# ucsdmanorlab/PSSR2

Hardware: AMD Instinct MI355X
Metric: HR tiles/sec (512^2 4xSR) train (higher is better)
Workload: dtype bf16

## Files before the change

### include/pssr_mi355.h

```cpp
#ifndef PSSR_MI355_H
#define PSSR_MI355_H

#include <stdint.h>

#ifdef __cplusplus
extern "C" {
#endif

typedef void* pssr_stream_t;

enum { PSSR_F32 = 0, PSSR_BF16 = 1, PSSR_F16 = 2 };

enum {
    PSSR_OK = 0,
    PSSR_ERR_ARG = -1,
    PSSR_ERR_LAUNCH = -2,
    PSSR_ERR_UNSUPPORTED = -3
};

int pssr_abi_version(void);
const char* pssr_last_error(void);

int pssr_pack_conv_weight(const float* w_oihw, void* packed, int cout, int cin, int ks,
                          int ci_begin, int ci_count, int mode, const int32_t* n_perm,
                          int k_pad, int n_pad, int dtype, pssr_stream_t stream);
typedef struct pssr_pack_item {
    const float* w; void* packed; const int32_t* n_perm;
    int32_t cout, cin, ks, ci_begin, ci_count, mode, k_pad, n_pad, dtype, center;
} pssr_pack_item;
int pssr_pack_conv_weight_batch(const pssr_pack_item* items_dev, int n_items, pssr_stream_t stream);
int64_t pssr_packed_weight_bytes(int taps, int k_pad, int n_pad, int dtype);

int pssr_unpack_conv_wgrad(const float* dw_packed, float* dw_oihw, int cout, int cin, int ks,
                           int ci_begin, int ci_count, int mode, const int32_t* n_perm,
                           int k_pad, int accumulate, pssr_stream_t stream);
int pssr_unpack_conv_wgrad_parts(const float* dw_parts, int parts, int rows, float* dw_oihw, int cout, int cin, int ks,
                                 int ci_begin, int ci_count, int mode, const int32_t* n_perm,
                                 int k_pad, int accumulate, pssr_stream_t stream);

enum { PSSR_PRO_NONE = 0, PSSR_PRO_BN_RELU = 1,
       PSSR_PRO_GELU = 2  };
enum {
    PSSR_EPI_STORE = 0,
    PSSR_EPI_TAIL = 1,
    PSSR_EPI_DGRAD_MASK = 2,
    PSSR_EPI_DGRAD_GELU = 4,
    PSSR_EPI_HEADQ = 5,
    PSSR_EPI_FINAL = 3
};
#define PSSR_STAT_STRIPES 32
#define PSSR_STAT_ROWS (2 * PSSR_STAT_STRIPES)

enum {
    PSSR_FLAG_RELU = 1,
    PSSR_FLAG_STATS = 2,
    PSSR_FLAG_HEADQ = 8,
    PSSR_FLAG_AFFINE = 4,
    PSSR_FLAG_SOLO = 32,
    PSSR_FLAG_SHUF2 = 16
};

typedef struct pssr_conv_desc {
    int32_t dtype;
    int32_t n, h, w;
    const void* in0; int32_t in0_cstride, in0_coff, cin0, taps0;
    const void* w0;
    const void* in1; int32_t in1_cstride, in1_coff, cin1, taps1;
    const void* w1;
    int32_t prologue;
    const float* pro_scale;
    const float* pro_shift;
    void* out; int32_t out_cstride, out_coff, cout, n_pad;
    const float* bias;
    int32_t epilogue, flags;
    const void* aux; int32_t aux_cstride, aux_coff;
    const float* aux_scale; const float* aux_shift;
    const float* aux_mean; const float* aux_invstd;
    double* stats;
    int32_t in0_blk, out_blk, aux_blk;
    float out_scale, out_shift;
    void* workspace; int64_t workspace_bytes;
    const float* head_w; float* head_q;
} pssr_conv_desc;

int pssr_conv2d(const pssr_conv_desc* desc, pssr_stream_t stream);
int64_t pssr_conv2d_workspace_bytes(const pssr_conv_desc* desc);
int pssr_conv2d_pipeline_mode(int mode);

int pssr_set_option(const char* name, int value);
int pssr_get_option(const char* name);

typedef struct pssr_wgrad_desc {
    int32_t dtype;
    int32_t n, h, w;
    const void* dy; int32_t dy_cstride, dy_coff, dy_blk, cout;
    const void* in; int32_t in_cstride, in_coff, in_blk, cin_pad;
    int32_t taps;
    int32_t prologue; const float* pro_scale; const float* pro_shift;
    float* dw;
    int32_t dw_parts;
} pssr_wgrad_desc;

int pssr_conv2d_wgrad(const pssr_wgrad_desc* desc, pssr_stream_t stream);
int pssr_conv2d_wgrad_parts(const pssr_wgrad_desc* desc);



int pssr_channel_stats_nchw(const float* x, int n, int c, int64_t hw, float pre_scale, float pre_shift,
                            double* stats, pssr_stream_t stream);

int pssr_bn_finalize(const double* stats, double count, const float* gamma, const float* beta, float eps,
                     float momentum, float* running_mean, float* running_var, float* scale, float* shift,
                     float* mean, float* invstd, int c, pssr_stream_t stream);
int pssr_bn_eval_affine(const float* gamma, const float* beta, const float* running_mean,
                        const float* running_var, float eps, float* scale, float* shift, int c,
                        pssr_stream_t stream);
int pssr_bn_relu_apply(const void* y, int y_cs, int y_co, const float* scale, const float* shift, void* a, int a_cs,
                       int a_co, int64_t npix, int c, int dtype, pssr_stream_t stream);
int pssr_bn_bwd_coefs(const double* stats, double count, const float* gamma, const float* mean,
                      const float* invstd, float* coef_a, float* coef_b, float* coef_c, float* dgamma,
                      float* dbeta, int c, pssr_stream_t stream);
int pssr_bn_bwd_apply(const void* g, int g_cs, int g_co, const void* y, int y_cs, int y_co,
                      const float* coef_a, const float* coef_b, const float* coef_c,
                      void* dy, int dy_cs, int dy_co, int64_t npix, int c, int dtype, pssr_stream_t stream);

int pssr_input_im2col(const float* x_nchw, void* xcol, int n, int c, int h, int w, int xc,
                      float pre_scale, float pre_shift, const float* scale, const float* shift,
                      int dtype, pssr_stream_t stream);
int pssr_input_norm_bwd(const void* dxcol_a, const void* dxcol_b, int xc, const float* x_nchw,
                        float pre_scale, float pre_shift, const float* mean, const float* invstd,
                        int n, int c, int h, int w, double* stats, int dtype, pssr_stream_t stream);

int pssr_input_norm_bwd2(const void* dxcol_a, const void* dxcol_b, int xc, const void* dpatch, int pc, int patch,
                         const float* x_nchw, float pre_scale, float pre_shift, const float* mean, const float* invstd,
                         int n, int c, int h, int w, double* stats, int dtype, pssr_stream_t stream);

int pssr_maxpool2(const void* in, int in_cs, int in_co, void* out, int out_cs, int out_co,
                  int n, int h, int w, int c, int dtype, pssr_stream_t stream);
int pssr_maxpool2_bwd(const void* act, int act_cs, int act_co, const void* dpool, int dp_cs, int dp_co,
                      const void* dskip, int ds_cs, int ds_co, void* dout, int do_cs, int do_co,
                      int n, int h, int w, int c, int dtype, pssr_stream_t stream);

int pssr_pixel_shuffle(const void* lo, int lo_cs, int lo_co, void* hi, int hi_cs, int hi_co,
                       int n, int h, int w, int c_hi, int r, int inverse, int dtype, pssr_stream_t stream);

int pssr_relu_bwd_stats(const void* dout, int do_cs, int do_co, const void* out, int o_cs, int o_co,
                        const void* y, int y_cs, int y_co, const float* mean, const float* invstd,
                        void* dz, int dz_cs, int dz_co, double* stats, int64_t npix, int c, int dtype,
                        pssr_stream_t stream);

int pssr_relu_bwd_stats_pool(const void* dpool, int dp_cs, int dp_co, const void* dskip, int ds_cs, int ds_co,
                             const void* out, int o_cs, int o_co, const void* y, int y_cs, int y_co,
                             const float* mean, const float* invstd, void* dz, int dz_cs, int dz_co, double* stats,
                             int n, int h, int w, int c, int dtype, pssr_stream_t stream);
int pssr_relu_bwd_stats_unshuffle(const void* dhi, int dh_cs, int dh_co, const void* out, int o_cs, int o_co,
                                  const void* y, int y_cs, int y_co, const float* mean, const float* invstd,
                                  void* dz, int dz_cs, int dz_co, double* stats, int n, int h, int w, int c, int dtype,
                                  pssr_stream_t stream);

int pssr_channel_sum_nhwc(const void* x, int cs, int co, int64_t npix, int c, double* out, int dtype,
                          pssr_stream_t stream);
int pssr_nchw_to_nhwc(const float* in, void* out, int n, int c, int64_t hw, int out_cs, float scale,
                      int dtype, pssr_stream_t stream);
int pssr_clip_u8(const float* in, uint8_t* out, int64_t n, pssr_stream_t stream);
int pssr_f64_to_f32(const double* in, float* out, int n, int accumulate, int stripes, pssr_stream_t stream);

int pssr_ssim_level_fwd(const float* x, const float* y, int planes, int h, int w, const float* win_host,
                        int k, float c1, float c2, double* sums, double* l1_sum, pssr_stream_t stream);
int pssr_avgpool2_planes(const float* in, float* out, int planes, int h, int w, pssr_stream_t stream);
int pssr_msssim_weights(const double* sums, int levels, int planes, const double* nvalid,
                        const float* level_weights, int ms, float mix, const double* l1_sum,
                        double l1_numel, const float* grad_out, float* loss_out, float* wts,
                        float* l1_coef, pssr_stream_t stream);
int pssr_ssim_level_bwd(const float* x, const float* y, int planes, int h, int w, const float* win_host,
                        int k, float c1, float c2, const float* wts, int use_ssim, const float* dcoarse,
                        int hc, int wc, const float* l1_coef, float* dx, pssr_stream_t stream);

int pssr_ssim_level_fwd_adj(const float* x, const float* y, float in_div, int planes, int h, int w, const float* win_host, int k,
                            float c1, float c2, int use_ssim, double* sums, double* l1_sum, int stripes, int64_t stripe_stride,
                            float* adj, pssr_stream_t stream);
int pssr_msssim_weights_striped(const double* sums, int stripes, int64_t stripe_stride, double* folded, int levels, int planes,
                                const double* nvalid, const float* level_weights, int ms, float mix, const double* l1_sum,
                                double l1_numel, const float* grad_out, float* loss_out, float* wts, float* l1_coef,
                                pssr_stream_t stream);
int pssr_ssim_level_bwd_adj(const float* x, const float* y, float in_div, const float* adj, int planes, int h, int w,
                            const float* win_host, int k, const float* wts, const float* dcoarse, int hc, int wc,
                            const float* l1_coef, float* dx, pssr_stream_t stream);
int pssr_avgpool2_planes_div(const float* in, float in_div, float* out, int planes, int h, int w, pssr_stream_t stream);
int pssr_avgpool2_pair_div(const float* x, const float* y, float in_div, float* xo, float* yo, int planes, int h, int w,
                           pssr_stream_t stream);

int pssr_adamw_step(float* p, const float* g, float* m, float* v, int64_t n, float lr, float beta1,
                    float beta2, float eps, float weight_decay, int64_t step, float grad_scale,
                    pssr_stream_t stream);
int pssr_adamw_step_dev(float* p, const float* g, float* m, float* v, int64_t n, int64_t* state,
                        float beta1, float beta2, float eps, float weight_decay, float grad_scale,
                        pssr_stream_t stream);
int pssr_amp_check(const float* g, int64_t n, int32_t* amp, pssr_stream_t stream);
int pssr_adamw_step_amp(float* p, const float* g, float* m, float* v, int64_t n, int64_t* state,
                        float beta1, float beta2, float eps, float weight_decay, float grad_scale,
                        int32_t* amp, float growth, float backoff, int interval, pssr_stream_t stream);

int pssr_bilinear_down_u8(const uint8_t* hr, uint8_t* tmp, uint8_t* lr, int planes, int H, int W,
                          int h, int w, pssr_stream_t stream);
int pssr_u8_to_f32(const uint8_t* in, float* out, int64_t n, pssr_stream_t stream);
int pssr_crappify_gaussian(const float* in, float* out, int tiles, int64_t per_tile, float intensity,
                           float gain, float spread, uint64_t seed, uint64_t tile_offset,
                           const double* noise, int flags, const uint64_t* tile_counter,
                           pssr_stream_t stream);
int pssr_crappify_poisson(const float* in, float* out, int tiles, int64_t per_tile, float intensity,
                          float gain, float spread, uint64_t seed, uint64_t tile_offset, int flags,
                          const uint64_t* tile_counter, pssr_stream_t stream);
int pssr_crappify_poisson_samples(const float* in, const double* samples, float* out, int64_t n, double intensity,
                                  double gain, int flags, pssr_stream_t stream);
int pssr_counter_add(uint64_t* counter, uint64_t inc, pssr_stream_t stream);
int pssr_gaussian_blur(const float* in, float* tmp, float* out, int planes, int h, int w, float sigma,
                       float gain, int flags, pssr_stream_t stream);

int pssr_crappify_saltpepper(const float* in, float* out, int tiles, int64_t per_tile, float amount, float gain, float spread,
                             uint64_t seed, uint64_t tile_offset, int flags, const uint64_t* tile_counter, pssr_stream_t stream);
int pssr_gaussian_blur_tiles(const float* in, float* tmp, float* out, int tiles, int planes_per_tile, int h, int w, float sigma,
                             float spread, float gain, uint64_t seed, uint64_t tile_offset, int flags, const uint64_t* tile_counter,
                             pssr_stream_t stream);
typedef struct pssr_gather_item { const uint8_t* src; int sh, sw, rot, flip_axis; } pssr_gather_item;
int pssr_gen_pair_geometry_u8(const pssr_gather_item* items_dev, int n_items, uint8_t* out, int c, int res, pssr_stream_t stream);
typedef struct pssr_sheet_desc { const uint8_t* base; int frames, h, w, reserved; } pssr_sheet_desc;
typedef struct pssr_window_item { int sheet, frame0, y0, x0, rot, flip_axis; } pssr_window_item;
int pssr_gather_windows_u8(const pssr_sheet_desc* sheets_dev, int n_sheets, const pssr_window_item* items_dev, int n_items,
                           uint8_t* out, int c, int res, pssr_stream_t stream);

typedef struct pssr_collage_panel {
    const void* src; int64_t image_stride; int32_t row_pitch, src_h, src_w, is_f32; const int32_t* yi; const int32_t* xi;
} pssr_collage_panel;
int pssr_collage_rows_u8(const pssr_collage_panel* panels, int n_panels, uint8_t* canvas, int64_t canvas_pitch, int row0, int n_images,
                         int h, int w, pssr_stream_t stream);

int64_t pssr_window_attn_workspace_bytes(int B, int H, int W, int heads, int ws);
int pssr_window_attn_fwd(const void* qkv, const float* bias_table, void* out, float* lse, int B, int H, int W, int C, int heads, int ws,
                         int shift, float scale, int dtype, pssr_stream_t stream);
int pssr_window_attn_bwd(const void* qkv, const float* bias_table, const float* lse, const void* dout, void* dqkv, float* dbias_table,
                         void* workspace, int64_t workspace_bytes, int B, int H, int W, int C, int heads, int ws, int shift, float scale,
                         int dtype, pssr_stream_t stream);


int pssr_input_plain(const float* x_nchw, void* out, int n, int c, int h, int w, int out_cs, float pre_scale, float pre_shift,
                     int dtype, pssr_stream_t stream);
int pssr_im2col_dil(const void* in, int in_cs, int in_co, int c, const float* scale, const float* shift, void* col, int cp,
                    int n, int h, int w, int dil, int dtype, pssr_stream_t stream);
int pssr_col2im_dil(const void* dcol, int cp, void* out, int out_cs, int out_co, int c, int n, int h, int w, int dil,
                    const void* y, int y_cs, int y_co, const float* scale, const float* shift, const float* mean,
                    const float* invstd, double* stats, int dtype, pssr_stream_t stream);
int pssr_channel_stats_nhwc(const void* x, int cs, int co, int c, int64_t npix, double* stats, int dtype, pssr_stream_t stream);
int pssr_sum_relu(const void* const* ins, const int* in_cs, const int* in_co, int n_in, void* out, int out_cs, int out_co,
                  int64_t npix, int c, int relu, int dtype, pssr_stream_t stream);
int pssr_relu_mask(const void* dout, int do_cs, int do_co, const void* out, int o_cs, int o_co, void* dz, int dz_cs, int dz_co,
                   int64_t npix, int c, int dtype, pssr_stream_t stream);
int pssr_affine_relu(const void* x, int cs, int co, const float* scale, const float* shift, void* out, int out_cs, int out_co,
                     int64_t npix, int c, int dtype, pssr_stream_t stream);
int pssr_maxpool_k(const void* in, int in_cs, int in_co, void* out, int out_cs, int out_co, int n, int h, int w, int c, int k,
                   int dtype, pssr_stream_t stream);
int pssr_maxpool_k_bwd(const void* act, int act_cs, int act_co, const void* dpool, int dp_cs, int dp_co, void* dx, int dx_cs,
                       int dx_co, int n, int h, int w, int c, int k, int dtype, pssr_stream_t stream);
int pssr_bilinear_up(const void* in, int in_cs, int in_co, void* out, int out_cs, int out_co, int n, int hs, int ws, int h, int w,
                     int c, int dtype, pssr_stream_t stream);
int pssr_bilinear_up_bwd(const void* dout, int do_cs, int do_co, void* din, int di_cs, int di_co, int n, int hs, int ws, int h,
                         int w, int c, int dtype, pssr_stream_t stream);

int pssr_input_patchify(const float* x_nchw, void* xpatch, int n, int c, int h, int w, int ps, int pc,
                        float pre_scale, float pre_shift, const float* scale, const float* shift, int dtype,
                        pssr_stream_t stream);
int pssr_dwconv7_pack(const float* w, float* packed, int c, int flip, pssr_stream_t stream);
#define PSSR_DWPACK_BATCH_MAX 48
typedef struct pssr_dwpack_batch {
    const float* w[PSSR_DWPACK_BATCH_MAX];
    float* packed[PSSR_DWPACK_BATCH_MAX];
    int32_t c[PSSR_DWPACK_BATCH_MAX];
    int32_t flip[PSSR_DWPACK_BATCH_MAX];
} pssr_dwpack_batch;
int pssr_dwconv7_pack_batch(const pssr_dwpack_batch* items, int n_items, pssr_stream_t stream);
int pssr_dwconv7(const void* in, int in_cs, int in_co, const float* w_packed, const float* bias, void* out, int out_cs,
                 int out_co, int n, int h, int w, int c, int accumulate, int dtype, pssr_stream_t stream);
int pssr_dwconv7_wgrad(const void* dy, int dy_cs, int dy_co, const void* x, int x_cs, int x_co, float* dw, int n, int h,
                       int w, int c, int dtype, pssr_stream_t stream);
int64_t pssr_dwconv7_wgrad_workspace_bytes(int n, int h, int w, int c);
int pssr_dwconv7_wgrad_ws(const void* dy, int dy_cs, int dy_co, const void* x, int x_cs, int x_co, float* dw, int n, int h,
                          int w, int c, int dtype, void* workspace, int64_t workspace_bytes, pssr_stream_t stream);
int pssr_layernorm2d_fwd(const void* in, int in_cs, int in_co, const float* gamma, const float* beta, float eps, void* out,
                         int out_cs, int out_co, int s2d, int c_pad, int n, int h, int w, int c, float* mean, float* rstd,
                         int dtype, pssr_stream_t stream);
int pssr_layernorm2d_bwd(const void* g, int g_cs, int g_co, int s2d, int c_pad, const void* x, int x_cs, int x_co,
                         const float* gamma, const float* mean, const float* rstd, void* dx, int dx_cs, int dx_co,
                         int accumulate, int n, int h, int w, int c, double* stats, int dtype, pssr_stream_t stream);
int pssr_image_channel_dot(const void* a, int a_cs, int a_co, const void* b, int b_cs, int b_co, int n, int hw, int c,
                           float scale, float* out, int dtype, pssr_stream_t stream);
int64_t pssr_image_channel_dot_workspace_bytes(int n, int hw, int c);
int pssr_image_channel_dot_ws(const void* a, int a_cs, int a_co, const void* b, int b_cs, int b_co, int n, int hw, int c,
                              float scale, float* out, int dtype, void* workspace, int64_t workspace_bytes, pssr_stream_t stream);
int pssr_ese_gate(const float* s_mean, const float* w_fc, const float* b_fc, int n, int c, float* u, float* gate,
                  pssr_stream_t stream);
int pssr_scale_nc(const void* t, int t_cs, int t_co, const float* gate, const float* gamma, const float* add, void* out,
                  int out_cs, int out_co, int n, int hw, int c, int dtype, pssr_stream_t stream);
int pssr_ese_bwd(const float* A, const float* gate, const float* u, const float* gamma, const float* s_mean,
                 const float* w_fc, int n, int c, int hw, float* du, float* dgamma, float* db_fc, float* dw_fc, float* add,
                 pssr_stream_t stream);

int pssr_head_q_gather(const float* q, const float* bias, float* out_nchw, int n, int h, int w,
                       float out_scale, float out_shift, pssr_stream_t stream);

int pssr_head_conv_fwd(const void* act, int act_cs, int act_co, int blk, const float* w_oihw, const float* bias,
                       float* out_nchw, int n, int h, int w, int cin, int cout, float out_scale, float out_shift,
                       int dtype, pssr_stream_t stream);
int pssr_head_conv_dgrad(const float* g_nchw, float g_scale, const float* w_oihw, const void* act, int act_cs, int act_co,
                         void* dact, int d_cs, int d_co, int blk, int n, int h, int w, int cin, int cout, int dtype,
                         pssr_stream_t stream);
int pssr_head_conv_wgrad(const float* g_nchw, float g_scale, const void* act, int act_cs, int act_co, int blk,
                         float* dw_oihw, int n, int h, int w, int cin, int cout, int dtype, pssr_stream_t stream);
int pssr_head_conv_bwd(const float* g_nchw, float g_scale, const float* w_oihw, const void* act, int act_cs, int act_co,
                       void* dact, int d_cs, int d_co, int blk, float* dw_oihw, float* bias_sum, int n, int h, int w, int cin,
                       int cout, int dtype, pssr_stream_t stream);

int pssr_head_conv_bwd_rows(const float* g_nchw, float g_scale, const float* w_oihw, const void* act, int act_cs, int act_co,
                            void* dact, int d_cs, int d_co, int blk, double* dw_rows, double* bias_rows, int n, int h, int w,
                            int cin, int cout, int dtype, pssr_stream_t stream);

int pssr_sliding_tiles_u8(const uint8_t* sheet, float* tiles, int c, int h, int w, int size, int stride, int tile0, int ntile,
                          pssr_stream_t stream);
int pssr_patch_tiles_u8(const uint8_t* tiles, uint8_t* sheet, int c, int n_rows, int n_cols, int size, int overlap, int margin,
                        pssr_stream_t stream);


int64_t pssr_normalize_preds_workspace_bytes(int64_t pixels_per_image);
int pssr_normalize_preds_u8(const uint8_t* hr, const uint8_t* hr_hat, uint8_t* hr_norm, uint8_t* hr_hat_norm, int n_images,
                            int64_t pixels_per_image, float pmin, float pmax, void* workspace, pssr_stream_t stream);
// ... 55 lines not shown
```

### pssr2_amd/_lib.py

```python
from __future__ import annotations

import ctypes as C
import os
from pathlib import Path

_LIB_PATH = Path(__file__).resolve().parent / "libpssr_mi355.so"
_lib = None

F32, BF16, F16 = 0, 1, 2
PRO_NONE, PRO_BN_RELU, PRO_GELU = 0, 1, 2
EPI_STORE, EPI_TAIL, EPI_DGRAD_MASK, EPI_FINAL, EPI_DGRAD_GELU, EPI_HEADQ = 0, 1, 2, 3, 4, 5
FLAG_RELU, FLAG_STATS, FLAG_AFFINE, FLAG_HEADQ, FLAG_SHUF2, FLAG_SOLO = 1, 2, 4, 8, 16, 32

c_void_p, c_int, c_i64, c_float = C.c_void_p, C.c_int, C.c_int64, C.c_float


class ConvDesc(C.Structure):
    _fields_ = [
        ("dtype", C.c_int32), ("n", C.c_int32), ("h", C.c_int32), ("w", C.c_int32),
        ("in0", c_void_p), ("in0_cstride", C.c_int32), ("in0_coff", C.c_int32), ("cin0", C.c_int32), ("taps0", C.c_int32),
        ("w0", c_void_p),
        ("in1", c_void_p), ("in1_cstride", C.c_int32), ("in1_coff", C.c_int32), ("cin1", C.c_int32), ("taps1", C.c_int32),
        ("w1", c_void_p),
        ("prologue", C.c_int32), ("pro_scale", c_void_p), ("pro_shift", c_void_p),
        ("out", c_void_p), ("out_cstride", C.c_int32), ("out_coff", C.c_int32), ("cout", C.c_int32), ("n_pad", C.c_int32),
        ("bias", c_void_p),
        ("epilogue", C.c_int32), ("flags", C.c_int32),
        ("aux", c_void_p), ("aux_cstride", C.c_int32), ("aux_coff", C.c_int32),
        ("aux_scale", c_void_p), ("aux_shift", c_void_p), ("aux_mean", c_void_p), ("aux_invstd", c_void_p),
        ("stats", c_void_p),
        ("in0_blk", C.c_int32), ("out_blk", C.c_int32), ("aux_blk", C.c_int32),
        ("out_scale", C.c_float), ("out_shift", C.c_float),
        ("workspace", c_void_p), ("workspace_bytes", C.c_int64),
        ("head_w", c_void_p), ("head_q", c_void_p),
    ]


class WgradDesc(C.Structure):
    _fields_ = [
        ("dtype", C.c_int32), ("n", C.c_int32), ("h", C.c_int32), ("w", C.c_int32),
        ("dy", c_void_p), ("dy_cstride", C.c_int32), ("dy_coff", C.c_int32), ("dy_blk", C.c_int32), ("cout", C.c_int32),
        ("in_", c_void_p), ("in_cstride", C.c_int32), ("in_coff", C.c_int32), ("in_blk", C.c_int32), ("cin_pad", C.c_int32),
        ("taps", C.c_int32),
        ("prologue", C.c_int32), ("pro_scale", c_void_p), ("pro_shift", c_void_p),
        ("dw", c_void_p), ("dw_parts", C.c_int32),
    ]


class GatherItem(C.Structure):
    _fields_ = [("src", C.c_void_p), ("sh", C.c_int), ("sw", C.c_int), ("rot", C.c_int), ("flip_axis", C.c_int)]


class SheetDesc(C.Structure):
    _fields_ = [("base", C.c_void_p), ("frames", C.c_int), ("h", C.c_int), ("w", C.c_int), ("reserved", C.c_int)]


class WindowItem(C.Structure):
    _fields_ = [("sheet", C.c_int), ("frame0", C.c_int), ("y0", C.c_int), ("x0", C.c_int), ("rot", C.c_int), ("flip_axis", C.c_int)]


class CollagePanel(C.Structure):
    _fields_ = [("src", C.c_void_p), ("image_stride", C.c_int64), ("row_pitch", C.c_int32), ("src_h", C.c_int32), ("src_w", C.c_int32),
                ("is_f32", C.c_int32), ("yi", C.c_void_p), ("xi", C.c_void_p)]


COPY_BATCH_MAX = 16


class FoldBatch(C.Structure):
    _fields_ = [("dst", C.c_void_p * 16), ("src", C.c_void_p * 16), ("n", C.c_int32 * 16), ("accumulate", C.c_int32 * 16)]


DWPACK_BATCH_MAX = 48


class DwPackBatch(C.Structure):
    _fields_ = [("w", C.c_void_p * DWPACK_BATCH_MAX), ("packed", C.c_void_p * DWPACK_BATCH_MAX), ("c", C.c_int32 * DWPACK_BATCH_MAX),
                ("flip", C.c_int32 * DWPACK_BATCH_MAX)]


class CopyBatch(C.Structure):
    _fields_ = [("dst", C.c_void_p * COPY_BATCH_MAX), ("src", C.c_void_p * COPY_BATCH_MAX), ("n", C.c_int64 * COPY_BATCH_MAX)]


class PackItem(C.Structure):
    _fields_ = [("w", c_void_p), ("packed", c_void_p), ("n_perm", c_void_p),
                ("cout", C.c_int32), ("cin", C.c_int32), ("ks", C.c_int32), ("ci_begin", C.c_int32), ("ci_count", C.c_int32),
                ("mode", C.c_int32), ("k_pad", C.c_int32), ("n_pad", C.c_int32), ("dtype", C.c_int32), ("center", C.c_int32)]


def lib():
    global _lib
    if _lib is None:
        if not _LIB_PATH.exists():
            raise RuntimeError(
                f"{_LIB_PATH} not found: build the HIP extension first (python -c 'import __graft_entry__ as g; g.build()' "
                "or make -C pssr2_amd/csrc). pssr2_amd has no CPU fallback.")
        import torch
        _lib = C.CDLL(str(_LIB_PATH))
        _lib.pssr_last_error.restype = C.c_char_p
        _lib.pssr_packed_weight_bytes.restype = C.c_int64
        _lib.pssr_conv2d_workspace_bytes.restype = C.c_int64
        _lib.pssr_gradhist_workspace_bytes.restype = C.c_int64
        _lib.pssr_noise_profile_workspace_bytes.restype = C.c_int64
        _lib.pssr_noise_profile_workspace_bytes.argtypes = [c_int, c_i64]
        for name in ("pssr_noise_profile_f32", "pssr_noise_profile_u8"):
            getattr(_lib, name).argtypes = [c_void_p, c_void_p, c_void_p, c_void_p, c_int, c_i64, c_void_p, c_i64, c_void_p]
        _lib.pssr_noise_profile_loss.argtypes = [c_void_p, c_void_p, c_void_p, c_void_p, c_int, c_i64, c_int, c_void_p, c_void_p, c_void_p,
                                                 c_void_p]
        _lib.pssr_gather_windows_u8.argtypes = [c_void_p, c_int, c_void_p, c_int, c_void_p, c_int, c_int, c_void_p]
        _lib.pssr_collage_rows_u8.argtypes = [c_void_p, c_int, c_void_p, c_i64, c_int, c_int, c_int, c_int, c_void_p]
        _lib.pssr_window_attn_workspace_bytes.restype = c_i64
        _lib.pssr_window_attn_workspace_bytes.argtypes = [c_int] * 5
        _lib.pssr_window_attn_fwd.argtypes = [c_void_p] * 4 + [c_int] * 7 + [c_float, c_int, c_void_p]
        _lib.pssr_window_attn_bwd.argtypes = [c_void_p] * 7 + [c_i64] + [c_int] * 7 + [c_float, c_int, c_void_p]
    return _lib


def check(status: int, what: str):
    if status != 0:
        raise RuntimeError(f"{what} failed ({status}): {lib().pssr_last_error().decode()}")


def ptr(t):
    return None if t is None else c_void_p(t.data_ptr())


def stream_ptr():
    import torch
    return c_void_p(torch.cuda.current_stream().cuda_stream)
```

### pssr2_amd/csrc/conv_igemm.hip

```cpp
#include "conv_igemm_args.h"

using pssr_conv::ConvArgs;

extern "C" int pssr_conv2d_pipeline_mode(int mode) {
    (void)mode;
    return 0;
}

static int conv2d_entry(const pssr_conv_desc* d, pssr_stream_t stream, long* query_ws);

#ifdef PSSR_V3_STAMPS
static unsigned* g_stamp_buf = nullptr;
extern "C" void pssr_debug_stamp_buffer(void* p) { g_stamp_buf = (unsigned*)p; }
#endif

extern "C" int pssr_conv2d(const pssr_conv_desc* d, pssr_stream_t stream) { return conv2d_entry(d, stream, nullptr); }

extern "C" int64_t pssr_conv2d_workspace_bytes(const pssr_conv_desc* d) {
    long bytes = 0;
    const int rc = conv2d_entry(d, nullptr, &bytes);
    return rc != PSSR_OK ? (int64_t)rc : (int64_t)bytes;
}

static int conv2d_entry(const pssr_conv_desc* d, pssr_stream_t stream, long* query_ws) {
    PSSR_CHECK(d != nullptr, PSSR_ERR_ARG, "conv2d: null desc");
    PSSR_CHECK(d->dtype == PSSR_F32 || d->dtype == PSSR_BF16 || d->dtype == PSSR_F16, PSSR_ERR_ARG, "conv2d: bad dtype %d", d->dtype);
    const int kch = d->dtype == PSSR_F32 ? 8 : 16;
    const int esz = d->dtype == PSSR_F32 ? 4 : 2;
    PSSR_CHECK(d->n > 0 && d->h > 0 && d->w > 0, PSSR_ERR_ARG, "conv2d: bad shape %dx%dx%d", d->n, d->h, d->w);
    PSSR_CHECK(query_ws || (d->in0 && d->w0 && d->out), PSSR_ERR_ARG, "conv2d: null pointer");
    PSSR_CHECK(d->cin0 > 0 && d->cin0 % kch == 0, PSSR_ERR_ARG, "conv2d: cin0=%d must be a positive multiple of %d", d->cin0, kch);
    PSSR_CHECK(d->taps0 == 9 || d->taps0 == 1, PSSR_ERR_ARG, "conv2d: taps0=%d", d->taps0);
    PSSR_CHECK((d->in0_cstride * esz) % 16 == 0 && (d->in0_coff * esz) % 16 == 0, PSSR_ERR_ARG, "conv2d: in0 stride/offset not 16-byte aligned");
    PSSR_CHECK(d->in0_coff + d->cin0 <= d->in0_cstride, PSSR_ERR_ARG, "conv2d: in0 slice exceeds stride");
    if (d->cin1) {
        PSSR_CHECK(d->in1 && d->w1 && d->cin1 % kch == 0 && d->taps1 == 1, PSSR_ERR_ARG, "conv2d: source 1 must be a 1x1 (or flat-K) source");
        PSSR_CHECK((d->in1_cstride * esz) % 16 == 0 && (d->in1_coff * esz) % 16 == 0 && d->in1_coff + d->cin1 <= d->in1_cstride, PSSR_ERR_ARG, "conv2d: in1 stride/offset");
    }
    if (d->epilogue == PSSR_EPI_FINAL) {
        PSSR_CHECK(d->cout > 0 && d->cout <= 32 && (d->flags & ~PSSR_FLAG_SOLO) == 0, PSSR_ERR_ARG, "conv2d: EPI_FINAL needs 0 < cout <= 32 and no flags");
    } else {
        PSSR_CHECK(d->cout > 0 && d->cout % 4 == 0, PSSR_ERR_ARG, "conv2d: cout=%d must be a positive multiple of 4", d->cout);
        PSSR_CHECK(d->out_coff % 4 == 0 && d->out_cstride % 4 == 0 &&
                   d->out_coff + ((d->flags & PSSR_FLAG_SHUF2) ? d->cout / 4 : d->cout) <= d->out_cstride, PSSR_ERR_ARG, "conv2d: out stride/offset");
    }
    PSSR_CHECK(d->n_pad % 128 == 0 && d->n_pad >= d->cout, PSSR_ERR_ARG, "conv2d: n_pad=%d", d->n_pad);
    PSSR_CHECK(d->prologue >= 0 && d->prologue <= PSSR_PRO_GELU, PSSR_ERR_ARG, "conv2d: prologue=%d", d->prologue);
    PSSR_CHECK(d->prologue != PSSR_PRO_BN_RELU || (d->pro_scale && d->pro_shift), PSSR_ERR_ARG, "conv2d: prologue needs scale/shift");
    PSSR_CHECK(d->epilogue >= 0 && d->epilogue <= 5, PSSR_ERR_ARG, "conv2d: epilogue=%d", d->epilogue);
    if (d->flags & PSSR_FLAG_HEADQ)
        PSSR_CHECK(d->epilogue == PSSR_EPI_STORE && !(d->flags & (PSSR_FLAG_STATS | PSSR_FLAG_AFFINE)) && (d->flags & PSSR_FLAG_RELU), PSSR_ERR_ARG,
                   "conv2d: FLAG_HEADQ goes with EPI_STORE | FLAG_RELU only");
    if (d->epilogue == PSSR_EPI_HEADQ || (d->flags & PSSR_FLAG_HEADQ)) {
        PSSR_CHECK(query_ws || (d->head_w && d->head_q), PSSR_ERR_ARG, "conv2d: EPI_HEADQ needs head_w / head_q");
        PSSR_CHECK(esz == 2 && d->cout == 1024 && d->taps0 == 9 && d->w >= 16 && d->h >= 16 && d->prologue != PSSR_PRO_GELU && !(d->flags & PSSR_FLAG_STATS),
                   PSSR_ERR_UNSUPPORTED, "conv2d: EPI_HEADQ needs 16-bit storage, a 3x3 source, cout = 16 x 64 (4 x upscaling) and at least 16x16 pixels");
    }
    PSSR_CHECK(d->in0_blk >= 0 && d->out_blk >= 0 && d->aux_blk >= 0 && d->in0_blk <= 3 && d->out_blk <= 3 && d->aux_blk <= 3, PSSR_ERR_ARG, "conv2d: blocked order");
    {
        const int mb = d->in0_blk > d->out_blk ? (d->in0_blk > d->aux_blk ? d->in0_blk : d->aux_blk) : (d->out_blk > d->aux_blk ? d->out_blk : d->aux_blk);
        PSSR_CHECK(d->h % (1 << mb) == 0 && d->w % (1 << mb) == 0, PSSR_ERR_ARG, "conv2d: blocked order needs H,W multiples of r");
    }
    if (d->epilogue == PSSR_EPI_TAIL || d->epilogue == PSSR_EPI_DGRAD_MASK) {
        PSSR_CHECK(d->aux && d->aux_scale && d->aux_shift && d->aux_coff % 4 == 0 && d->aux_cstride % 4 == 0, PSSR_ERR_ARG, "conv2d: epilogue needs aux tensor");
    }
    if (d->epilogue == PSSR_EPI_DGRAD_GELU)
        PSSR_CHECK(d->aux && d->aux_coff % 4 == 0 && d->aux_cstride % 4 == 0, PSSR_ERR_ARG, "conv2d: GELU backward needs the pre-activation as aux");
    if (d->flags & PSSR_FLAG_SHUF2) {
        PSSR_CHECK(d->epilogue == PSSR_EPI_STORE && !(d->flags & (PSSR_FLAG_STATS | PSSR_FLAG_HEADQ)) && d->out_blk == 0, PSSR_ERR_ARG,
                   "conv2d: FLAG_SHUF2 goes with EPI_STORE, without statistics, tap planes or a blocked output order");
        PSSR_CHECK(esz == 2 && d->cout % 32 == 0 && d->out_coff % 8 == 0 && d->out_cstride % 8 == 0 && pssr_tunables().conv_epi8, PSSR_ERR_UNSUPPORTED,
                   "conv2d: FLAG_SHUF2 needs 16-bit storage, cout a multiple of 32 and 8-channel aligned outputs");
    }
    if (d->flags & PSSR_FLAG_AFFINE) {
        PSSR_CHECK(d->epilogue == PSSR_EPI_STORE && !(d->flags & PSSR_FLAG_STATS) && d->aux_scale && d->aux_shift, PSSR_ERR_ARG,
                   "conv2d: FLAG_AFFINE needs EPI_STORE without statistics and aux_scale / aux_shift");
        PSSR_CHECK(esz == 2 && d->cout % 8 == 0 && d->out_coff % 8 == 0 && d->out_cstride % 8 == 0 && pssr_tunables().conv_epi8, PSSR_ERR_UNSUPPORTED,
                   "conv2d: FLAG_AFFINE needs 16-bit storage and 8-channel aligned outputs");
    }
    if (d->flags & PSSR_FLAG_STATS) {
        PSSR_CHECK(d->stats != nullptr, PSSR_ERR_ARG, "conv2d: stats buffer missing");
        PSSR_CHECK(d->epilogue != PSSR_EPI_DGRAD_MASK || (d->aux_mean && d->aux_invstd), PSSR_ERR_ARG, "conv2d: mask stats need mean/invstd");
        PSSR_CHECK(d->epilogue != PSSR_EPI_TAIL, PSSR_ERR_ARG, "conv2d: no stats on tail");
    }
    ConvArgs a;
    a.N = d->n; a.H = d->h; a.W = d->w;
    a.in[0] = d->in0; a.in_cs[0] = d->in0_cstride; a.in_co[0] = d->in0_coff; a.nchunks[0] = d->cin0 / kch; a.taps[0] = d->taps0; a.w[0] = d->w0;
    a.in[1] = d->in1; a.in_cs[1] = d->in1_cstride; a.in_co[1] = d->in1_coff; a.nchunks[1] = d->cin1 ? d->cin1 / kch : 0; a.taps[1] = d->cin1 ? d->taps1 : 1; a.w[1] = d->w1;
    a.prologue = d->prologue; a.pro_scale = d->pro_scale; a.pro_shift = d->pro_shift;
    a.out = d->out; a.out_cs = d->out_cstride; a.out_co = d->out_coff; a.cout = d->cout; a.n_pad = d->n_pad;
    a.bias = d->bias; a.epi = d->epilogue; a.flags = d->flags;
    a.aux = d->aux; a.aux_cs = d->aux_cstride; a.aux_co = d->aux_coff;
    a.aux_scale = d->aux_scale; a.aux_shift = d->aux_shift; a.aux_mean = d->aux_mean; a.aux_invstd = d->aux_invstd;
    a.stats = d->stats;
    a.in0_blk = d->in0_blk; a.out_blk = d->out_blk; a.aux_blk = d->aux_blk;
    a.out_scale = d->out_scale; a.out_shift = d->out_shift;
    const bool headq = a.epi == PSSR_EPI_HEADQ || (a.flags & PSSR_FLAG_HEADQ);
    a.head_w = headq ? d->head_w : nullptr;
    a.head_q = headq ? d->head_q : nullptr;
    a.tiles_x = a.tiles_y = a.tiles_n = 0;
    a.epi8 = esz == 2 && d->epilogue != PSSR_EPI_FINAL && d->cout % 8 == 0 && d->out_coff % 8 == 0 && d->out_cstride % 8 == 0 &&
             (d->epilogue == PSSR_EPI_STORE || d->epilogue == PSSR_EPI_HEADQ || (d->aux_coff % 8 == 0 && d->aux_cstride % 8 == 0));
    if (!pssr_tunables().conv_epi8) a.epi8 = 0;
    a.dbg = pssr_tunables().igemm_dbg;
    a.stamps = nullptr;
#ifdef PSSR_V3_STAMPS
    a.stamps = g_stamp_buf;
#endif
    long ws_query = 0;
    if (query_ws) { a.ksplit = -1; a.ws = (float*)&ws_query; }
    else { a.ws = (float*)d->workspace; a.ksplit = d->workspace ? (int)(d->workspace_bytes / 1024) : 0; }
    hipStream_t s = (hipStream_t)stream;
    const int rc = d->dtype == PSSR_BF16 ? pssr_conv::launch_bf16(a, s) : d->dtype == PSSR_F16 ? pssr_conv::launch_f16(a, s) : pssr_conv::launch_f32(a, s);
    if (query_ws) *query_ws = ws_query;
    return rc;
}
```

### pssr2_amd/csrc/conv_igemm_args.h

```cpp
#pragma once
#include "common.h"
#include "tunables.h"

namespace pssr_conv {

struct ConvArgs {
    int N, H, W;
    int tiles_x, tiles_y, tiles_n;
    const void* in[2]; int in_cs[2]; int in_co[2]; int nchunks[2]; int taps[2]; const void* w[2];
    int prologue; const float* pro_scale; const float* pro_shift;
    void* out; int out_cs, out_co, cout, n_pad;
    const float* bias;
    int epi, flags;
    const void* aux; int aux_cs, aux_co;
    const float* aux_scale; const float* aux_shift; const float* aux_mean; const float* aux_invstd;
    double* stats;
    int in0_blk, out_blk, aux_blk;
    float out_scale, out_shift;
    int epi8;
    unsigned* stamps;
    int dbg;
    int ksplit; float* ws;
    const float* head_w; float* head_q;
};

int launch_bf16(const ConvArgs& a, hipStream_t s);
int launch_f16(const ConvArgs& a, hipStream_t s);
int launch_f32(const ConvArgs& a, hipStream_t s);

}
```

### pssr2_amd/csrc/conv_igemm_impl.h

```cpp
#pragma once
#include <type_traits>

#include "conv_igemm_args.h"

using pssr_conv::ConvArgs;

namespace {



constexpr int PRO_LDS_MAX = 4096 * 8;

template <int GEO> struct Geo;
template <> struct Geo<0> { static constexpr int TWL = 4, THL = 3; };
template <> struct Geo<1> { static constexpr int TWL = 3, THL = 3; };
template <> struct Geo<2> { static constexpr int TWL = 2, THL = 2; };
template <> struct Geo<3> { static constexpr int TWL = 1, THL = 1; };
template <> struct Geo<4> { static constexpr int TWL = 0, THL = 0; };
template <> struct Geo<5> { static constexpr int TWL = 4, THL = 4; };

template <int BN, int GEO> struct Cfg {
    static constexpr int TWL = Geo<GEO>::TWL, THL = Geo<GEO>::THL;
    static constexpr bool BIG = GEO == 5;
    static_assert(!BIG || BN == 64, "the 256-pixel tile is built for 64 output channels");
// ... 4 lines not shown
    static constexpr int HW2 = TW + 2, HPI = (TH + 2) * (TW + 2), HP = NI * HPI;
    static constexpr int HWP = (TW == 16 && !BIG) ? 32 : HW2;
    static constexpr int HPIP = (TH + 2) * HWP;
    static constexpr int A_ITEMS = (2 * HP + 255) / 256;
    static constexpr int A_BYTES = NI * HPIP * 32;
    static constexpr int B_BYTES = 9 * BN * 32;
    static constexpr int B_ITEMS = (9 * BN * 2 + 255) / 256;
    static constexpr int E_BYTES = WM * 32 * BN * 4;
    static constexpr int RED_BYTES = 4 * BN * 2 * 4;
    static constexpr int MAIN_BYTES = A_BYTES + B_BYTES;
    static constexpr int LDS_BYTES = (MAIN_BYTES > E_BYTES + RED_BYTES) ? MAIN_BYTES : (E_BYTES + RED_BYTES);
    static constexpr int PERM = 0;
};

template <class C> __device__ __forceinline__ int epi_pixel(int row, int mi) {
    int r = row & 31;
    if constexpr (C::PERM != 0) {
        const int rx = r & 15, ry = (r >> 4) ^ ((rx >= 4 && rx < 12) ? 1 : 0);
        if constexpr (C::PERM == 2)
            return (((row >> 5) * 4 + (mi >> 1) * 2 + ry) << 5) | ((mi & 1) << 4) | rx;
        r = (ry << 4) | rx;
    }
    return (row >> 5) * C::MI * 32 + mi * 32 + r;
}

template <typename T, int BN, class C>
__device__ __forceinline__ void conv_epilogue(const ConvArgs& p, f32x16 (&acc)[C::MI][C::NJ], char* smem, int tid, int x0, int y0, int img0, int n0) {
    using X = TT<T>;
    const int lane = tid & 63, wave = tid >> 6;
    const int wm = wave / C::WN, wn = wave % C::WN;
    const int h = lane >> 5, r = lane & 31;
    float* Es = (float*)smem;
    float* Red = (float*)(smem + C::E_BYTES);
    constexpr int CG = BN / 4;
    constexpr int PASSES = C::WM * 32 * CG / 256;
#pragma unroll
    for (int nj = 0; nj < C::NJ; ++nj)
#pragma unroll
        for (int e = 0; e < 16; ++e) {
            const int row = wm * 32 + (e & 3) + 8 * (e >> 2) + 4 * h;
            const int col = wn * C::NJ * 32 + nj * 32 + r;
            Es[row * BN + col] = acc[0][nj][e];
        }
    asm volatile("" ::: "memory");
    const int c4 = tid % CG;
    const int n_base = n0 + c4 * 4;
    const bool n_ok = n_base < p.cout;
    float bias[4] = {0, 0, 0, 0}, xs[4] = {0, 0, 0, 0}, xh[4] = {0, 0, 0, 0}, xm[4] = {0, 0, 0, 0}, xi[4] = {0, 0, 0, 0};
    if (n_ok) {
        if (p.bias) {
            if (p.epi == PSSR_EPI_FINAL) { for (int e = 0; e < 4; ++e) if (n_base + e < p.cout) bias[e] = p.bias[n_base + e]; }
            else load4(p.bias + n_base, bias);
        }
        if (p.epi == PSSR_EPI_TAIL || p.epi == PSSR_EPI_DGRAD_MASK) { load4(p.aux_scale + n_base, xs); load4(p.aux_shift + n_base, xh); }
        if (p.epi == PSSR_EPI_DGRAD_MASK && (p.flags & PSSR_FLAG_STATS)) {
            load4(p.aux_mean + n_base, xm); load4(p.aux_invstd + n_base, xi);
        }
    }
    float s1[4] = {0, 0, 0, 0}, s2[4] = {0, 0, 0, 0};
    T* outp = (T*)p.out;
    const T* auxp = (const T*)p.aux;

#pragma unroll
    for (int mi = 0; mi < C::MI; ++mi) {
        if (mi) {
            __syncthreads();
#pragma unroll
            for (int nj = 0; nj < C::NJ; ++nj)
#pragma unroll
                for (int e = 0; e < 16; ++e) {
                    const int row = wm * 32 + (e & 3) + 8 * (e >> 2) + 4 * h;
                    const int col = wn * C::NJ * 32 + nj * 32 + r;
                    Es[row * BN + col] = acc[mi][nj][e];
                }
        }
        __syncthreads();
#pragma unroll
        for (int ps = 0; ps < PASSES; ++ps) {
            const int piece = tid + ps * 256;
            const int row = piece / CG;
            const int m = epi_pixel<C>(row, mi);
            const int tx = m & (C::TW - 1), ty = (m >> C::TWL) & (C::TH - 1), img = m >> (C::TWL + C::THL);
            const int gy = y0 + ty, gx = x0 + tx, gi = img0 + img;
            if (!(n_ok && gi < p.N && gy < p.H && gx < p.W)) continue;
            float v[4];
            load4(Es + row * BN + c4 * 4, v);
            if (p.epi == PSSR_EPI_FINAL) {
                float* of = (float*)p.out;
#pragma unroll
                for (int e = 0; e < 4; ++e)
                    if (n_base + e < p.cout)
                        of[(((long)gi * p.cout + n_base + e) * p.H + gy) * p.W + gx] = fmaf(v[e] + bias[e], p.out_scale, p.out_shift);
                continue;
            }
            const long pix = pix_index(gi, gy, gx, p.H, p.W, p.out_blk);
            if (p.epi == PSSR_EPI_STORE) {
#pragma unroll
                for (int e = 0; e < 4; ++e) {
                    v[e] += bias[e];
                    if (p.flags & PSSR_FLAG_RELU) v[e] = fmaxf(v[e], 0.f);
                }
            } else {
                float a[4];
                load4(auxp + pix_index(gi, gy, gx, p.H, p.W, p.aux_blk) * p.aux_cs + p.aux_co + n_base, a);
                if (p.epi == PSSR_EPI_TAIL) {
#pragma unroll
                    for (int e = 0; e < 4; ++e) v[e] = fmaxf(v[e] + bias[e] + fmaf(a[e], xs[e], xh[e]), 0.f);
                } else if (p.epi == PSSR_EPI_DGRAD_GELU) {
                    gelu_grad_mul_vec<T, 4>(a, v);
                } else {
#pragma unroll
                    for (int e = 0; e < 4; ++e) {
                        v[e] = (fmaf(a[e], xs[e], xh[e]) > 0.f) ? v[e] : 0.f;
                        a[e] = (a[e] - xm[e]) * xi[e];
                    }
                }
                if (p.flags & PSSR_FLAG_STATS) {
#pragma unroll
                    for (int e = 0; e < 4; ++e) { const float g = X::round(v[e]); s1[e] += g; s2[e] += g * a[e]; }
                }
            }
            if (p.epi == PSSR_EPI_STORE && (p.flags & PSSR_FLAG_STATS)) {
#pragma unroll
                for (int e = 0; e < 4; ++e) { const float g = X::round(v[e]); s1[e] += g; s2[e] += g * g; }
            }
            store4(outp + pix * p.out_cs + p.out_co + n_base, v);
        }
    }
    if (p.flags & PSSR_FLAG_STATS) {
#pragma unroll
        for (int off = 32; off >= CG; off >>= 1)
#pragma unroll
            for (int e = 0; e < 4; ++e) { s1[e] += __shfl_xor(s1[e], off); s2[e] += __shfl_xor(s2[e], off); }
        if (lane < CG) {
#pragma unroll
            for (int e = 0; e < 4; ++e) {
                Red[(wave * BN + lane * 4 + e) * 2 + 0] = s1[e];
                Red[(wave * BN + lane * 4 + e) * 2 + 1] = s2[e];
            }
        }
        __syncthreads();
        if (tid < BN && n0 + tid < p.cout) {
            float t1 = 0, t2 = 0;
#pragma unroll
            for (int w = 0; w < 4; ++w) { t1 += Red[(w * BN + tid) * 2]; t2 += Red[(w * BN + tid) * 2 + 1]; }
            double* st = p.stats + (long)(blockIdx.x % PSSR_STAT_STRIPES) * 2 * p.cout;
            const long lo = (long)PSSR_STAT_STRIPES * 2 * p.cout;
            stat_add(st + n0 + tid, lo, t1);
            stat_add(st + p.cout + n0 + tid, lo, t2);
        }
    }
}

template <typename T, int BN, class C, int EPI, bool STATS, bool TR = false, bool AFF = false>
__device__ __forceinline__ void conv_epilogue8(const ConvArgs& p, f32x16 (&acc)[C::MI][C::NJ], char* smem, int tid, int x0, int y0, int img0, int n0) {
    static_assert(!AFF || (EPI == PSSR_EPI_STORE && !STATS), "FLAG_AFFINE: EPI_STORE without statistics");
    using X = TT<T>;
    static_assert(sizeof(T) == 2, "8-channel pieces are 16 bytes of a 16-bit type");
    const int lane = tid & 63, wave = tid >> 6;
    const int wm = wave / C::WN, wn = wave % C::WN;
    const int h = lane >> 5, r = lane & 31;
    float* Es = (float*)smem;
    float* Red = (float*)(smem + C::E_BYTES);
    constexpr int CG = BN / 8, RP = 256 / CG;
    constexpr int EP = TR ? BN + 4 : BN;
    constexpr int ROWS = C::WM * 32, PASSES = ROWS / RP;
    static_assert(PASSES >= 1 && ROWS % RP == 0, "pass geometry");
    int wcol[C::NJ];
#pragma unroll
    for (int nj = 0; nj < C::NJ; ++nj) {
        const int col = wn * C::NJ * 32 + nj * 32 + r;
        wcol[nj] = ((col >> 2) & 1) * (BN / 2) + ((col >> 3) << 2) + (col & 3);
    }
    auto es_write = [&](int mi) {
        if constexpr (TR) {
#pragma unroll
            for (int nj = 0; nj < C::NJ; ++nj)
#pragma unroll
                for (int q = 0; q < 4; ++q) {
                    const int c = (wn * C::NJ + nj) * 4 + q;
                    *(float4*)(Es + (wm * 32 + r) * EP + h * (BN / 2) + 4 * c) =
                        make_float4(acc[mi][nj][4 * q], acc[mi][nj][4 * q + 1], acc[mi][nj][4 * q + 2], acc[mi][nj][4 * q + 3]);
                }
        } else {
#pragma unroll
            for (int nj = 0; nj < C::NJ; ++nj)
#pragma unroll
                for (int e = 0; e < 16; ++e) {
                    const int row = wm * 32 + (e & 3) + 8 * (e >> 2) + 4 * h;
                    Es[row * EP + wcol[nj]] = acc[mi][nj][e];
                }
        }
    };
    es_write(0);
    asm volatile("" ::: "memory");
    const int c8 = tid % CG, rs = tid / CG;
    const int row0 = (TR && CG == 8) ? ((rs >> 1) & 7) + ((rs & 1) << 3) + ((rs >> 4) << 4) : rs;
    const int n_base = n0 + c8 * 8;
    const bool n_ok = n_base < p.cout;
    float bias[8] = {0, 0, 0, 0, 0, 0, 0, 0}, xs[8], xh[8], xm[8], xi[8];
#pragma unroll
    for (int e = 0; e < 8; ++e) { xs[e] = 0.f; xh[e] = 0.f; xm[e] = 0.f; xi[e] = 0.f; }
    if (n_ok) {
        if ((EPI == PSSR_EPI_STORE || EPI == PSSR_EPI_TAIL) && p.bias) { load4(p.bias + n_base, bias); load4(p.bias + n_base + 4, bias + 4); }
        if (EPI == PSSR_EPI_TAIL || EPI == PSSR_EPI_DGRAD_MASK || AFF) {
            load4(p.aux_scale + n_base, xs); load4(p.aux_scale + n_base + 4, xs + 4);
            load4(p.aux_shift + n_base, xh); load4(p.aux_shift + n_base + 4, xh + 4);
        }
        if (EPI == PSSR_EPI_DGRAD_MASK && STATS) {
            load4(p.aux_mean + n_base, xm); load4(p.aux_mean + n_base + 4, xm + 4);
            load4(p.aux_invstd + n_base, xi); load4(p.aux_invstd + n_base + 4, xi + 4);
        }
    }
    const float relu_lo = (EPI == PSSR_EPI_STORE && (p.flags & PSSR_FLAG_RELU)) ? 0.f : -__builtin_inff();
    float s1[8], s2[8];
#pragma unroll
    for (int e = 0; e < 8; ++e) { s1[e] = 0.f; s2[e] = 0.f; }
    T* outp = (T*)p.out + p.out_co + n_base;
    const T* auxp = (const T*)p.aux + p.aux_co + n_base;
    const bool shuf = EPI == PSSR_EPI_STORE && !STATS && (p.flags & PSSR_FLAG_SHUF2);
    int shuf_i = 0, shuf_j = 0;
    if (shuf) {
        const int q4 = p.cout >> 2, s = n_base / q4;
        shuf_i = s >> 1; shuf_j = s & 1;
        outp = (T*)p.out + p.out_co + (n_base - s * q4);
    }

#pragma unroll
    for (int mi = 0; mi < C::MI; ++mi) {
        if (mi) {
            __syncthreads();
            es_write(mi);
        }
        __syncthreads();
#pragma unroll 1
        for (int ps = 0; ps < PASSES; ++ps) {
            const int row = row0 + ps * RP;
            const int m = epi_pixel<C>(row, mi);
            const int tx = m & (C::TW - 1), ty = (m >> C::TWL) & (C::TH - 1), img = m >> (C::TWL + C::THL);
            const int gy = y0 + ty, gx = x0 + tx, gi = img0 + img;
            if (!(n_ok && gi < p.N && gy < p.H && gx < p.W)) continue;
            float v[8];
            load4(Es + row * EP + c8 * 4, v);
            load4(Es + row * EP + BN / 2 + c8 * 4, v + 4);
            float a[8];
            if (EPI != PSSR_EPI_STORE) {
                const u32x4 araw = *(const u32x4*)(auxp + pix_index(gi, gy, gx, p.H, p.W, p.aux_blk) * p.aux_cs);
                X::unpack(araw, a);
            }
            if constexpr (EPI == PSSR_EPI_DGRAD_GELU) gelu_grad_mul_vec<T, 8>(a, v);
#pragma unroll
            for (int e = 0; e < 8; ++e) {
                if (EPI == PSSR_EPI_STORE) v[e] = fmaxf(AFF ? fmaf(v[e] + bias[e], xs[e], xh[e]) : v[e] + bias[e], relu_lo);
                else if (EPI == PSSR_EPI_TAIL) v[e] = fmaxf(v[e] + bias[e] + fmaf(a[e], xs[e], xh[e]), 0.f);
                else if (EPI == PSSR_EPI_DGRAD_GELU) {}
                else {
                    v[e] = (fmaf(a[e], xs[e], xh[e]) > 0.f) ? v[e] : 0.f;
                    a[e] = (a[e] - xm[e]) * xi[e];
                }
            }
            const u32x4 packed = X::pack(v);
            if (STATS) {
                float g[8];
                X::unpack(packed, g);
#pragma unroll
                for (int e = 0; e < 8; ++e) {
                    if (EPI == PSSR_EPI_DGRAD_GELU) asm volatile("v_add_f32 %0, %0, %1" : "+v"(s1[e]) : "v"(g[e]));
                    else s1[e] += g[e];
                    s2[e] += g[e] * (EPI == PSSR_EPI_STORE ? g[e] : a[e]);
                }
            }
            const long opix = shuf ? ((long)gi * 2 * p.H + 2 * gy + shuf_i) * (2 * p.W) + 2 * gx + shuf_j : pix_index(gi, gy, gx, p.H, p.W, p.out_blk);
            *(u32x4*)(outp + opix * p.out_cs) = packed;
        }
    }
    if (STATS) {
#pragma unroll
        for (int off = 32; off >= CG; off >>= 1)
#pragma unroll
            for (int e = 0; e < 8; ++e) { s1[e] += __shfl_xor(s1[e], off); s2[e] += __shfl_xor(s2[e], off); }
        if (lane < CG) {
#pragma unroll
            for (int e = 0; e < 8; ++e) {
                Red[(wave * BN + lane * 8 + e) * 2 + 0] = s1[e];
                Red[(wave * BN + lane * 8 + e) * 2 + 1] = s2[e];
            }
        }
        __syncthreads();
        if (tid < BN && n0 + tid < p.cout) {
            float t1 = 0, t2 = 0;
#pragma unroll
            for (int w = 0; w < 4; ++w) { t1 += Red[(w * BN + tid) * 2]; t2 += Red[(w * BN + tid) * 2 + 1]; }
            double* st = p.stats + (long)(blockIdx.x % PSSR_STAT_STRIPES) * 2 * p.cout;
            const long lo = (long)PSSR_STAT_STRIPES * 2 * p.cout;
            stat_add(st + n0 + tid, lo, t1);
            stat_add(st + p.cout + n0 + tid, lo, t2);
        }
    }
}

constexpr int HEADQ_LDS = (64 * 9 + 128) * 4;
__device__ __forceinline__ void conv_headq_stage(const ConvArgs& p, float* hq, int tid, int n0) {
    for (int i = tid; i < 64 * 9; i += 256) hq[i] = p.head_w[i];
    if (tid < 128) hq[576 + tid] = (p.bias && n0 + tid < p.cout) ? p.bias[n0 + tid] : 0.f;
}

template <typename T, class C>
__device__ __forceinline__ void conv_headq_epilogue(const ConvArgs& p, f32x16 (&acc)[C::MI][C::NJ], const float* hq, char* smem, int tid, int x0, int y0, int img0,
                                                    int n0) {
    using X = TT<T>;
    static_assert(sizeof(T) == 2 && C::NJ == 2 && C::MI == 4, "conv_v3 tiles of 128 channels");
    const int lane = tid & 63, wave = tid >> 6;
    const int wm = wave / C::WN, wn = wave % C::WN;
    const int h = lane >> 5, r = lane & 31;
    const int cbase = n0 + wn * 64;
    const int sub = cbase >> 6;
    float bias[2][16];
    u32x4 wa[2][2];
#pragma unroll
    for (int nj = 0; nj < 2; ++nj) {
#pragma unroll
        for (int e = 0; e < 16; ++e) bias[nj][e] = hq[576 + wn * 64 + nj * 32 + (e & 3) + 8 * (e >> 2) + 4 * h];
#pragma unroll
        for (int ks = 0; ks < 2; ++ks) {
            float wv[8];
#pragma unroll
            for (int i = 0; i < 8; ++i) {
                const int e = 8 * ks + i;
                const int c = nj * 32 + (e & 3) + 8 * (e >> 2) + 4 * h;
                wv[i] = r < 9 ? hq[c * 9 + r] : 0.f;
            }
            wa[nj][ks] = X::pack(wv);
        }
    }
    const long lrplane = (long)p.N * p.H * p.W;
    float* const qsub = p.head_q + (long)sub * lrplane + (long)img0 * p.H * p.W;
#pragma unroll
    for (int mi = 0; mi < 4; ++mi) {
        f32x16 q;
#pragma unroll
        for (int e = 0; e < 16; ++e) q[e] = 0.f;
#pragma unroll
        for (int nj = 0; nj < 2; ++nj)
#pragma unroll
            for (int ks = 0; ks < 2; ++ks) {
                float v[8];
#pragma unroll
                for (int i = 0; i < 8; ++i) v[i] = fmaxf(acc[mi][nj][8 * ks + i] + bias[nj][8 * ks + i], 0.f);
                X::mma(q, wa[nj][ks], X::pack(v));
            }
        const int m = epi_pixel<C>(wm * 32 + r, mi);
        const int tx = m & (C::TW - 1), ty = (m >> C::TWL) & (C::TH - 1);
        const int gy = y0 + ty, gx = x0 + tx;
        if (gy < p.H && gx < p.W) {
            float* const d = qsub + (long)gy * p.W + gx;
#pragma unroll
            for (int u = 0; u < 4; ++u) d[(long)(4 * h + u) * 16 * lrplane] = q[u];
            if (h == 0) d[(long)8 * 16 * lrplane] = q[4];
        }
    }
    (void)smem;
}

template <typename T, int BN, class C, bool TR = false>
__device__ __forceinline__ void conv_epilogue8_any(const ConvArgs& p, f32x16 (&acc)[C::MI][C::NJ], char* smem, int tid, int x0, int y0, int img0, int n0) {
    const bool st = p.flags & PSSR_FLAG_STATS;
    switch (p.epi) {
    case PSSR_EPI_STORE:
        if (st) conv_epilogue8<T, BN, C, PSSR_EPI_STORE, true, TR>(p, acc, smem, tid, x0, y0, img0, n0);
        else if (p.flags & PSSR_FLAG_AFFINE) conv_epilogue8<T, BN, C, PSSR_EPI_STORE, false, TR, true>(p, acc, smem, tid, x0, y0, img0, n0);
        else conv_epilogue8<T, BN, C, PSSR_EPI_STORE, false, TR>(p, acc, smem, tid, x0, y0, img0, n0);
        return;
    case PSSR_EPI_TAIL: conv_epilogue8<T, BN, C, PSSR_EPI_TAIL, false, TR>(p, acc, smem, tid, x0, y0, img0, n0); return;
    case PSSR_EPI_DGRAD_MASK:
        if (st) conv_epilogue8<T, BN, C, PSSR_EPI_DGRAD_MASK, true, TR>(p, acc, smem, tid, x0, y0, img0, n0);
        else conv_epilogue8<T, BN, C, PSSR_EPI_DGRAD_MASK, false, TR>(p, acc, smem, tid, x0, y0, img0, n0);
        return;
    default:
        if (st) conv_epilogue8<T, BN, C, PSSR_EPI_DGRAD_GELU, true, TR>(p, acc, smem, tid, x0, y0, img0, n0);
        else conv_epilogue8<T, BN, C, PSSR_EPI_DGRAD_GELU, false, TR>(p, acc, smem, tid, x0, y0, img0, n0);
        return;
    }
}

template <typename T, int BN, class C>
__device__ __forceinline__ void conv_epilogue_any(const ConvArgs& p, f32x16 (&acc)[C::MI][C::NJ], char* smem, int tid, int x0, int y0, int img0, int n0) {
    if constexpr (sizeof(T) == 2) {
        if (p.epi8) { conv_epilogue8_any<T, BN, C>(p, acc, smem, tid, x0, y0, img0, n0); return; }
    }
    conv_epilogue<T, BN, C>(p, acc, smem, tid, x0, y0, img0, n0);
}

template <typename T, int BN, int GEO, int TAPS0>
__global__ __launch_bounds__(256) void conv_igemm_kernel(const ConvArgs p) {
    using C = Cfg<BN, GEO>;
    using X = TT<T>;
    constexpr int EPS = X::EPS, KCH = X::KCH;
    extern __shared__ __attribute__((aligned(16))) char smem[];
    char* As = smem;
    char* Bs = smem + C::A_BYTES;

    const int tid = threadIdx.x, lane = tid & 63, wave = tid >> 6;
    const int wm = wave / C::WN, wn = wave % C::WN;
    const int h = lane >> 5, r = lane & 31;

    int bid = blockIdx.x;
    if (p.ksplit <= 1 && !(p.dbg & 64)) {
        const int per = gridDim.x >> 3;
        if (bid < per * 8) bid = (bid & 7) * per + (bid >> 3);
    }
    const int tn = bid % p.tiles_n;
    int tmi = bid / p.tiles_n;
    const int tile_x = tmi % p.tiles_x; tmi /= p.tiles_x;
    const int tile_y = tmi % p.tiles_y;
    const int tile_i = tmi / p.tiles_y;
    const int x0 = tile_x << C::TWL, y0 = tile_y << C::THL, img0 = tile_i * C::NI, n0 = tn * BN;

    const long img_base = (long)img0 * p.H * p.W;
    constexpr int ESZ = (int)sizeof(T);
    unsigned a_off0[C::A_ITEMS], a_off1[C::A_ITEMS];
    int a_lds[C::A_ITEMS];
    bool a_ok[C::A_ITEMS];
    const int half = tid & 1;
#pragma unroll
    for (int it = 0; it < C::A_ITEMS; ++it) {
        const int idx = tid + it * 256;
        const int pp = idx >> 1;
        const int img = pp / C::HPI, rem = pp % C::HPI;
        const int hy = rem / C::HW2, hx = rem % C::HW2;
        const int gy = y0 + hy - 1, gx = x0 + hx - 1, gi = img0 + img;
        const bool inb = (idx < 2 * C::HP) && gi < p.N && gy >= 0 && gy < p.H && gx >= 0 && gx < p.W;
        a_ok[it] = inb;
        a_off0[it] = inb ? (unsigned)((pix_index(gi, gy, gx, p.H, p.W, p.in0_blk) - img_base) * p.in_cs[0] * ESZ + half * 16) : 0u;
        a_off1[it] = inb ? (unsigned)(((long)img * p.H + gy) * p.W + gx) * (unsigned)(p.in_cs[1] * ESZ) + half * 16 : 0u;
        const int pl = img * C::HPIP + hy * C::HWP + hx;
        a_lds[it] = (idx < 2 * C::HP) ? (pl * 32 + ((half ^ ((pl >> 3) & 1)) << 4)) : -1;
    }
    const __amdgpu_buffer_rsrc_t ra0 = __builtin_amdgcn_make_buffer_rsrc(
        (void*)((const char*)p.in[0] + (img_base * p.in_cs[0] + p.in_co[0]) * ESZ), 0, (int)0xfffffff0u, 0x00020000);
    const __amdgpu_buffer_rsrc_t ra1 = __builtin_amdgcn_make_buffer_rsrc(
        (void*)((const char*)p.in[1] + (img_base * p.in_cs[1] + p.in_co[1]) * ESZ), 0, (int)0xfffffff0u, 0x00020000);
    const __amdgpu_buffer_rsrc_t rw0 = __builtin_amdgcn_make_buffer_rsrc((void*)((const char*)p.w[0] + (long)n0 * 32), 0, (int)0xfffffff0u, 0x00020000);
    const __amdgpu_buffer_rsrc_t rw1 = __builtin_amdgcn_make_buffer_rsrc((void*)((const char*)p.w[1] + (long)n0 * 32), 0, (int)0xfffffff0u, 0x00020000);
    constexpr int PT = BN * 2, TPI = 256 / PT;
    const int tap_stride = p.n_pad * 32;
    const unsigned b_voff = (unsigned)((tid / PT) * tap_stride + (tid % PT) * 16);
    const unsigned b_voff_tail = (unsigned)((tid % PT) * 16);
    constexpr int CT = (TAPS0 == 9) ? 4 : 0;
    int a_rd[C::MI][TAPS0];
#pragma unroll
// ... 557 lines not shown
```

### pssr2_amd/csrc/loss.hip

```cpp
#include "common.h"

namespace {

constexpr int TS = 32;
constexpr int MAXW = 33;

struct Win { float g[MAXW]; int k; };

template <int K_DUMMY>
__global__ __launch_bounds__(256) void ssim_fwd_kernel(const float* __restrict__ X, const float* __restrict__ Y, int H, int W,
                                                       Win win, float C1, float C2, double* sums ,
                                                       double* l1_sum ) {
    extern __shared__ float lds[];
    const int k = win.k, halo = k - 1, IN = TS + halo;
    float* xs = lds;
    float* ys = xs + IN * IN;
    float* hp = ys + IN * IN;
    const int plane = blockIdx.z;
    const int oy0 = blockIdx.y * TS, ox0 = blockIdx.x * TS;
    const int VH = H - halo, VW = W - halo;
    const float* xp = X + (long)plane * H * W;
    const float* yp = Y + (long)plane * H * W;
    const int tid = threadIdx.x;
    float l1 = 0.f;
// ... 223 lines not shown
        }
        th[i] = s0; th[AD * TS + i] = s1; th[2 * AD * TS + i] = s2;
    }
    __syncthreads();
    const float l1c = l1_coef_p ? l1_coef_p[0] : 0.f;
    const int r5 = k / 2;
    float* dxp = dX + (long)plane * H * W;
    for (int i = tid; i < TS * TS; i += 256) {
        const int r = i / TS, c = i % TS;
        const int gy = qy0 + r, gx = qx0 + c;
        if (gy >= H || gx >= W) continue;
        float s0 = 0, s1 = 0, s2 = 0;
        for (int t = 0; t < k; ++t) {
            const float gw = win.g[t];
            const int src = (r + halo - t) * TS + c;
            s0 = fmaf(gw, th[src], s0); s1 = fmaf(gw, th[AD * TS + src], s1); s2 = fmaf(gw, th[2 * AD * TS + src], s2);
        }
        const float xv = xs[(r + halo) * IN + c + halo], yv = ys[(r + halo) * IN + c + halo];
        float g = s0 + 2.f * xv * s1 + yv * s2;
        if (dcoarse) {
            const int cy = (gy + (H & 1)) >> 1, cx = (gx + (W & 1)) >> 1;
            g += 0.25f * dcoarse[((long)plane * HC + cy) * WC + cx];
        }
        if (l1c != 0.f) {
            float sy = 0.f, sx = 0.f;
            for (int t = 0; t < k; ++t) {
                const int yy = gy + t - r5, xx = gx + t - r5;
                if (yy >= 0 && yy < H) sy += win.g[t];
                if (xx >= 0 && xx < W) sx += win.g[t];
            }
            const float d = xv - yv;
            g += l1c * sy * sx * (d > 0.f ? 1.f : (d < 0.f ? -1.f : 0.f));
        }
        dxp[(long)gy * W + gx] = g;
    }
}

template <int K, int SEG, int NQ>
__device__ __forceinline__ void fir_seg(const float (*v)[SEG + K - 1], const Win& win, float (*out)[SEG]) {
#pragma unroll
    for (int o = 0; o < SEG; ++o)
#pragma unroll
        for (int q = 0; q < NQ; ++q) {
            float s = 0.f;
#pragma unroll
            for (int t = 0; t < K; ++t) s = fmaf(win.g[t], v[q][o + t], s);
            out[q][o] = s;
        }
}

template <int K>
__global__ __launch_bounds__(256) void ssim_fwd_k(const float* __restrict__ X, const float* __restrict__ Y, int H, int W,
                                                  Win win, float C1, float C2, double* sums, double* l1_sum) {
    constexpr int halo = K - 1, IN = TS + halo, SEG = 8, NS = TS / SEG;
    constexpr int HPW = TS + 1;
    extern __shared__ float lds[];
    float* xs = lds;
    float* ys = xs + IN * IN;
    float* hp = ys + IN * IN;
    const int plane = blockIdx.z;
    const int oy0 = blockIdx.y * TS, ox0 = blockIdx.x * TS;
    const int VH = H - halo, VW = W - halo;
    const float* xp = X + (long)plane * H * W;
    const float* yp = Y + (long)plane * H * W;
    const int tid = threadIdx.x;
    float l1 = 0.f;
    for (int i = tid; i < IN * IN; i += 256) {
        const int r = i / IN, c = i % IN;
        const int gy = oy0 + r, gx = ox0 + c;
        float xv = 0.f, yv = 0.f;
        if (gy < H && gx < W) { xv = xp[(long)gy * W + gx]; yv = yp[(long)gy * W + gx]; }
        xs[i] = xv; ys[i] = yv;
    }
    __syncthreads();
    if (l1_sum) {
        constexpr int r5 = K / 2;
        float wsum = 0.f;
#pragma unroll
        for (int t = 0; t < K; ++t) wsum += win.g[t];
        for (int i = tid; i < TS * TS; i += 256) {
            const int r = i / TS, c = i % TS;
            const int gy = oy0 + r, gx = ox0 + c;
            if (gy < H && gx < W) {
                float sy = wsum, sx = wsum;
                if (gy < r5 || gy >= H - r5) {
                    sy = 0.f;
#pragma unroll
                    for (int t = 0; t < K; ++t) { const int yy = gy + t - r5; if (yy >= 0 && yy < H) sy += win.g[t]; }
                }
                if (gx < r5 || gx >= W - r5) {
                    sx = 0.f;
#pragma unroll
                    for (int t = 0; t < K; ++t) { const int xx = gx + t - r5; if (xx >= 0 && xx < W) sx += win.g[t]; }
                }
                l1 += fabsf(xs[r * IN + c] - ys[r * IN + c]) * sy * sx;
            }
        }
    }
    for (int it = tid; it < IN * NS; it += 256) {
        const int r = it / NS, c0 = (it % NS) * SEG;
        float v[5][SEG + K - 1];
#pragma unroll
        for (int j = 0; j < SEG + K - 1; ++j) {
            const float a = xs[r * IN + c0 + j], b = ys[r * IN + c0 + j];
            v[0][j] = a; v[1][j] = b; v[2][j] = a * a; v[3][j] = b * b; v[4][j] = a * b;
        }
        float o[5][SEG];
        fir_seg<K, SEG, 5>(v, win, o);
#pragma unroll
        for (int q = 0; q < 5; ++q)
#pragma unroll
            for (int j = 0; j < SEG; ++j) hp[q * IN * HPW + r * HPW + c0 + j] = o[q][j];
    }
    __syncthreads();
    float cs_acc = 0.f, ss_acc = 0.f;
    for (int it = tid; it < TS * NS; it += 256) {
        const int c = it % TS, r0 = (it / TS) * SEG;
        float v[5][SEG + K - 1];
#pragma unroll
        for (int q = 0; q < 5; ++q)
#pragma unroll
            for (int j = 0; j < SEG + K - 1; ++j) v[q][j] = hp[q * IN * HPW + (r0 + j) * HPW + c];
        float m[5][SEG];
        fir_seg<K, SEG, 5>(v, win, m);
#pragma unroll
        for (int j = 0; j < SEG; ++j) {
            if (oy0 + r0 + j >= VH || ox0 + c >= VW) continue;
            const float mx = m[0][j], my = m[1][j];
            const float sxx = m[2][j] - mx * mx, syy = m[3][j] - my * my, sxy = m[4][j] - mx * my;
            const float Dcs = sxx + syy + C2;
            const float cs = (2.f * sxy + C2) / Dcs;
            const float Dl = mx * mx + my * my + C1;
            const float lum = (2.f * mx * my + C1) / Dl;
            cs_acc += cs; ss_acc += lum * cs;
        }
    }
    __shared__ float red[3][256];
    red[0][tid] = cs_acc; red[1][tid] = ss_acc; red[2][tid] = l1;
    __syncthreads();
    for (int o = 128; o > 0; o >>= 1) {
        if (tid < o) { red[0][tid] += red[0][tid + o]; red[1][tid] += red[1][tid + o]; red[2][tid] += red[2][tid + o]; }
        __syncthreads();
    }
    if (tid == 0) {
        atomicAdd(sums + plane * 2, (double)red[0][0]);
        atomicAdd(sums + plane * 2 + 1, (double)red[1][0]);
        if (l1_sum) atomicAdd(l1_sum, (double)red[2][0]);
    }
}

template <int K>
__global__ __launch_bounds__(256) void ssim_fwd_adj_k(const float* __restrict__ X, const float* __restrict__ Y, int H, int W,
                                                      Win win, float C1, float C2, double* sums, double* l1_sum, int stripes, long stripe_stride,
                                                      float* __restrict__ adj, int use_ssim, float in_mul) {
    constexpr int halo = K - 1, IN = TS + halo, SEG = 8, NS = TS / SEG;
    constexpr int HPW = TS + 1;
    extern __shared__ float lds[];
    float* xs = lds;
    float* ys = xs + IN * IN;
    float* hp = ys + IN * IN;
    const int plane = blockIdx.z;
    const int oy0 = blockIdx.y * TS, ox0 = blockIdx.x * TS;
    const int VH = H - halo, VW = W - halo;
    const float* xp = X + (long)plane * H * W;
    const float* yp = Y + (long)plane * H * W;
    const int tid = threadIdx.x;
    float l1 = 0.f;
    for (int i = tid; i < IN * IN; i += 256) {
        const int r = i / IN, c = i % IN;
        const int gy = oy0 + r, gx = ox0 + c;
        float xv = 0.f, yv = 0.f;
        if (gy < H && gx < W) { xv = __fmul_rn(xp[(long)gy * W + gx], in_mul); yv = __fmul_rn(yp[(long)gy * W + gx], in_mul); }
        xs[i] = xv; ys[i] = yv;
    }
    __syncthreads();
    if (l1_sum) {
        constexpr int r5 = K / 2;
        float wsum = 0.f;
#pragma unroll
        for (int t = 0; t < K; ++t) wsum += win.g[t];
        for (int i = tid; i < TS * TS; i += 256) {
            const int r = i / TS, c = i % TS;
            const int gy = oy0 + r, gx = ox0 + c;
            if (gy < H && gx < W) {
                float sy = wsum, sx = wsum;
                if (gy < r5 || gy >= H - r5) {
                    sy = 0.f;
#pragma unroll
                    for (int t = 0; t < K; ++t) { const int yy = gy + t - r5; if (yy >= 0 && yy < H) sy += win.g[t]; }
                }
                if (gx < r5 || gx >= W - r5) {
                    sx = 0.f;
#pragma unroll
                    for (int t = 0; t < K; ++t) { const int xx = gx + t - r5; if (xx >= 0 && xx < W) sx += win.g[t]; }
                }
                l1 += fabsf(xs[r * IN + c] - ys[r * IN + c]) * sy * sx;
            }
        }
    }
    const bool vitem = tid < TS * NS;
    const int vc = tid % TS, vr0 = (tid / TS) * SEG;
    float m[5][SEG];
#pragma unroll
    for (int q = 0; q < 5; ++q) {
        for (int it = tid; it < IN * NS; it += 256) {
            const int r = it / NS, c0 = (it % NS) * SEG;
            float v[1][SEG + K - 1];
#pragma unroll
            for (int j = 0; j < SEG + K - 1; ++j) {
                const float a = (q == 1 || q == 3) ? 0.f : xs[r * IN + c0 + j];
                const float b = (q == 0 || q == 2) ? 0.f : ys[r * IN + c0 + j];
                v[0][j] = q == 0 ? a : q == 1 ? b : q == 2 ? a * a : q == 3 ? b * b : a * b;
            }
            float o[1][SEG];
            fir_seg<K, SEG, 1>(v, win, o);
#pragma unroll
            for (int j = 0; j < SEG; ++j) hp[r * HPW + c0 + j] = o[0][j];
        }
        __syncthreads();
        if (vitem) {
            float v[1][SEG + K - 1];
#pragma unroll
            for (int j = 0; j < SEG + K - 1; ++j) v[0][j] = hp[(vr0 + j) * HPW + vc];
            float o[1][SEG];
            fir_seg<K, SEG, 1>(v, win, o);
#pragma unroll
            for (int j = 0; j < SEG; ++j) m[q][j] = o[0][j];
        }
        if (q < 4) __syncthreads();
    }
    float cs_acc = 0.f, ss_acc = 0.f;
    if (vitem) {
#pragma unroll
        for (int j = 0; j < SEG; ++j) {
            if (oy0 + vr0 + j >= VH || ox0 + vc >= VW) continue;
            const float mx = m[0][j], my = m[1][j];
            const float sxx = m[2][j] - mx * mx, syy = m[3][j] - my * my, sxy = m[4][j] - mx * my;
            const float Dcs = sxx + syy + C2;
            const float cs = (2.f * sxy + C2) / Dcs;
            const float Dl = mx * mx + my * my + C1;
            const float lum = (2.f * mx * my + C1) / Dl;
            cs_acc += cs; ss_acc += lum * cs;
            const float dcs_dmx = 2.f * (cs * mx - my) / Dcs, dcs_dexx = -cs / Dcs, dcs_dexy = 2.f / Dcs;
            float a = dcs_dmx, b = dcs_dexx, cc = dcs_dexy;
            if (use_ssim) {
                const float dl_dmx = 2.f * (my - lum * mx) / Dl;
                a = lum * dcs_dmx + cs * dl_dmx; b = lum * dcs_dexx; cc = lum * dcs_dexy;
            }
            float* ap = adj + ((long)plane * 3 * H + (oy0 + vr0 + j)) * W + ox0 + vc;
            ap[0] = a; ap[(long)H * W] = b; ap[2L * H * W] = cc;
        }
    }
    __shared__ float red[3][256];
    red[0][tid] = cs_acc; red[1][tid] = ss_acc; red[2][tid] = l1;
    __syncthreads();
    for (int o = 128; o > 0; o >>= 1) {
        if (tid < o) { red[0][tid] += red[0][tid + o]; red[1][tid] += red[1][tid + o]; red[2][tid] += red[2][tid + o]; }
        __syncthreads();
    }
    if (tid == 0) {
        const long so = (long)((blockIdx.x + blockIdx.y * 5) % stripes) * stripe_stride, lo = (long)stripes * stripe_stride;
        stat_add(sums + so + plane * 2, lo, red[0][0]);
        stat_add(sums + so + plane * 2 + 1, lo, red[1][0]);
        if (l1_sum) stat_add(l1_sum + so, lo, red[2][0]);
    }
}

template <int K>
__global__ __launch_bounds__(256) void ssim_bwd_adj_k(const float* __restrict__ X, const float* __restrict__ Y, const float* __restrict__ ADJ,
                                                      int H, int W, Win win, const float* __restrict__ wts,
                                                      const float* __restrict__ dcoarse, int HC, int WC, const float* l1_coef_p,
                                                      float* __restrict__ dX, float in_mul) {
    constexpr int halo = K - 1, AD = TS + halo;
    constexpr int SEG = 8, NS = TS / SEG;
    constexpr int ADC = AD + 1;
    constexpr int THR = AD + SEG, THW = TS + 1;
    constexpr int NL = (AD * AD + 255) / 256;
    extern __shared__ float lds[];
    float* ad = lds;
    float* th = lds + AD * ADC;
    const int plane = blockIdx.z;
    const int qy0 = blockIdx.y * TS, qx0 = blockIdx.x * TS;
    const int VH = H - halo, VW = W - halo;
    const float* xp = X + (long)plane * H * W;
    const float* yp = Y + (long)plane * H * W;
    const float* ap = ADJ + (long)plane * 3 * H * W;
    const int tid = threadIdx.x;
    const float wt = wts[plane];
    int goff[NL], lslot[NL];
#pragma unroll
    for (int u = 0; u < NL; ++u) {
        const int i = tid + u * 256;
        const int r = i / AD, c = i - r * AD;
        const int py = qy0 - halo + r, px = qx0 - halo + c;
        lslot[u] = i < AD * AD ? r * ADC + c : -1;
        goff[u] = (i < AD * AD && py >= 0 && py < VH && px >= 0 && px < VW) ? py * W + px : -1;
    }
    float pre[NL];
#define SB_LOAD(Q)                                                                                                \
    _Pragma("unroll") for (int u = 0; u < NL; ++u) pre[u] = goff[u] >= 0 ? wt * ap[(long)(Q) * H * W + goff[u]] : 0.f;
    SB_LOAD(0)
    const bool vitem = tid < TS * NS;
    const int vc = tid % TS, vr0 = (tid / TS) * SEG;
    float xv[SEG], yv[SEG], gsum[SEG];
#pragma unroll
    for (int o = 0; o < SEG; ++o) {
        const int gy = qy0 + vr0 + o, gx = qx0 + vc;
        const bool ok = vitem && gy < H && gx < W;
        xv[o] = ok ? __fmul_rn(xp[(long)gy * W + gx], in_mul) : 0.f;
        yv[o] = ok ? __fmul_rn(yp[(long)gy * W + gx], in_mul) : 0.f;
        gsum[o] = 0.f;
    }
#pragma unroll
    for (int q = 0; q < 3; ++q) {
#pragma unroll
        for (int u = 0; u < NL; ++u) if (lslot[u] >= 0) ad[lslot[u]] = pre[u];
        __syncthreads();
        if (q < 2) { SB_LOAD(q + 1) }
        for (int it = tid; it < AD * NS; it += 256) {
            const int r = it / NS, c0 = (it % NS) * SEG;
            float v[SEG + K - 1];
#pragma unroll
            for (int j = 0; j < SEG + K - 1; ++j) v[j] = ad[r * ADC + c0 + j];
#pragma unroll
            for (int o = 0; o < SEG; ++o) {
                float s_ = 0.f;
#pragma unroll
                for (int t = 0; t < K; ++t) s_ = fmaf(win.g[t], v[o + halo - t], s_);
// ... 95 lines not shown
        float o[5][SA];
        fir_seg<K, SA, 5>(v, win, o);
#pragma unroll
        for (int q = 0; q < 5; ++q)
#pragma unroll
            for (int j = 0; j < SA; ++j) hp[q * IN * ADP + r * ADP + c0 + j] = o[q][j];
    }
    __syncthreads();
    for (int it = tid; it < AD * NSA; it += 256) {
        const int c = it % AD, r0 = (it / AD) * SA;
        float v[5][SA + K - 1];
#pragma unroll
        for (int q = 0; q < 5; ++q)
#pragma unroll
            for (int j = 0; j < SA + K - 1; ++j) {
                const int rr = r0 + j;
                v[q][j] = rr < IN ? hp[q * IN * ADP + rr * ADP + c] : 0.f;
            }
        float m[5][SA];
        fir_seg<K, SA, 5>(v, win, m);
#pragma unroll
        for (int j = 0; j < SA; ++j) {
            const int r = r0 + j;
            if (r >= AD) continue;
            const int py = qy0 - halo + r, px = qx0 - halo + c;
            float a = 0.f, b = 0.f, cc = 0.f;
            if (py >= 0 && py < VH && px >= 0 && px < VW) {
                const float mx = m[0][j], my = m[1][j];
                const float sxx = m[2][j] - mx * mx, syy = m[3][j] - my * my, sxy = m[4][j] - mx * my;
                const float Dcs = sxx + syy + C2, cs = (2.f * sxy + C2) / Dcs;
                const float dcs_dmx = 2.f * (cs * mx - my) / Dcs, dcs_dexx = -cs / Dcs, dcs_dexy = 2.f / Dcs;
                if (use_ssim) {
                    const float Dl = mx * mx + my * my + C1, lum = (2.f * mx * my + C1) / Dl;
                    const float dl_dmx = 2.f * (my - lum * mx) / Dl;
                    a = wt * (lum * dcs_dmx + cs * dl_dmx); b = wt * lum * dcs_dexx; cc = wt * lum * dcs_dexy;
                } else {
                    a = wt * dcs_dmx; b = wt * dcs_dexx; cc = wt * dcs_dexy;
                }
            }
            ad[0 * ADR * ADC + r * ADC + c] = a; ad[1 * ADR * ADC + r * ADC + c] = b; ad[2 * ADR * ADC + r * ADC + c] = cc;
        }
    }
    __syncthreads();
    float* th = hp;
    constexpr int THR = AD + SEG;
    for (int it = tid; it < AD * NS; it += 256) {
        const int r = it / NS, c0 = (it % NS) * SEG;
#pragma unroll
        for (int q = 0; q < 3; ++q) {
            float v[SEG + K - 1];
#pragma unroll
            for (int j = 0; j < SEG + K - 1; ++j) v[j] = ad[q * ADR * ADC + r * ADC + c0 + j];
#pragma unroll
            for (int o = 0; o < SEG; ++o) {
                float s = 0.f;
#pragma unroll
                for (int t = 0; t < K; ++t) s = fmaf(win.g[t], v[o + halo - t], s);
                th[q * THR * TS + r * TS + c0 + o] = s;
            }
        }
    }
    __syncthreads();
    const float l1c = l1_coef_p ? l1_coef_p[0] : 0.f;
    constexpr int r5 = K / 2;
    float wsum = 0.f;
#pragma unroll
    for (int t = 0; t < K; ++t) wsum += win.g[t];
    float* dxp = dX + (long)plane * H * W;
    for (int it = tid; it < TS * NS; it += 256) {
        const int c = it % TS, r0 = (it / TS) * SEG;
        float s[3][SEG];
#pragma unroll
        for (int q = 0; q < 3; ++q) {
            float v[SEG + K - 1];
#pragma unroll
            for (int j = 0; j < SEG + K - 1; ++j) v[j] = th[q * THR * TS + (r0 + j) * TS + c];
#pragma unroll
            for (int o = 0; o < SEG; ++o) {
                float a = 0.f;
#pragma unroll
                for (int t = 0; t < K; ++t) a = fmaf(win.g[t], v[o + halo - t], a);
                s[q][o] = a;
            }
        }
#pragma unroll
        for (int o = 0; o < SEG; ++o) {
            const int r = r0 + o;
            const int gy = qy0 + r, gx = qx0 + c;
            if (gy >= H || gx >= W) continue;
            const float xv = xp[(long)gy * W + gx], yv = yp[(long)gy * W + gx];
            float g = s[0][o] + 2.f * xv * s[1][o] + yv * s[2][o];
            if (dcoarse) {
                const int cy = (gy + (H & 1)) >> 1, cx = (gx + (W & 1)) >> 1;
                g += 0.25f * dcoarse[((long)plane * HC + cy) * WC + cx];
            }
            if (l1c != 0.f) {
                float sy = wsum, sx = wsum;
                if (gy < r5 || gy >= H - r5) {
                    sy = 0.f;
#pragma unroll
                    for (int t = 0; t < K; ++t) { const int yy = gy + t - r5; if (yy >= 0 && yy < H) sy += win.g[t]; }
                }
                if (gx < r5 || gx >= W - r5) {
                    sx = 0.f;
#pragma unroll
                    for (int t = 0; t < K; ++t) { const int xx = gx + t - r5; if (xx >= 0 && xx < W) sx += win.g[t]; }
                }
                const float d = xv - yv;
                g += l1c * sy * sx * (d > 0.f ? 1.f : (d < 0.f ? -1.f : 0.f));
            }
            dxp[(long)gy * W + gx] = g;
        }
    }
}

template <int K> constexpr size_t bwd_lds_k() {
    constexpr int halo = K - 1, AD = TS + halo, IN = TS + 2 * halo, SA = 7, NSA = (AD + SA - 1) / SA, ADP = NSA * SA, INP = IN + SA;
    return (size_t)(2 * IN * INP + 5 * IN * ADP) * sizeof(float);
}

Win make_win(const float* g, int k) {
    Win w; w.k = k;
    for (int i = 0; i < MAXW; ++i) w.g[i] = i < k ? g[i] : 0.f;
    return w;
}

}

extern "C" {

int pssr_ssim_level_fwd(const float* x, const float* y, int planes, int h, int w, const float* win_host, int k,
                        float c1, float c2, double* sums, double* l1_sum, pssr_stream_t s) {
    PSSR_CHECK(x && y && sums && win_host && planes > 0 && k > 0 && k <= MAXW && (k & 1), PSSR_ERR_ARG, "ssim_level_fwd: bad args");
    PSSR_CHECK(h >= k && w >= k, PSSR_ERR_ARG, "ssim_level_fwd: image %dx%d smaller than window %d", h, w, k);
    const int IN = TS + k - 1;
    const size_t lds = (size_t)(2 * IN * IN + 5 * IN * (TS + 1)) * sizeof(float);
    const int eh = l1_sum ? h : h - k + 1, ew = l1_sum ? w : w - k + 1;
    static bool attr = false;
    if (!attr) {
        (void)hipFuncSetAttribute((const void*)ssim_fwd_kernel<0>, hipFuncAttributeMaxDynamicSharedMemorySize, 160 * 1024 - 4096);
        (void)hipFuncSetAttribute((const void*)ssim_fwd_k<11>, hipFuncAttributeMaxDynamicSharedMemorySize, 160 * 1024 - 4096);
        attr = true;
    }
    if (k == 11)
        hipLaunchKernelGGL(ssim_fwd_k<11>, dim3(cdiv(ew, TS), cdiv(eh, TS), planes), dim3(256), lds, (hipStream_t)s, x, y, h, w,
                           make_win(win_host, k), c1, c2, sums, l1_sum);
    else
        hipLaunchKernelGGL(ssim_fwd_kernel<0>, dim3(cdiv(ew, TS), cdiv(eh, TS), planes), dim3(256), lds, (hipStream_t)s, x, y, h, w,
                           make_win(win_host, k), c1, c2, sums, l1_sum);
    PSSR_LAUNCH_CHECK();
    return PSSR_OK;
}

int pssr_ssim_level_fwd_adj(const float* x, const float* y, float in_div, int planes, int h, int w, const float* win_host, int k, float c1,
                            float c2, int use_ssim, double* sums, double* l1_sum, int stripes, int64_t stripe_stride, float* adj,
                            pssr_stream_t s) {
    PSSR_CHECK(x && y && sums && win_host && planes > 0 && adj && k == 11, PSSR_ERR_ARG,
               "ssim_level_fwd_adj: needs the adjoint buffer and the 11-tap window (k=%d)", k);
    PSSR_CHECK(h >= k && w >= k && stripes >= 1 && (stripes == 1 || stripe_stride > 0) && in_div > 0.f, PSSR_ERR_ARG, "ssim_level_fwd_adj: bad size / stripes / in_div");
    const int IN = TS + k - 1;
    const size_t lds = (size_t)(2 * IN * IN + IN * (TS + 1)) * sizeof(float);
    const int eh = l1_sum ? h : h - k + 1, ew = l1_sum ? w : w - k + 1;
    hipLaunchKernelGGL(ssim_fwd_adj_k<11>, dim3(cdiv(ew, TS), cdiv(eh, TS), planes), dim3(256), lds, (hipStream_t)s, x, y, h, w,
                       make_win(win_host, k), c1, c2, sums, l1_sum, stripes, (long)stripe_stride, adj, use_ssim, in_div == 1.f ? 1.f : 1.f / in_div);
    PSSR_LAUNCH_CHECK();
    return PSSR_OK;
}

int pssr_ssim_level_bwd_adj(const float* x, const float* y, float in_div, const float* adj, int planes, int h, int w, const float* win_host,
                            int k, const float* wts, const float* dcoarse, int hc, int wc, const float* l1_coef, float* dx, pssr_stream_t s) {
    PSSR_CHECK(x && y && adj && wts && dx && win_host && planes > 0 && k == 11, PSSR_ERR_ARG, "ssim_level_bwd_adj: bad args (k=%d)", k);
    constexpr int AD = TS + 10;
    const size_t lds = (size_t)(AD * (AD + 1) + (AD + 8) * (TS + 1)) * sizeof(float);
    hipLaunchKernelGGL(ssim_bwd_adj_k<11>, dim3(cdiv(w, TS), cdiv(h, TS), planes), dim3(256), lds, (hipStream_t)s, x, y, adj, h, w,
                       make_win(win_host, k), wts, dcoarse, hc, wc, l1_coef, dx, in_div == 1.f ? 1.f : 1.f / in_div);
    PSSR_LAUNCH_CHECK();
    return PSSR_OK;
}

int pssr_avgpool2_planes(const float* in, float* out, int planes, int h, int w, pssr_stream_t s) {
    return pssr_avgpool2_planes_div(in, 1.f, out, planes, h, w, s);
}

int pssr_avgpool2_planes_div(const float* in, float in_div, float* out, int planes, int h, int w, pssr_stream_t s) {
    PSSR_CHECK(in && out && planes > 0 && h > 0 && w > 0 && in_div > 0.f, PSSR_ERR_ARG, "avgpool2_planes: bad args");
    const int ho = (h + 2 * (h & 1) - 2) / 2 + 1, wo = (w + 2 * (w & 1) - 2) / 2 + 1;
    const long total = (long)planes * ho * wo;
    int blocks = (int)((total + 255) / 256); if (blocks > 8192) blocks = 8192;
    hipLaunchKernelGGL(avgpool_kernel, dim3(blocks), dim3(256), 0, (hipStream_t)s, in, out, in, out, planes, h, w, ho, wo, in_div == 1.f ? 1.f : 1.f / in_div);
    PSSR_LAUNCH_CHECK();
    return PSSR_OK;
}

int pssr_avgpool2_pair_div(const float* x, const float* y, float in_div, float* xo, float* yo, int planes, int h, int w, pssr_stream_t s) {
    PSSR_CHECK(x && y && xo && yo && planes > 0 && h > 0 && w > 0 && in_div > 0.f, PSSR_ERR_ARG, "avgpool2_pair: bad args");
    const int ho = (h + 2 * (h & 1) - 2) / 2 + 1, wo = (w + 2 * (w & 1) - 2) / 2 + 1;
    const long total = (long)planes * ho * wo;
    int blocks = (int)((total + 255) / 256); if (blocks > 8192) blocks = 8192;
    hipLaunchKernelGGL(avgpool_kernel, dim3(blocks, 2), dim3(256), 0, (hipStream_t)s, x, xo, y, yo, planes, h, w, ho, wo, in_div == 1.f ? 1.f : 1.f / in_div);
    PSSR_LAUNCH_CHECK();
    return PSSR_OK;
}

int pssr_msssim_weights(const double* sums, int levels, int planes, const double* nvalid, const float* level_weights, int ms,
                        float mix, const double* l1_sum, double l1_numel, const float* grad_out, float* loss_out, float* wts,
                        float* l1_coef, pssr_stream_t s) {
    PSSR_CHECK(sums && nvalid && loss_out && wts && l1_coef && levels > 0 && levels <= 8 && planes > 0, PSSR_ERR_ARG, "msssim_weights: bad args");
    hipLaunchKernelGGL(weights_kernel, dim3(1), dim3(256), 0, (hipStream_t)s, sums, levels, planes, nvalid, level_weights, ms, mix,
                       l1_sum, l1_numel, grad_out, loss_out, wts, l1_coef, 1, 0L, (double*)nullptr);
    PSSR_LAUNCH_CHECK();
    return PSSR_OK;
}

int pssr_msssim_weights_striped(const double* sums, int stripes, int64_t stripe_stride, double* folded, int levels, int planes,
                                const double* nvalid, const float* level_weights, int ms, float mix, const double* l1_sum,
                                double l1_numel, const float* grad_out, float* loss_out, float* wts, float* l1_coef, pssr_stream_t s) {
    PSSR_CHECK(sums && folded && stripes >= 1 && stripe_stride > 0 && nvalid && loss_out && wts && l1_coef && levels > 0 && levels <= 8 && planes > 0,
               PSSR_ERR_ARG, "msssim_weights_striped: bad args");
    hipLaunchKernelGGL(weights_kernel, dim3(1), dim3(256), 0, (hipStream_t)s, sums, levels, planes, nvalid, level_weights, ms, mix,
                       l1_sum, l1_numel, grad_out, loss_out, wts, l1_coef, stripes, (long)stripe_stride, folded);
    PSSR_LAUNCH_CHECK();
    return PSSR_OK;
}

int pssr_ssim_level_bwd(const float* x, const float* y, int planes, int h, int w, const float* win_host, int k, float c1, float c2,
                        const float* wts, int use_ssim, const float* dcoarse, int hc, int wc, const float* l1_coef, float* dx,
                        pssr_stream_t s) {
    PSSR_CHECK(x && y && wts && dx && win_host && planes > 0 && k > 0 && k <= MAXW && (k & 1), PSSR_ERR_ARG, "ssim_level_bwd: bad args");
    const int halo = k - 1, AD = TS + halo, IN = TS + 2 * halo;
    const size_t lds = (size_t)(2 * IN * IN + 5 * IN * AD + 3 * AD * AD) * sizeof(float);
    PSSR_CHECK(lds <= 156 * 1024, PSSR_ERR_UNSUPPORTED, "ssim_level_bwd: window %d needs %zu bytes of LDS", k, lds);
    static bool attr = false;
    if (!attr) {
        (void)hipFuncSetAttribute((const void*)ssim_bwd_kernel, hipFuncAttributeMaxDynamicSharedMemorySize, 160 * 1024 - 4096);
        (void)hipFuncSetAttribute((const void*)ssim_bwd_k<11>, hipFuncAttributeMaxDynamicSharedMemorySize, 160 * 1024 - 4096);
        attr = true;
    }
    if (k == 11)
        hipLaunchKernelGGL(ssim_bwd_k<11>, dim3(cdiv(w, TS), cdiv(h, TS), planes), dim3(256), bwd_lds_k<11>(), (hipStream_t)s, x, y, h, w,
                           make_win(win_host, k), c1, c2, wts, use_ssim, dcoarse, hc, wc, l1_coef, dx);
    else
        hipLaunchKernelGGL(ssim_bwd_kernel, dim3(cdiv(w, TS), cdiv(h, TS), planes), dim3(256), lds, (hipStream_t)s, x, y, h, w,
                           make_win(win_host, k), c1, c2, wts, use_ssim, dcoarse, hc, wc, l1_coef, dx);
    PSSR_LAUNCH_CHECK();
    return PSSR_OK;
}

}
```

### pssr2_amd/engine.py

```python
from __future__ import annotations

import os
from types import SimpleNamespace

import torch

from . import _lib as L
from . import atrous as A
from . import ops

BN_EPS, BN_MOMENTUM = 1e-5, 0.1


def _blocked_order(r: int):
    if r < 1:
        raise ValueError(f"upscaling factor must be a positive integer, got scale={r}")
    l = r.bit_length() - 1
    return (l, False) if (1 << l) == r else (0, True)


_NO_MATERIALISE = os.environ.get("PSSR_MATERIALISE", "0") != "1"
_XCOL_SIDE = os.environ.get("PSSR_XCOL_SIDE", "0") == "1"
_FUSE_DOUT = os.environ.get("PSSR_FUSE_DOUT", "1") != "0"
_OVERWRITE_GRADS = os.environ.get("PSSR_OVERWRITE_GRADS", "1") != "0"
_EVAL_SHUF = os.environ.get("PSSR_EVAL_SHUF", "1") != "0"
_EVAL_AFFINE = os.environ.get("PSSR_EVAL_AFFINE", "1") != "0"
_HEAD_FUSE = os.environ.get("PSSR_HEAD_FUSE", "1") != "0"

FWD, DGRAD = dict(mode=0), dict(mode=1)
FWD_FLAT, DGRAD_FLAT = dict(mode=2), dict(mode=3)
FWD_CENTER, DGRAD_CENTER = dict(mode=2, center=True), dict(mode=3, center=True)


class _Arena:

    def __init__(self):
        self.req = []

    def take(self, n):
        self.req.append(n)
        return len(self.req) - 1

    def build(self, dtype, device):
        offs, tot = [], 0
        for n in self.req:
            offs.append(tot)
            tot += (n + 3) // 4 * 4
        self.buf = torch.zeros(max(tot, 4), dtype=dtype, device=device)
        self.views = [self.buf[o:o + n] for o, n in zip(offs, self.req)]
        return self


class _BNState:
    def __init__(self, c, f32: _Arena, f64: _Arena):
        self.c = c
        self.i32 = [f32.take(c) for _ in range(7)]
        self.i64 = [f64.take(2 * c * ops.STAT_STRIPES) for _ in range(2)]

    def bind(self, f32: _Arena, f64: _Arena):
        self.scale, self.shift, self.mean, self.invstd, self.ca, self.cb, self.cc = (f32.views[i] for i in self.i32)
        self.stats, self.bstats = (f64.views[i] for i in self.i64)
        self.eval_key = None


class _Conv:

    def __init__(self, module, specs, wepoch=None):
        self.m = module
        self.specs = specs
        self.packed = {}
        self.version = {}
        self.wepoch = wepoch if wepoch is not None else [0]

    def ver(self):
        return (self.wepoch[0], self.m.weight._version)

    def weight_for(self, spec):
        w = self.m.weight
        if spec.get("center"):
            w3 = torch.zeros(w.shape[0], w.shape[1], 3, 3, device=w.device, dtype=w.dtype)
            w3[:, :, 1, 1] = w.detach()[:, :, 0, 0]
            return w3
        return w.detach()

    def item(self, name, dtype):
        spec, pw, w = self.specs[name], self.packed[(name, dtype)], self.m.weight
        center = bool(spec.get("center"))
        it = L.PackItem()
        it.w, it.packed = w.data_ptr(), pw.data.data_ptr()
        perm = spec.get("n_perm")
        it.n_perm = perm.data_ptr() if perm is not None else None
        it.cout, it.cin, it.ks = w.shape[0], w.shape[1], 3 if center else w.shape[2]
        it.ci_begin = spec.get("ci_begin", 0)
        it.ci_count = spec.get("ci_count") if spec.get("ci_count") is not None else w.shape[1] - it.ci_begin
        it.mode, it.k_pad, it.n_pad, it.dtype, it.center = spec["mode"], pw.k_pad, pw.n_pad, dtype, int(center)
        return it

    def get(self, name, dtype):
        spec = self.specs[name]
        key = (name, dtype)
        ver = self.ver()
        if self.version.get(key) != ver or key not in self.packed:
            self.packed[key] = ops.pack_conv_weight(self.weight_for(spec).contiguous(), dtype, mode=spec["mode"],
                                                    ci_begin=spec.get("ci_begin", 0), ci_count=spec.get("ci_count"),
                                                    n_perm=spec.get("n_perm"), out=self.packed.get(key))
            self.version[key] = ver
        return self.packed[key]


class Engine:
    _warned_bf16_infer = False
    _QUEUES = ("_folds", "_moves", "_keepalive")

    def __init__(self, model):
        self.model = model
        self.plans = {}
        self.saved = None
        self._convs = {}
        self._built_for = None
        self.cin = self.cout = self.hidden = self.L = self.atrous = self.r = self.blk = self.explicit_shuffle = None
        self.xc = self.h0 = self.pre_perm = self.pre_perm_long = self.pre_specs = None
        self.reducer = None
        self._wepoch = [0]
        self._flat_grad = self._flat_key = self._goffs = self._gsizes = self._gindex = self._gviews = None
        self._overwrite_grads = False
        self.side_wgrad = os.environ.get("PSSR_WGRAD_STREAM", "1") != "0"
        self._side = None
        self._side_on = False
        self._pending = {}
        self._deferred = None
        self._folds, self._moves = [], []
        self._keepalive = []
        self._will_backward = False
        self._fwd_deferred = None
        self._fwd_side = False
        self._wgrad_dma = None
        self._nbt_key = self._nbt_flat = None
        self._fold_cache = {}
        self._shuf_perms = {}
        self._pack_tables = {}
        self._pack_tables_kept = []
        self._eval_steppers = {}
        self.last_train_stepper = None

    def mark_weights_changed(self):
        self._wepoch[0] += 1

    def publish_grads(self):
        if self._flat_grad is None:
            return
        for prm, view in zip(self.model.parameters(), self._gviews):
            if prm.requires_grad and prm.grad is None:
                prm.grad = view

    def _grad_layout(self, device):
        params = list(self.model.parameters())
        key = (str(device), tuple(p.numel() for p in params))
        if self._flat_grad is not None and self._flat_key == key:
            return
        offs, tot = [], 0
        for p in params:
            offs.append(tot)
            tot += (p.numel() + 3) // 4 * 4
        self._flat_grad = torch.zeros(tot, dtype=torch.float32, device=device)
        self._flat_key = key
        self._goffs = offs
        self._gsizes = [p.numel() for p in params]
        self._gindex = {id(p): i for i, p in enumerate(params)}
        self._gviews = [self._flat_grad[o:o + p.numel()].view(p.shape) for p, o in zip(params, offs)]

    def attach_reducer(self, bucket_bytes=64 << 20, group=None):
        from .distributed import GradReducer
        dev = next(self.model.parameters()).device
        self._grad_layout(dev)
        self.reducer = GradReducer(self._flat_grad, self._goffs, self._gsizes, bucket_bytes, group)
        return self.reducer
# ... 254 lines not shown
        p.ones_pre = torch.ones(r2h0, dtype=torch.float32, device=p.device)
        p.zeros_pre = torch.zeros(r2h0, dtype=torch.float32, device=p.device)

    def _plan(self, n, h, w, dt, device):
        key = (n, h, w, dt, str(device))
        p = self.plans.get(key)
        if p is not None:
            return p
        Lv, hid, m = self.L, self.hidden, self.model
        p = self._new_plan(n, h, w, dt, device)
        p.dims = [(h >> i, w >> i) for i in range(Lv)]
        p.cat = [self._buf(p, *p.dims[l], hid[l + 1] // 4 + hid[l]) for l in range(Lv - 1)]
        p.pooled = [self._buf(p, *p.dims[l + 1], hid[l]) for l in range(Lv - 1)]
        p.enc = [self._block_state(p, m.encoder[i], i, hid[i], self.cin if i == 0 else hid[i - 1], out=i == Lv - 1) for i in range(Lv)]
        p.dec = [self._block_state(p, m.decoder[Lv - 2 - l], l, hid[l], hid[l + 1] // 4 + hid[l]) for l in range(Lv - 1)]
        if self.atrous:
            p.xin = self._buf(p, h, w, self.cin)
        self._finish_plan(p, p.enc + p.dec, p.dims[Lv - 1], p.dims[0])
        self.plans[key] = p
        return p

    def _new_bwd_buffers(self, p):
        def per_block():
            return [self._buf(p, *p.dims[i], c) for i, c in enumerate(self.hidden)]
        b = SimpleNamespace(dpre_hr=None, h64=None)
        b.dz, b.dy, b.g = per_block(), per_block(), per_block()
        b.dy2 = per_block() if self.side_wgrad else b.dy
        b.dy3 = per_block() if self.side_wgrad else b.dy
        b.dout = per_block()
        b.dcat = [torch.zeros_like(c) for c in p.cat]
        b.dxcol_b = self._buf(p, p.h, p.w, self.xc)
        r = self.r
        b.g_hr = torch.zeros(p.n, p.h * r, p.w * r, 16, dtype=p.dt, device=p.device)
        b.dpre = torch.zeros_like(p.pre)
        b.sum64 = torch.zeros(ops.STAT_STRIPES * max(16, r * r * self.h0), dtype=torch.float64, device=p.device)
        b.drpool = torch.zeros_like(p.rpool_out) if p.rpool is not None else None
        b.depool = torch.zeros_like(p.epool_out) if p.epool is not None else None
        return b

    def _bwd_buffers(self, p):
        if p.bwd is None:
            b = p.bwd = self._new_bwd_buffers(p)
            b.dpooled = [torch.zeros_like(t) for t in p.pooled]
            b.dxcol_a = self._buf(p, p.h, p.w, self.xc)
        return p.bwd

    def _count_batches(self):
        bns = [mod for mod in self.model.modules() if isinstance(mod, torch.nn.BatchNorm2d) and mod.num_batches_tracked is not None]
        if not bns:
            return
        key = tuple(b.num_batches_tracked.data_ptr() for b in bns)
        if self._nbt_key != key:
            flat = torch.stack([b.num_batches_tracked.detach().reshape(()) for b in bns]).contiguous()
            for i, b in enumerate(bns):
                b.num_batches_tracked.data = flat[i]
            self._nbt_flat = flat
            self._nbt_key = tuple(b.num_batches_tracked.data_ptr() for b in bns)
        self._nbt_flat.add_(1)

    def _sync_world(self):
        if not self.model.sync_bn:
            return 1
        from . import distributed as D
        return D.rank_world()[1]

    def bn_stats_count(self, stats, count):
        world = self._sync_world()
        if world > 1:
            torch.distributed.all_reduce(stats)
        return count * world

    def bn_coefs(self, bstats, count, gamma, mean, invstd, ca, cb, cc, dgamma, dbeta):
        world = self._sync_world()
        if world > 1:
            ops.bn_bwd_coefs(bstats, count, gamma, mean, invstd, ca, cb, cc, dgamma, dbeta)
            torch.distributed.all_reduce(bstats)
            ops.bn_bwd_coefs(bstats, count * world, gamma, mean, invstd, ca, cb, cc, None, None)
        else:
            ops.bn_bwd_coefs(bstats, count, gamma, mean, invstd, ca, cb, cc, dgamma, dbeta)

    def _bn_forward(self, st, bn_module, count, train, stats=None, synced=False):
        if train:
            st.eval_key = None
            stats = st.stats if stats is None else stats
            if not synced:
                count = self.bn_stats_count(stats, count)
            ops.bn_finalize(stats, count, bn_module.weight, bn_module.bias, BN_EPS, BN_MOMENTUM,
                            bn_module.running_mean, bn_module.running_var, st.scale, st.shift, st.mean, st.invstd)
        else:
            ts = (bn_module.weight, bn_module.bias, bn_module.running_mean, bn_module.running_var)
            key = (self._wepoch[0],) + tuple((t.data_ptr(), t._version) for t in ts)
            if st.eval_key != key:
                ops.bn_eval_affine(*ts, BN_EPS, st.scale, st.shift)
                st.eval_key = key

    def _materialise_ok(self, p, c):
        if p.code == L.F32 or c < 8 or (c & (c - 1)) or _NO_MATERIALISE:
            return False
        if self._wgrad_dma is None:
            self._wgrad_dma = L.lib().pssr_get_option(b"WGRAD_DMA") > 0
        return self._wgrad_dma

    def _materialise(self, p, blk, k):
        if blk.act is None:
            blk.act = [torch.zeros_like(blk.y[0]) for _ in range(len(blk.y) - 1)]
        st = blk.bn[k]
        hh, ww = p.dims[blk.level]
        if self._side is None:
            self._side = torch.cuda.Stream(blk.y[0].device)
        self._flush_fwd()
        ev = torch.cuda.Event()
        ev.record(torch.cuda.current_stream())
        n_el, c, code = p.n * hh * ww, blk.c, p.code
        self._fwd_deferred = (ev, lambda: ops.bn_relu_apply(blk.y[k], st.scale, st.shift, blk.act[k], n_el, c, code))

    def _flush_fwd(self):
        d = self._fwd_deferred
        if d is None:
            return
        self._fwd_deferred = None
        ev, fn = d
        with torch.cuda.stream(self._side):
            self._side.wait_event(ev)
            fn()
        self._fwd_side = True

    def _folded_last(self, module, st, conv, code, perm=None):
        cache = self._fold_cache
        rp = module.respass
        key = (self._wepoch[0], conv.weight._version, conv.bias._version, rp.bias._version, st.eval_key)
        ck = (id(conv), code, perm is not None)
        ent = cache.get(ck)
        if ent is None or ent[0] != key:
            with torch.no_grad():
                wf = conv.weight.detach() * st.scale.view(-1, 1, 1, 1)
                bf = torch.addcmul(st.shift, conv.bias.detach(), st.scale).add_(rp.bias.detach())
                if perm is not None:
                    wf, bf = wf[perm], bf[perm]
                wf = wf.contiguous()
            pw = ops.pack_conv_weight(wf, code, mode=0, out=ent[1] if ent is not None else None)
            if ent is not None:
                bf = ent[2].copy_(bf)
            ent = cache[ck] = (key, pw, bf)
        return ent[1], ent[2]

    def _shuf_perm(self, c, device):
        cache = self._shuf_perms
        if (c, device) not in cache:
            idx = torch.arange(c, device=device)
            perm = (idx % (c // 4)) * 4 + idx // (c // 4)
            cache[(c, device)] = (perm, perm.to(torch.int32))
        return cache[(c, device)]

    def _block_forward(self, p, blk, module, src, cin, first, dst, dst_coff, train, shuf=None):
        if blk.a is not None:
            A.ablock_forward(self, blk.a, module, p.xin if first else src, 0, p.n, p.code, dst, dst_coff, train)
            return
        n = p.n
        hh, ww = p.dims[blk.level]
        count = float(n * hh * ww)
        nl = len(blk.y)
        rp = module.respass
        fwd_in, fwd_rp = (FWD_FLAT, FWD_CENTER) if first else (FWD, FWD)
        if not train and p.code != L.F32 and _EVAL_AFFINE and blk.c % 8 == 0:
            for k in range(nl):
                conv, bn = module.conv[3 * k], module.conv[3 * k + 1]
                self._bn_forward(blk.bn[k], bn, count, False)
                spec, inp, icn = (fwd_in, src, cin) if k == 0 else (FWD, blk.y[k - 1], blk.c)
                if k < nl - 1:
                    pw = self._pw(conv, "fwd", p.code, **spec)
                    ops.conv2d(inp, icn, pw, blk.y[k], blk.c, n=n, h=hh, w=ww, bias=conv.bias, flags=L.FLAG_RELU | L.FLAG_AFFINE,
                               aux_scale=blk.bn[k].scale, aux_shift=blk.bn[k].shift)
                    continue
                pwr = self._pw(rp, "fwd", p.code, **fwd_rp)
                if spec is FWD:
                    if shuf is not None and _EVAL_SHUF and blk.c % 32 == 0 and not first:
                        perm_l, perm_i = self._shuf_perm(blk.c, inp.device)
                        pwf, bf = self._folded_last(module, blk.bn[k], conv, p.code, perm_l)
                        pwr = self._pw(rp, "fwd_shuf", p.code, mode=0, n_perm=perm_i)
                        ops.conv2d(inp, icn, pwf, shuf, blk.c, n=n, h=hh, w=ww, out_coff=0, bias=bf, x1=src, cin1=cin, w1=pwr,
                                   flags=L.FLAG_RELU | L.FLAG_SHUF2)
                        return True
                    pwf, bf = self._folded_last(module, blk.bn[k], conv, p.code)
                    ops.conv2d(inp, icn, pwf, dst, blk.c, n=n, h=hh, w=ww, out_coff=dst_coff, bias=bf, x1=src, cin1=cin, w1=pwr,
                               flags=L.FLAG_RELU)
                    return
                pw = self._pw(conv, "fwd", p.code, **spec)
                ops.conv2d(inp, icn, pw, blk.y[k], blk.c, n=n, h=hh, w=ww, bias=conv.bias)
            nl = 0
        for k in range(nl):
            conv = module.conv[3 * k]
            bn = module.conv[3 * k + 1]
            if k == 0:
                pw = self._pw(conv, "fwd", p.code, **fwd_in)
                ops.conv2d(src, cin, pw, blk.y[0], blk.c, n=n, h=hh, w=ww, bias=conv.bias,
                           flags=L.FLAG_STATS if train else 0, stats=blk.bn[0].stats if train else None)
            else:
                pw = self._pw(conv, "fwd", p.code, **FWD)
                prev = blk.bn[k - 1]
                ops.conv2d(blk.y[k - 1], blk.c, pw, blk.y[k], blk.c, n=n, h=hh, w=ww, bias=conv.bias,
                           pro_scale=prev.scale, pro_shift=prev.shift,
                           flags=L.FLAG_STATS if train else 0, stats=blk.bn[k].stats if train else None)
                self._flush_fwd()
            self._bn_forward(blk.bn[k], bn, count, train)
            if train and k < nl - 1 and self._will_backward and self._materialise_ok(p, blk.c):
                self._materialise(p, blk, k)
        pw = self._pw(rp, "fwd", p.code, **fwd_rp)
        last = blk.bn[-1]
        ops.conv2d(src, cin, pw, dst, blk.c, n=n, h=hh, w=ww, out_coff=dst_coff, bias=rp.bias, epilogue=L.EPI_TAIL,
                   aux=blk.y[-1], aux_scale=last.scale, aux_shift=last.shift)

    def _forward_begin(self, x, train):
        m = self.model
        if not x.is_cuda:
            raise RuntimeError(f"pssr2_amd.{type(m).__name__} runs on an MI355X (HIP) device only; there is no CPU fallback")
        x = x.contiguous().float()
        self._structure(x.device)
        n, c, h, w = x.shape
        if c != self.cin:
            raise ValueError(f"expected {self.cin} input channels, got {c}")
        dt = self.storage_dtype(train)
        code = ops.dtype_code(dt)
        self._check_supported(code, h, w, train)
        p = self._plan(n, h, w, dt, x.device)
        self._repack_all(code)
        if train:
            p.f64.buf.zero_()
            self._count_batches()
        if self.atrous:
            p.bn_in.scale.fill_(1.0), p.bn_in.shift.zero_()
            if p.xin is not None:
                ops.input_plain(x, p.xin, code)
        else:
            if train:
                ops.channel_stats_nchw(x, p.bn_in.stats, 1 / 128, -1.0)
            self._bn_forward(p.bn_in, m.norm, float(n * h * w), train)
        ops.input_im2col(x, p.xcol, p.bn_in.scale, p.bn_in.shift, code)
        return x, p

    def forward(self, x, train):
        m = self.model
        x, p = self._forward_begin(x, train)
        n, code = p.n, p.code
        Lv, hid = self.L, self.hidden
        for i in range(Lv):
            blk = p.enc[i]
            src, cin = (p.xcol, self.xc) if i == 0 else (p.pooled[i - 1], ops.pad_to(hid[i - 1], 16))
            if i < Lv - 1:
                dst, off = p.cat[i], hid[i + 1] // 4
            else:
                dst, off = blk.out, 0
            shuffled = self._block_forward(p, blk, m.encoder[i], src, cin, i == 0, dst, off, train,
                                           shuf=p.cat[Lv - 2] if (i == Lv - 1 and Lv > 1 and p.epool is None and not train) else None)
            if i < Lv - 1:
                ops.maxpool2(dst, p.pooled[i], n, *p.dims[i], hid[i], code, in_coff=off)
        deep = p.enc[Lv - 1].out
        if p.epool is not None:
            A.psp_forward(self, p.epool, m.encoder_pool, deep, 0, n, code, p.epool_out, 0, train)
            deep = p.epool_out
        for l in range(Lv - 2, -1, -1):
            prev = deep if l == Lv - 2 else p.dec[l + 1].out
            if not shuffled:
                ops.pixel_shuffle(prev, p.cat[l], n, *p.dims[l + 1], hid[l + 1] // 4, 2, code)
            blk = p.dec[l]
            shuffled = self._block_forward(p, blk, m.decoder[Lv - 2 - l], p.cat[l], p.cat[l].shape[-1], False, blk.out, 0, train,
                                           shuf=p.cat[l - 1] if (l > 0 and not train) else None)
        feat = p.dec[0].out if Lv > 1 else deep
        if p.rpool is not None:
            A.psp_forward(self, p.rpool, m.reconstruction_pool, feat, 0, n, code, p.rpool_out, 0, train)
            feat = p.rpool_out
        out = self._head_forward(p, feat, x, train)
        self._flush_fwd()
        self.saved = (p, x) if train else None
        return out

    def _head_forward(self, p, feat, x, train=True):
        rec = self.model.reconstruction
        n, h, w, code, h0, r = p.n, p.h, p.w, p.code, self.h0, self.r
        pw0, pw1 = self._pw_pre("fwd0", code), self._pw_pre("fwd1", code)
        p.pre_bias = rec.pre.bias.detach()[self.pre_perm_long].contiguous()
        out = torch.empty(n, self.cout, h * r, w * r, dtype=torch.float32, device=x.device)
        if _HEAD_FUSE and ops.head_q_supported(code, h0, self.cout, r, h, w):
            if p.head_q is None:
                p.head_q = torch.empty(9, r * r, n, h, w, dtype=torch.float32, device=x.device)
            if train:
                ops.conv2d(feat, h0, pw0, p.pre, r * r * h0, n=n, h=h, w=w, bias=p.pre_bias, x1=p.xcol, cin1=self.xc,
                           w1=pw1, flags=L.FLAG_RELU | L.FLAG_HEADQ, head_w=rec.conv.weight, head_q=p.head_q)
            else:
                ops.conv2d(feat, h0, pw0, p.head_q, r * r * h0, n=n, h=h, w=w, bias=p.pre_bias, x1=p.xcol, cin1=self.xc,
                           w1=pw1, epilogue=L.EPI_HEADQ, head_w=rec.conv.weight, head_q=p.head_q)
            ops.head_q_gather(p.head_q, rec.conv.bias, out, n, h, w, 128.0, 128.0)
            return out
        ops.conv2d(feat, h0, pw0, p.pre, r * r * h0, n=n, h=h, w=w, bias=p.pre_bias, x1=p.xcol, cin1=self.xc, w1=pw1, flags=L.FLAG_RELU)
        pre_hr = self._pre_hr(p)
        if self.explicit_shuffle:
            ops.pixel_shuffle(p.pre, pre_hr, n, h, w, h0, r, code)
        if ops.head_conv_supported(code, h0, self.cout):
            ops.head_conv_fwd(pre_hr, self.blk, rec.conv.weight, rec.conv.bias, out, n, h * r, w * r, h0, self.cout, 128.0, 128.0, code)
        else:
            ops.conv2d(pre_hr, h0, self._pw(rec.conv, "fwd", code, **FWD), out, self.cout, n=n, h=h * r, w=w * r, bias=rec.conv.bias,
                       epilogue=L.EPI_FINAL, in0_blk=self.blk, out_scale=128.0, out_shift=128.0)
        return out

    def _pw_pre(self, name, code):
        return self._pw(self.model.reconstruction.pre, name, code, **self.pre_specs[name])

    def _rows_head(self, code):
        return ops.head_conv_supported(code, self.h0, self.cout) and not self.explicit_shuffle and self.blk <= 2 and self.h0 in (32, 64, 128)

    def _pre_hr(self, p):
        n, h, w, r, h0 = p.n, p.h, p.w, self.r, self.h0
        if not self.explicit_shuffle:
            return p.pre.view(n, h * r, w * r, h0)
        if p.pre_hr is None:
            p.pre_hr = torch.zeros(n, h * r, w * r, h0, dtype=p.pre.dtype, device=p.pre.device)
        return p.pre_hr

    def _head_backward(self, p, bw, grads, dout, feat, dfeat):
        rec = self.model.reconstruction
        n, h, w, code, h0, r = p.n, p.h, p.w, p.code, self.h0, self.r
        dev = dout.device
        H, W = h * r, w * r
        dout = dout.contiguous().float()
        pre_hr = self._pre_hr(p)
        if self.explicit_shuffle:
            if bw.dpre_hr is None:
                bw.dpre_hr = torch.zeros_like(pre_hr)
            dpre_hr = bw.dpre_hr
        else:
            dpre_hr = bw.dpre.view(n, H, W, h0)
        if ops.head_conv_supported(code, h0, self.cout):
            gw = grads[id(rec.conv.weight)] = self._gbuf(rec.conv.weight)
            gb = torch.empty(2 * self.cout, dtype=torch.float32, device=dev)
            grads[id(rec.conv.bias)] = gb[:self.cout]
            gpb = torch.empty(r * r * h0, dtype=torch.float32, device=dev) if self._rows_head(code) else None
            if gpb is not None:
                S = ops.STAT_STRIPES
                sizes = (S * 2 * self.cout, S * gw.numel(), S * gpb.numel())
                if bw.h64 is None or bw.h64.numel() != sum(sizes):
                    bw.h64 = torch.zeros(sum(sizes), dtype=torch.float64, device=dev)
                else:
                    bw.h64.zero_()
                s_out, dw64, s_pre = torch.split(bw.h64, sizes)
                ops.channel_stats_nchw(dout, s_out, 128.0, 0.0)
                ops.head_conv_bwd_rows(dout, 128.0, rec.conv.weight, pre_hr, dpre_hr, self.blk, dw64, s_pre, n, H, W, h0, self.cout, code)
                ops.f64_to_f32_batch([(s_out, gb, False), (dw64, gw.view(-1), False), (s_pre, gpb, False)])
            else:
                bw.sum64.zero_()
                ops.channel_stats_nchw(dout, bw.sum64, 128.0, 0.0)
                ops.f64_to_f32(bw.sum64[:ops.STAT_STRIPES * 2 * self.cout], gb)
                ops.head_conv_wgrad(dout, 128.0, pre_hr, self.blk, gw, n, H, W, h0, self.cout, code)
                ops.head_conv_dgrad(dout, 128.0, rec.conv.weight, pre_hr, dpre_hr, self.blk, n, H, W, h0, self.cout, code)
        else:
            gpb = None
            ops.nchw_to_nhwc(dout, bw.g_hr, 128.0, code)
            bw.sum64.zero_()
            ops.channel_sum_nhwc(bw.g_hr, n * H * W, 16, bw.sum64, code)
            gb = torch.empty(16, dtype=torch.float32, device=dev)
            ops.f64_to_f32(bw.sum64, gb)
            grads[id(rec.conv.bias)] = gb[:self.cout]
            self._wgrad(p, grads, rec.conv, bw.g_hr, 16, pre_hr, h0, 9, in_blk=self.blk, hh=H, ww=W)
            ops.conv2d(bw.g_hr, 16, self._pw(rec.conv, "dgrad", code, **DGRAD), dpre_hr, h0, n=n, h=H, w=W, epilogue=L.EPI_DGRAD_MASK,
                       aux=pre_hr, aux_scale=p.ones_pre, aux_shift=p.zeros_pre, out_blk=self.blk, aux_blk=self.blk)
        cpre_n = r * r * h0
        if self.explicit_shuffle:
            ops.pixel_shuffle(bw.dpre, dpre_hr, n, h, w, h0, r, code, inverse=True)
        if gpb is None:
            bw.sum64.zero_()
            ops.channel_sum_nhwc(bw.dpre, n * h * w, cpre_n, bw.sum64, code)
            gpb = torch.empty(cpre_n, dtype=torch.float32, device=dev)
            ops.f64_to_f32(bw.sum64, gpb)
        gb_pre = torch.empty_like(gpb)
        gb_pre[self.pre_perm_long] = gpb
        grads[id(rec.pre.bias)] = gb_pre
        self._wgrad(p, grads, rec.pre, bw.dpre, cpre_n, feat, h0, 9, mode=0, ci_begin=0, ci_count=h0, n_perm=self.pre_perm, hh=h, ww=w)
        self._wgrad(p, grads, rec.pre, bw.dpre, cpre_n, p.xcol, self.xc, 1, mode=2, ci_begin=h0, ci_count=self.cin, n_perm=self.pre_perm, hh=h, ww=w)
        self._ready(grads, list(rec.parameters()))
        ops.conv2d(bw.dpre, cpre_n, self._pw_pre("dgrad0", code), dfeat, h0, n=n, h=h, w=w)
        if not self.atrous:
            pw1 = self._pw_pre("dgrad1", code)

            def dgrad_x():
                ops.conv2d(bw.dpre, cpre_n, pw1, bw.dxcol_b, self.xc, n=n, h=h, w=w)
            if self._side_on and _XCOL_SIDE:
                self._on_side([bw.dpre, bw.dxcol_b], dgrad_x)
            else:
                dgrad_x()

    @staticmethod
    def _wgrad_rows(cout, code):
        esz = 4 if code == L.F32 else 2
        return cout if (cout * esz) % 16 == 0 else ops.pad_to(cout, 16)

    def _wgrad1x1(self, grads, conv_module, dy, cout, dy_coff, src, cin_pad, n, hh, ww, code, *, side, mode=0, pro=None, src_coff=0,
                  gelu_in=False, first=None):
        rows = self._wgrad_rows(cout, code)
        assert rows == cout or dy_coff == 0
        slot = grads[id(conv_module.weight)] = self._gbuf(conv_module.weight)

        def run():
            if first is not None:
                first()
            parts = ops.conv2d_wgrad_parts(dy, rows, src, cin_pad, 1, n=n, h=hh, w=ww, dtype=code, dy_coff=dy_coff, in_coff=src_coff, gelu_in=gelu_in,
                                           pro_scale=pro.scale if pro is not None else None, pro_shift=pro.shift if pro is not None else None)
            ops.unpack_conv_wgrad(parts, slot, mode=mode, k_pad=cin_pad, accumulate=True)
        if side and self._side_on:
            self._on_side([dy], run)
        else:
            run()

    def _wgrad(self, p, grads, conv_module, dy, cout, src, cin_pad, taps, *, mode=0, ci_begin=0, ci_count=None,
               n_perm=None, pro=None, dy_blk=0, in_blk=0, hh, ww, center=False, dy_view_c=None):
        code = p.code
        co_eff = self._wgrad_rows(cout, code)
        w = conv_module.weight
        gname = id(w)

        def parts():
            return ops.conv2d_wgrad_parts(dy, co_eff, src, cin_pad, taps, n=p.n, h=hh, w=ww, dtype=code, dy_blk=dy_blk, in_blk=in_blk,
# ... 156 lines not shown
```

### pssr2_amd/ops.py

```python
from __future__ import annotations

import ctypes as C

import torch

from . import _lib as L

TORCH_DTYPE = {L.F32: torch.float32, L.BF16: torch.bfloat16, L.F16: torch.float16}


def dtype_code(dt: torch.dtype) -> int:
    if dt == torch.float32:
        return L.F32
    if dt == torch.bfloat16:
        return L.BF16
    if dt == torch.float16:
        return L.F16
    raise ValueError(f"unsupported compute dtype {dt}; use torch.float32, torch.bfloat16 or torch.float16")


def pad_to(v: int, m: int) -> int:
    return (v + m - 1) // m * m


class PackedWeight:
    __slots__ = ("data", "taps", "k_pad", "n_pad", "dtype")

    def __init__(self, data, taps, k_pad, n_pad, dtype):
        self.data, self.taps, self.k_pad, self.n_pad, self.dtype = data, taps, k_pad, n_pad, dtype


def pack_conv_weight(w: torch.Tensor, dtype: int, mode: int = 0, ci_begin: int = 0, ci_count: int | None = None,
                     n_perm: torch.Tensor | None = None, out: PackedWeight | None = None) -> PackedWeight:
    assert w.is_cuda and w.dtype == torch.float32 and w.is_contiguous() and w.dim() == 4
    cout, cin, ks, _ = w.shape
    ci_count = cin - ci_begin if ci_count is None else ci_count
    s2dk = ks * ks * pad_to(cin, 16)
    gk = ci_count if mode == 0 else cout if mode in (1, 3, 5) else s2dk if mode == 4 else ci_count * ks * ks
    gn = ci_count if mode == 1 else ci_count * ks * ks if mode == 3 else s2dk if mode == 5 else cout
    taps = 1 if mode >= 2 else ks * ks
    k_pad, n_pad = pad_to(gk, 16), pad_to(gn, 128)
    if out is None:
        nbytes = L.lib().pssr_packed_weight_bytes(taps, k_pad, n_pad, dtype)
        out = PackedWeight(torch.empty(nbytes, dtype=torch.uint8, device=w.device), taps, k_pad, n_pad, dtype)
    L.check(L.lib().pssr_pack_conv_weight(L.ptr(w), L.ptr(out.data), cout, cin, ks, ci_begin, ci_count, mode,
                                          L.ptr(n_perm), k_pad, n_pad, dtype, L.stream_ptr()), "pssr_pack_conv_weight")
    return out


SOLO = [False]


def conv2d(x, cin0, w0: PackedWeight, out, cout, *, n, h, w, in0_coff=0, out_coff=0, bias=None,
           x1=None, cin1=0, w1: PackedWeight | None = None, in1_coff=0,
           pro_scale=None, pro_shift=None, epilogue=L.EPI_STORE, flags=0,
           aux=None, aux_coff=0, aux_scale=None, aux_shift=None, aux_mean=None, aux_invstd=None, stats=None,
           in0_blk=0, out_blk=0, aux_blk=0, out_scale=1.0, out_shift=0.0, gelu_in=False, head_w=None, head_q=None):
    d = L.ConvDesc()
    d.dtype = w0.dtype
    d.n, d.h, d.w = n, h, w
    d.in0, d.in0_cstride, d.in0_coff, d.cin0, d.taps0, d.w0 = L.ptr(x), x.shape[-1], in0_coff, cin0, w0.taps, L.ptr(w0.data)
    if w1 is not None:
        d.in1, d.in1_cstride, d.in1_coff, d.cin1, d.taps1, d.w1 = L.ptr(x1), x1.shape[-1], in1_coff, cin1, w1.taps, L.ptr(w1.data)
        assert w1.n_pad == w0.n_pad and w1.dtype == w0.dtype
    d.prologue = L.PRO_GELU if gelu_in else L.PRO_BN_RELU if pro_scale is not None else L.PRO_NONE
    d.pro_scale, d.pro_shift = L.ptr(pro_scale), L.ptr(pro_shift)
    d.out, d.out_cstride, d.out_coff, d.cout, d.n_pad = L.ptr(out), out.shape[-1], out_coff, cout, w0.n_pad
    d.bias = L.ptr(bias)
    d.epilogue, d.flags = epilogue, flags | (L.FLAG_SOLO if SOLO[0] else 0)
    if aux is not None:
        d.aux, d.aux_cstride, d.aux_coff = L.ptr(aux), aux.shape[-1], aux_coff
    d.aux_scale, d.aux_shift, d.aux_mean, d.aux_invstd = L.ptr(aux_scale), L.ptr(aux_shift), L.ptr(aux_mean), L.ptr(aux_invstd)
    d.stats = L.ptr(stats)
    d.in0_blk, d.out_blk, d.aux_blk, d.out_scale, d.out_shift = in0_blk, out_blk, aux_blk, out_scale, out_shift
    if epilogue == L.EPI_FINAL:
        d.out_cstride, d.out_coff = cout, 0
    if epilogue == L.EPI_HEADQ:
        d.out_cstride, d.out_coff = cout, 0
    if epilogue == L.EPI_HEADQ or flags & L.FLAG_HEADQ:
        d.head_w, d.head_q = L.ptr(head_w), L.ptr(head_q)
    ws_bytes = L.lib().pssr_conv2d_workspace_bytes(C.byref(d))
    if ws_bytes > 0:
        ws = torch.empty(ws_bytes, dtype=torch.uint8, device=out.device)
        d.workspace, d.workspace_bytes = L.ptr(ws), ws_bytes
    L.check(L.lib().pssr_conv2d(C.byref(d), L.stream_ptr()), "pssr_conv2d")
    return out


def _wgrad_desc(dy, cout, x, cin_pad, taps, *, n, h, w, dtype, dy_coff=0, in_coff=0, dy_blk=0, in_blk=0, pro_scale=None, pro_shift=None,
                gelu_in=False):
    d = L.WgradDesc()
    d.dtype, d.n, d.h, d.w = dtype, n, h, w
    d.dy, d.dy_cstride, d.dy_coff, d.dy_blk, d.cout = L.ptr(dy), dy.shape[-1], dy_coff, dy_blk, cout
    d.in_, d.in_cstride, d.in_coff, d.in_blk, d.cin_pad = L.ptr(x), x.shape[-1], in_coff, in_blk, cin_pad
    d.taps = taps
    d.prologue = L.PRO_GELU if gelu_in else L.PRO_BN_RELU if pro_scale is not None else L.PRO_NONE
    d.pro_scale, d.pro_shift = L.ptr(pro_scale), L.ptr(pro_shift)
    return d


def conv2d_wgrad(dy, cout, x, cin_pad, taps, dw, **kw):
    d = _wgrad_desc(dy, cout, x, cin_pad, taps, **kw)
    d.dw, d.dw_parts = L.ptr(dw), 0
    L.check(L.lib().pssr_conv2d_wgrad(C.byref(d), L.stream_ptr()), "pssr_conv2d_wgrad")
    return dw


def conv2d_wgrad_parts(dy, cout, x, cin_pad, taps, **kw):
    d = _wgrad_desc(dy, cout, x, cin_pad, taps, **kw)
    parts = L.lib().pssr_conv2d_wgrad_parts(C.byref(d))
    if parts <= 0:
        L.check(parts if parts < 0 else -1, "pssr_conv2d_wgrad_parts")
    dw = torch.empty(parts, cout, taps, cin_pad, dtype=torch.float32, device=dy.device)
    d.dw, d.dw_parts = L.ptr(dw), parts
    L.check(L.lib().pssr_conv2d_wgrad(C.byref(d), L.stream_ptr()), "pssr_conv2d_wgrad")
    return dw


def unpack_conv_wgrad(dw_packed, dw_oihw, *, mode=0, ci_begin=0, ci_count=None, n_perm=None, k_pad, accumulate=False):
    cout, cin, ks, _ = dw_oihw.shape
    ci_count = cin - ci_begin if ci_count is None else ci_count
    parts, rows = (dw_packed.shape[0], dw_packed.shape[1]) if dw_packed.dim() == 4 else (1, dw_packed.shape[0])
    L.check(L.lib().pssr_unpack_conv_wgrad_parts(L.ptr(dw_packed), parts, rows, L.ptr(dw_oihw), cout, cin, ks, ci_begin, ci_count, mode,
                                                 L.ptr(n_perm), k_pad, int(accumulate), L.stream_ptr()), "pssr_unpack_conv_wgrad_parts")
    return dw_oihw


def _ref(t, coff=0):
    return L.ptr(t), t.shape[-1], coff


def channel_stats_nchw(x, stats, pre_scale=1.0, pre_shift=0.0):
    n, c, h, w = x.shape
    L.check(L.lib().pssr_channel_stats_nchw(L.ptr(x), n, c, C.c_int64(h * w), C.c_float(pre_scale), C.c_float(pre_shift),
                                            L.ptr(stats), L.stream_ptr()), "pssr_channel_stats_nchw")


def bn_finalize(stats, count, gamma, beta, eps, momentum, running_mean, running_var, scale, shift, mean, invstd):
    c = scale.numel()
    L.check(L.lib().pssr_bn_finalize(L.ptr(stats), C.c_double(count), L.ptr(gamma), L.ptr(beta), C.c_float(eps), C.c_float(momentum),
                                     L.ptr(running_mean), L.ptr(running_var), L.ptr(scale), L.ptr(shift), L.ptr(mean), L.ptr(invstd),
                                     c, L.stream_ptr()), "pssr_bn_finalize")


def bn_eval_affine(gamma, beta, running_mean, running_var, eps, scale, shift):
    L.check(L.lib().pssr_bn_eval_affine(L.ptr(gamma), L.ptr(beta), L.ptr(running_mean), L.ptr(running_var), C.c_float(eps),
                                        L.ptr(scale), L.ptr(shift), scale.numel(), L.stream_ptr()), "pssr_bn_eval_affine")


def bn_bwd_coefs(stats, count, gamma, mean, invstd, coef_a, coef_b, coef_c, dgamma, dbeta):
    L.check(L.lib().pssr_bn_bwd_coefs(L.ptr(stats), C.c_double(count), L.ptr(gamma), L.ptr(mean), L.ptr(invstd), L.ptr(coef_a),
                                      L.ptr(coef_b), L.ptr(coef_c), L.ptr(dgamma), L.ptr(dbeta), coef_a.numel(), L.stream_ptr()),
            "pssr_bn_bwd_coefs")


def bn_bwd_apply(g, y, coef_a, coef_b, coef_c, dy, npix, c, dtype, g_coff=0, y_coff=0, dy_coff=0):
    L.check(L.lib().pssr_bn_bwd_apply(*_ref(g, g_coff), *_ref(y, y_coff), L.ptr(coef_a), L.ptr(coef_b), L.ptr(coef_c),
                                      *_ref(dy, dy_coff), C.c_int64(npix), c, dtype, L.stream_ptr()), "pssr_bn_bwd_apply")


def bn_relu_apply(y, scale, shift, a, npix, c, dtype, y_coff=0, a_coff=0):
    L.check(L.lib().pssr_bn_relu_apply(L.ptr(y), y.shape[-1], y_coff, L.ptr(scale), L.ptr(shift), L.ptr(a), a.shape[-1], a_coff, C.c_int64(npix), c, dtype,
                                       L.stream_ptr()), "pssr_bn_relu_apply")


def input_im2col(x, xcol, scale, shift, dtype, pre_scale=1 / 128, pre_shift=-1.0):
    n, c, h, w = x.shape
    L.check(L.lib().pssr_input_im2col(L.ptr(x), L.ptr(xcol), n, c, h, w, xcol.shape[-1], C.c_float(pre_scale), C.c_float(pre_shift),
                                      L.ptr(scale), L.ptr(shift), dtype, L.stream_ptr()), "pssr_input_im2col")


def input_norm_bwd(dxcol_a, dxcol_b, x, mean, invstd, stats, dtype, pre_scale=1 / 128, pre_shift=-1.0):
    n, c, h, w = x.shape
    L.check(L.lib().pssr_input_norm_bwd(L.ptr(dxcol_a), L.ptr(dxcol_b), dxcol_a.shape[-1], L.ptr(x), C.c_float(pre_scale),
                                        C.c_float(pre_shift), L.ptr(mean), L.ptr(invstd), n, c, h, w, L.ptr(stats), dtype,
                                        L.stream_ptr()), "pssr_input_norm_bwd")


def maxpool2(x, out, n, h, w, c, dtype, in_coff=0, out_coff=0):
    L.check(L.lib().pssr_maxpool2(*_ref(x, in_coff), *_ref(out, out_coff), n, h, w, c, dtype, L.stream_ptr()), "pssr_maxpool2")


def maxpool2_bwd(act, dpool, dskip, dout, n, h, w, c, dtype, act_coff=0, dskip_coff=0):
    ds = _ref(dskip, dskip_coff) if dskip is not None else (None, 0, 0)
    L.check(L.lib().pssr_maxpool2_bwd(*_ref(act, act_coff), *_ref(dpool), *ds, *_ref(dout), n, h, w, c, dtype, L.stream_ptr()),
            "pssr_maxpool2_bwd")


def pixel_shuffle(lo, hi, n, h, w, c_hi, r, dtype, lo_coff=0, hi_coff=0, inverse=False):
    L.check(L.lib().pssr_pixel_shuffle(*_ref(lo, lo_coff), *_ref(hi, hi_coff), n, h, w, c_hi, r, int(inverse), dtype,
                                       L.stream_ptr()), "pssr_pixel_shuffle")


def relu_bwd_stats(dout, out, y, mean, invstd, dz, stats, npix, c, dtype, out_coff=0):
    L.check(L.lib().pssr_relu_bwd_stats(*_ref(dout), *_ref(out, out_coff), *_ref(y), L.ptr(mean), L.ptr(invstd), *_ref(dz),
                                        L.ptr(stats), C.c_int64(npix), c, dtype, L.stream_ptr()), "pssr_relu_bwd_stats")


def relu_bwd_stats_fused_ok(dtype, c, h=2, w=2, unshuffle=False):
    return dtype != L.F32 and (c & (c - 1)) == 0 and c >= (32 if unshuffle else 8) and (unshuffle or (h % 2 == 0 and w % 2 == 0))


def relu_bwd_stats_pool(dpool, dskip, dskip_coff, out, out_coff, y, mean, invstd, dz, stats, n, h, w, c, dtype):
    L.check(L.lib().pssr_relu_bwd_stats_pool(*_ref(dpool), *_ref(dskip, dskip_coff), *_ref(out, out_coff), *_ref(y), L.ptr(mean), L.ptr(invstd),
                                             *_ref(dz), L.ptr(stats), n, h, w, c, dtype, L.stream_ptr()), "pssr_relu_bwd_stats_pool")


def relu_bwd_stats_unshuffle(dhi, out, out_coff, y, mean, invstd, dz, stats, n, h, w, c, dtype):
    L.check(L.lib().pssr_relu_bwd_stats_unshuffle(*_ref(dhi), *_ref(out, out_coff), *_ref(y), L.ptr(mean), L.ptr(invstd), *_ref(dz), L.ptr(stats),
                                                  n, h, w, c, dtype, L.stream_ptr()), "pssr_relu_bwd_stats_unshuffle")


def channel_sum_nhwc(x, npix, c, out, dtype, coff=0, cstride=None):
    cs = x.shape[-1] if cstride is None else cstride
    L.check(L.lib().pssr_channel_sum_nhwc(L.ptr(x), cs, coff, C.c_int64(npix), c, L.ptr(out), dtype, L.stream_ptr()),
            "pssr_channel_sum_nhwc")


def nchw_to_nhwc(x, out, scale, dtype):
    n, c, h, w = x.shape
    L.check(L.lib().pssr_nchw_to_nhwc(L.ptr(x), L.ptr(out), n, c, C.c_int64(h * w), out.shape[-1], C.c_float(scale), dtype,
                                      L.stream_ptr()), "pssr_nchw_to_nhwc")


def clip_u8(x, out):
    L.check(L.lib().pssr_clip_u8(L.ptr(x), L.ptr(out), C.c_int64(x.numel()), L.stream_ptr()), "pssr_clip_u8")


STAT_STRIPES = 64


def f64_to_f32(src, dst, accumulate=False, stripes=STAT_STRIPES):
    L.check(L.lib().pssr_f64_to_f32(L.ptr(src), L.ptr(dst), dst.numel(), int(accumulate), stripes, L.stream_ptr()), "pssr_f64_to_f32")


def f64_to_f32_batch(items, stripes=STAT_STRIPES):
    for k in range(0, len(items), L.COPY_BATCH_MAX):
        chunk = items[k:k + L.COPY_BATCH_MAX]
        fb = L.FoldBatch()
        for i, (src, dst, acc) in enumerate(chunk):
            if src.dtype != torch.float64 or dst.dtype != torch.float32 or src.numel() < stripes * dst.numel() or not (src.is_contiguous() and dst.is_contiguous()):
                raise ValueError("f64_to_f32_batch needs contiguous float64 [stripes * n] sources and float32 [n] destinations")
            fb.dst[i], fb.src[i], fb.n[i], fb.accumulate[i] = dst.data_ptr(), src.data_ptr(), dst.numel(), int(acc)
        L.check(L.lib().pssr_f64_to_f32_batch(C.byref(fb), len(chunk), stripes, L.stream_ptr()), "pssr_f64_to_f32_batch")


def _win(win):
    arr = (C.c_float * len(win))(*[float(v) for v in win])
    return arr, len(win)


def ssim_level_fwd(x, y, planes, h, w, win, c1, c2, sums, l1_sum=None):
    arr, k = _win(win)
    L.check(L.lib().pssr_ssim_level_fwd(L.ptr(x), L.ptr(y), planes, h, w, arr, k, C.c_float(c1), C.c_float(c2), L.ptr(sums),
                                        L.ptr(l1_sum), L.stream_ptr()), "pssr_ssim_level_fwd")


def ssim_level_fwd_adj(x, y, planes, h, w, win, c1, c2, use_ssim, sums, l1_sum, stripes, stripe_stride, adj, in_div=1.0):
    k = len(win); arr = (C.c_float * k)(*win)
    L.check(L.lib().pssr_ssim_level_fwd_adj(L.ptr(x), L.ptr(y), C.c_float(in_div), planes, h, w, arr, k, C.c_float(c1), C.c_float(c2), int(use_ssim), L.ptr(sums),
                                            L.ptr(l1_sum), stripes, C.c_int64(stripe_stride), L.ptr(adj), L.stream_ptr()), "pssr_ssim_level_fwd_adj")


def msssim_weights_striped(sums, stripes, stripe_stride, folded, levels, planes, nvalid, level_weights, ms, mix, l1_sum, l1_numel, grad_out,
                           loss_out, wts, l1_coef):
    L.check(L.lib().pssr_msssim_weights_striped(L.ptr(sums), stripes, C.c_int64(stripe_stride), L.ptr(folded), levels, planes, L.ptr(nvalid),
                                                L.ptr(level_weights), int(ms), C.c_float(mix), L.ptr(l1_sum), C.c_double(l1_numel),
                                                L.ptr(grad_out), L.ptr(loss_out), L.ptr(wts), L.ptr(l1_coef), L.stream_ptr()),
            "pssr_msssim_weights_striped")


def ssim_level_bwd_adj(x, y, adj, planes, h, w, win, wts, dcoarse, hc, wc, l1_coef, dx, in_div=1.0):
    k = len(win); arr = (C.c_float * k)(*win)
    L.check(L.lib().pssr_ssim_level_bwd_adj(L.ptr(x), L.ptr(y), C.c_float(in_div), L.ptr(adj), planes, h, w, arr, k, L.ptr(wts), L.ptr(dcoarse), hc, wc,
                                            L.ptr(l1_coef), L.ptr(dx), L.stream_ptr()), "pssr_ssim_level_bwd_adj")


def avgpool2_planes(x, out, planes, h, w, in_div=1.0):
    L.check(L.lib().pssr_avgpool2_planes_div(L.ptr(x), C.c_float(in_div), L.ptr(out), planes, h, w, L.stream_ptr()), "pssr_avgpool2_planes_div")


def avgpool2_pair(x, y, xo, yo, planes, h, w, in_div=1.0):
    L.check(L.lib().pssr_avgpool2_pair_div(L.ptr(x), L.ptr(y), C.c_float(in_div), L.ptr(xo), L.ptr(yo), planes, h, w, L.stream_ptr()),
            "pssr_avgpool2_pair_div")


def msssim_weights(sums, levels, planes, nvalid, level_weights, ms, mix, l1_sum, l1_numel, grad_out, loss_out, wts, l1_coef):
    L.check(L.lib().pssr_msssim_weights(L.ptr(sums), levels, planes, L.ptr(nvalid), L.ptr(level_weights), int(ms), C.c_float(mix),
                                        L.ptr(l1_sum), C.c_double(l1_numel), L.ptr(grad_out), L.ptr(loss_out), L.ptr(wts),
                                        L.ptr(l1_coef), L.stream_ptr()), "pssr_msssim_weights")


def ssim_level_bwd(x, y, planes, h, w, win, c1, c2, wts, use_ssim, dcoarse, hc, wc, l1_coef, dx):
    arr, k = _win(win)
    L.check(L.lib().pssr_ssim_level_bwd(L.ptr(x), L.ptr(y), planes, h, w, arr, k, C.c_float(c1), C.c_float(c2), L.ptr(wts),
                                        int(use_ssim), L.ptr(dcoarse), hc, wc, L.ptr(l1_coef), L.ptr(dx), L.stream_ptr()),
            "pssr_ssim_level_bwd")


def adamw_step(p, g, m, v, lr, beta1, beta2, eps, weight_decay, step, grad_scale=1.0):
    L.check(L.lib().pssr_adamw_step(L.ptr(p), L.ptr(g), L.ptr(m), L.ptr(v), C.c_int64(p.numel()), C.c_float(lr), C.c_float(beta1),
                                    C.c_float(beta2), C.c_float(eps), C.c_float(weight_decay), C.c_int64(step), C.c_float(grad_scale),
                                    L.stream_ptr()), "pssr_adamw_step")


ROUND_CLIP, CLIP = 2, 1


def bilinear_down_u8(hr, h, w):
    assert hr.dtype == torch.uint8 and hr.is_cuda and hr.is_contiguous()
    H, W = hr.shape[-2:]
    planes = hr.numel() // (H * W)
    tmp = torch.empty(planes * H * w, dtype=torch.uint8, device=hr.device)
    lr = torch.empty(*hr.shape[:-2], h, w, dtype=torch.uint8, device=hr.device)
    L.check(L.lib().pssr_bilinear_down_u8(L.ptr(hr), L.ptr(tmp), L.ptr(lr), planes, H, W, h, w, L.stream_ptr()), "pssr_bilinear_down_u8")
    return lr


def u8_to_f32(x):
    out = torch.empty(x.shape, dtype=torch.float32, device=x.device)
    L.check(L.lib().pssr_u8_to_f32(L.ptr(x), L.ptr(out), C.c_int64(x.numel()), L.stream_ptr()), "pssr_u8_to_f32")
    return out


def crappify_gaussian(x, intensity, gain, spread, seed, tile_offset, flags, noise=None, out=None, tile_counter=None):
    out = torch.empty_like(x) if out is None else out
    tiles = x.shape[0]
    L.check(L.lib().pssr_crappify_gaussian(L.ptr(x), L.ptr(out), tiles, C.c_int64(x.numel() // tiles), C.c_float(intensity), C.c_float(gain),
                                           C.c_float(spread), C.c_uint64(seed), C.c_uint64(tile_offset), L.ptr(noise), flags,
                                           L.ptr(tile_counter), L.stream_ptr()), "pssr_crappify_gaussian")
    return out


def crappify_poisson(x, intensity, gain, spread, seed, tile_offset, flags, out=None, tile_counter=None):
    out = torch.empty_like(x) if out is None else out
    tiles = x.shape[0]
    L.check(L.lib().pssr_crappify_poisson(L.ptr(x), L.ptr(out), tiles, C.c_int64(x.numel() // tiles), C.c_float(intensity), C.c_float(gain),
                                          C.c_float(spread), C.c_uint64(seed), C.c_uint64(tile_offset), flags, L.ptr(tile_counter),
                                          L.stream_ptr()), "pssr_crappify_poisson")
    return out


def crappify_poisson_samples(x, samples, intensity, gain, flags, out=None):
    out = torch.empty_like(x) if out is None else out
    if samples.dtype != torch.float64 or samples.numel() != x.numel():
        raise ValueError("samples: float64, one per element of x")
    L.check(L.lib().pssr_crappify_poisson_samples(L.ptr(x), L.ptr(samples.contiguous()), L.ptr(out), C.c_int64(x.numel()), C.c_double(intensity),
                                                  C.c_double(gain), flags, L.stream_ptr()), "pssr_crappify_poisson_samples")
    return out


def gaussian_blur(x, sigma, gain, flags):
    h, w = x.shape[-2:]
    planes = x.numel() // (h * w)
    tmp, out = torch.empty_like(x), torch.empty_like(x)
    L.check(L.lib().pssr_gaussian_blur(L.ptr(x), L.ptr(tmp), L.ptr(out), planes, h, w, C.c_float(sigma), C.c_float(gain), flags,
                                       L.stream_ptr()), "pssr_gaussian_blur")
    return out


def counter_add(counter, inc):
    L.check(L.lib().pssr_counter_add(L.ptr(counter), C.c_uint64(inc), L.stream_ptr()), "pssr_counter_add")


def adamw_step_dev(p, g, m, v, state, beta1, beta2, eps, weight_decay, grad_scale=1.0):
    L.check(L.lib().pssr_adamw_step_dev(L.ptr(p), L.ptr(g), L.ptr(m), L.ptr(v), C.c_int64(p.numel()), L.ptr(state), C.c_float(beta1),
                                        C.c_float(beta2), C.c_float(eps), C.c_float(weight_decay), C.c_float(grad_scale),
                                        L.stream_ptr()), "pssr_adamw_step_dev")


def amp_check(g, amp):
    L.check(L.lib().pssr_amp_check(L.ptr(g), C.c_int64(g.numel()), L.ptr(amp), L.stream_ptr()), "pssr_amp_check")


def adamw_step_amp(p, g, m, v, state, beta1, beta2, eps, weight_decay, amp, growth, backoff, interval, grad_scale=1.0):
    L.check(L.lib().pssr_adamw_step_amp(L.ptr(p), L.ptr(g), L.ptr(m), L.ptr(v), C.c_int64(p.numel()), L.ptr(state), C.c_float(beta1),
                                        C.c_float(beta2), C.c_float(eps), C.c_float(weight_decay), C.c_float(grad_scale), L.ptr(amp),
                                        C.c_float(growth), C.c_float(backoff), int(interval), L.stream_ptr()), "pssr_adamw_step_amp")


def input_patchify(x, xpatch, scale, shift, patch, dtype, pre_scale=1 / 128, pre_shift=-1.0):
    n, c, h, w = x.shape
    L.check(L.lib().pssr_input_patchify(L.ptr(x), L.ptr(xpatch), n, c, h, w, patch, xpatch.shape[-1], C.c_float(pre_scale),
                                        C.c_float(pre_shift), L.ptr(scale), L.ptr(shift), dtype, L.stream_ptr()), "pssr_input_patchify")


def input_norm_bwd2(dxcol_a, dxcol_b, dpatch, patch, x, mean, invstd, stats, dtype, pre_scale=1 / 128, pre_shift=-1.0):
    n, c, h, w = x.shape
    col = dxcol_a if dxcol_a is not None else dxcol_b
    L.check(L.lib().pssr_input_norm_bwd2(L.ptr(dxcol_a), L.ptr(dxcol_b), col.shape[-1] if col is not None else 0, L.ptr(dpatch),
                                         dpatch.shape[-1] if dpatch is not None else 0, patch, L.ptr(x), C.c_float(pre_scale),
                                         C.c_float(pre_shift), L.ptr(mean), L.ptr(invstd), n, c, h, w, L.ptr(stats), dtype,
                                         L.stream_ptr()), "pssr_input_norm_bwd2")


def dwconv7_pack_batch(items):
    for k in range(0, len(items), L.DWPACK_BATCH_MAX):
        chunk = items[k:k + L.DWPACK_BATCH_MAX]
        b = L.DwPackBatch()
        for i, (w, out, flip) in enumerate(chunk):
            c = w.shape[0]
            if w.dtype != torch.float32 or out.dtype != torch.float32 or not (w.is_contiguous() and out.is_contiguous()) or w.numel() != 49 * c \
                    or out.numel() < 49 * c:
                raise ValueError("dwconv7_pack_batch needs contiguous float32 [C,1,7,7] weights and [49, C] destinations")
            b.w[i], b.packed[i], b.c[i], b.flip[i] = w.data_ptr(), out.data_ptr(), c, int(flip)
        L.check(L.lib().pssr_dwconv7_pack_batch(C.byref(b), len(chunk), L.stream_ptr()), "pssr_dwconv7_pack_batch")


def dwconv7_pack(w, out, flip=False):
    c = w.shape[0]
    L.check(L.lib().pssr_dwconv7_pack(L.ptr(w), L.ptr(out), c, int(flip), L.stream_ptr()), "pssr_dwconv7_pack")
    return out


# ... 468 lines not shown
```

### pssr2_amd/util.py

```python
from __future__ import annotations

import inspect
import math

import numpy as np
import torch
import torch.nn as nn

from . import ops

MS_WEIGHTS = (0.0448, 0.2856, 0.3001, 0.2363, 0.1333)


def _gauss_1d(size: int, sigma: float):
    coords = torch.arange(size, dtype=torch.float) - size // 2
    g = torch.exp(-(coords ** 2) / (2 * sigma ** 2))
    return (g / g.sum()).tolist()


_CONST_CACHE = {}


class _SSIMLossFunction(torch.autograd.Function):
    @staticmethod
    def forward(ctx, x, y, cfg, in_div=1.0):
        if not x.is_cuda:
            raise RuntimeError("pssr2_amd.SSIMLoss runs on an MI355X (HIP) device only; there is no CPU fallback")
        win, mix, ms, k1, k2, data_range, lvl_w = cfg
        x = x.detach().contiguous().float()
        y = y.detach().contiguous().float()
        n, c, h, w = x.shape
        planes, k = n * c, len(win)
        levels = len(lvl_w) if ms else 1
        if ms and min(h, w) <= (k - 1) * 2 ** 4:
            raise AssertionError(f"Image size should be larger than {(k - 1) * 2 ** 4} due to the 4 downsamplings in ms-ssim")
        c1, c2 = (k1 * data_range) ** 2, (k2 * data_range) ** 2
        dev = x.device
        fused_div = in_div != 1.0 and k == 11 and ctx.needs_input_grad[0]
        if in_div != 1.0 and not fused_div:
            x, y = x / in_div, y / in_div
        div0 = in_div if fused_div else 1.0
        xs, ys, dims = [x], [y], [(h, w)]
        for lv in range(1, levels):
            hh, ww = dims[-1]
            ho, wo = (hh + 2 * (hh & 1) - 2) // 2 + 1, (ww + 2 * (ww & 1) - 2) // 2 + 1
            xo = torch.empty(planes, ho, wo, device=dev)
            yo = torch.empty(planes, ho, wo, device=dev)
            ops.avgpool2_pair(xs[-1], ys[-1], xo, yo, planes, hh, ww, div0 if lv == 1 else 1.0)
            xs.append(xo), ys.append(yo), dims.append((ho, wo))
        adjs = None
        if k == 11 and ctx.needs_input_grad[0]:
            adjs = [torch.empty(planes * 3 * hh * ww, device=dev) for hh, ww in dims]
        stripes = 16 if adjs is not None else 1
        sstride = levels * planes * 2 + 2
        rows = 2 * stripes if stripes > 1 else 1
        sums = torch.zeros(rows * sstride + (sstride if stripes > 1 else 0), dtype=torch.float64, device=dev)
        l1_sum = sums[sstride - 2:sstride - 1] if mix < 1 else None
        for l in range(levels):
            hh, ww = dims[l]
            if adjs is not None:
                ops.ssim_level_fwd_adj(xs[l], ys[l], planes, hh, ww, win, c1, c2, l == levels - 1, sums[l * planes * 2:],
                                       l1_sum if l == 0 else None, stripes, sstride, adjs[l], div0 if l == 0 else 1.0)
            else:
                ops.ssim_level_fwd(xs[l], ys[l], planes, hh, ww, win, c1, c2, sums[l * planes * 2:], l1_sum if l == 0 else None)
        ckey = (tuple(dims), k, tuple(lvl_w) if ms else (1.0,), str(dev))
        cached = _CONST_CACHE.get(ckey)
        if cached is None:
            cached = _CONST_CACHE[ckey] = (
                torch.tensor([float((hh - k + 1) * (ww - k + 1)) for hh, ww in dims], dtype=torch.float64, device=dev),
                torch.tensor(list(lvl_w) if ms else [1.0], dtype=torch.float32, device=dev))
        nvalid, lw = cached
        loss = torch.empty(1, dtype=torch.float32, device=dev)
        wts = torch.empty(levels * planes, dtype=torch.float32, device=dev)
        l1c = torch.empty(1, dtype=torch.float32, device=dev)
        if stripes > 1:
            ops.msssim_weights_striped(sums, stripes, sstride, sums[rows * sstride:], levels, planes, nvalid, lw, ms, mix, l1_sum, float(x.numel()),
                                       None, loss, wts, l1c)
            sums = sums[rows * sstride:]
            l1_sum = sums[levels * planes * 2:levels * planes * 2 + 1] if l1_sum is not None else None
        else:
            ops.msssim_weights(sums, levels, planes, nvalid, lw, ms, mix, l1_sum, float(x.numel()), None, loss, wts, l1c)
        ctx.saved = (xs, ys, dims, sums, nvalid, lw, l1_sum, cfg, planes, x.shape, adjs, div0, in_div if not fused_div else 1.0)
        return loss[0]

    @staticmethod
    def backward(ctx, grad_out):
        xs, ys, dims, sums, nvalid, lw, l1_sum, cfg, planes, shape, adjs, div0, post_div = ctx.saved
        win, mix, ms, k1, k2, data_range, lvl_w = cfg
        levels = len(xs)
        dev = xs[0].device
        c1, c2 = (k1 * data_range) ** 2, (k2 * data_range) ** 2
        go = grad_out.detach().float().reshape(1).contiguous()
        loss = torch.empty(1, dtype=torch.float32, device=dev)
        wts = torch.empty(levels * planes, dtype=torch.float32, device=dev)
        l1c = torch.empty(1, dtype=torch.float32, device=dev)
        ops.msssim_weights(sums, levels, planes, nvalid, lw, ms, mix, l1_sum, float(xs[0].numel()), go, loss, wts, l1c)
        dcoarse, hc, wc = None, 0, 0
        for l in range(levels - 1, -1, -1):
            hh, ww = dims[l]
            dx = torch.empty(planes, hh, ww, device=dev)
            use_ssim = (l == levels - 1)
            l1_arg = l1c if (l == 0 and l1_sum is not None) else None
            if adjs is not None:
                ops.ssim_level_bwd_adj(xs[l], ys[l], adjs[l], planes, hh, ww, win, wts[l * planes:], dcoarse, hc, wc, l1_arg, dx,
                                       div0 if l == 0 else 1.0)
            else:
                ops.ssim_level_bwd(xs[l], ys[l], planes, hh, ww, win, c1, c2, wts[l * planes:], use_ssim, dcoarse, hc, wc, l1_arg, dx)
            dcoarse, hc, wc = dx, hh, ww
        g = dcoarse.view(shape)
        if post_div != 1.0:
            g = g / post_div
        return g, None, None, None


class SSIMLoss(nn.Module):
    def __init__(self, channels: int = 1, mix: float = .8, win_size: int = 11, win_sigma: float = 1.5, ms: bool = True, kwargs=None):
        super().__init__()
        kwargs = {} if kwargs is None else dict(kwargs)
        if win_size % 2 != 1:
            raise ValueError("Window size should be odd.")
        self.K = tuple(kwargs.pop("K", (0.01, 0.03)))
        self.weights = tuple(kwargs.pop("weights", None) or MS_WEIGHTS)
        if kwargs:
            raise TypeError(f"unsupported pytorch_msssim options on the MI355X path: {sorted(kwargs)}")
        self.win = _gauss_1d(win_size, win_sigma)
        self.channels, self.win_size, self.mix, self.ms = channels, win_size, mix, ms

    def forward(self, input, target):
        if input.shape != target.shape:
            raise ValueError(f"Input images should have the same dimensions, but got {input.shape} and {target.shape}.")
        cfg = (self.win, float(self.mix), bool(self.ms), self.K[0], self.K[1], 1.0, self.weights)
        return _SSIMLossFunction.apply(input, target, cfg)

    def forward_divided(self, input, target, divisor: float):
        if input.shape != target.shape:
            raise ValueError(f"Input images should have the same dimensions, but got {input.shape} and {target.shape}.")
        cfg = (self.win, float(self.mix), bool(self.ms), self.K[0], self.K[1], 1.0, self.weights)
        return _SSIMLossFunction.apply(input, target, cfg, float(divisor))


class _FnCtx:

    def __init__(self, needs_input_grad):
        self.needs_input_grad = needs_input_grad


class _CrappifierLossFunction(torch.autograd.Function):

    @staticmethod
    def forward(ctx, lr, lr_hat, ds_hr, hist_cfg, ssim_cfg, clamp=False):
        if not (lr.is_cuda and lr_hat.is_cuda and ds_hr.is_cuda):
            raise RuntimeError("pssr2_amd crappifier loss runs on an MI355X (HIP) device only; there is no CPU fallback")
        if not (lr.shape == lr_hat.shape == ds_hr.shape):
            raise ValueError(f"lr, lr_hat and ds_hr must have one shape, got {tuple(lr.shape)}, {tuple(lr_hat.shape)}, {tuple(ds_hr.shape)}")
        lr, lr_hat, ds_hr = (t.detach().contiguous().float() for t in (lr, lr_hat, ds_hr))
        bins, lo, hi, sigma = hist_cfg
        pred, target = torch.empty_like(lr_hat), torch.empty_like(lr)
        ops.crappifier_profiles(lr_hat, lr, ds_hr, pred, target, clamp)
        hp, ht = ops.gradhist_fwd([(pred, None), (target, None)], bins, lo, hi, sigma)
        sctx = _FnCtx((ctx.needs_input_grad[1], False, False, False))
        p_loss = _SSIMLossFunction.forward(sctx, pred, target, ssim_cfg)
        parts = torch.empty(3, dtype=torch.float32, device=lr.device)
        batch, w_lr = lr.shape[0], lr.shape[-1]
        ops.crappifier_loss_combine(hp, ht, p_loss, 1.0 / (batch * bins) / (w_lr * w_lr), parts)
        ctx.state = (lr_hat, ds_hr, hp, ht, parts, sctx, hist_cfg, bool(clamp), batch, w_lr)
        return parts[0]

    @staticmethod
    def backward(ctx, grad_out):
        lr_hat, ds_hr, hp, ht, parts, sctx, (bins, lo, hi, sigma), clamp, batch, w_lr = ctx.state
        go = grad_out.detach().float().reshape(1).contiguous()
        sc = torch.empty(2, dtype=torch.float32, device=go.device)
        ops.crappifier_loss_bwd_scalars(parts, go, sc)
        g = _SSIMLossFunction.backward(sctx, sc[0:1])[0]
        ops.gradhist_bwd(lr_hat, ds_hr, hp, g, bins, lo, hi, sigma, g_ref=ht, dev_scale=sc[1:2], g_scale=2.0 / (batch * bins * w_lr * w_lr),
                         clamp=clamp, accumulate=True)
        return None, g, None, None, None, None


def ssim(X, Y, data_range=255, win_size=11, win_sigma=1.5):
    cfg = (_gauss_1d(win_size, win_sigma), 1.0, False, 0.01, 0.03, float(data_range), (1.0,))
    with torch.no_grad():
        return 1 - _SSIMLossFunction.apply(X, Y, cfg)


def pixel_metric(mse: float, image_range: int = 255):
    return math.sqrt(mse) * image_range


def _psnr_metric(mse):
    return 20 * torch.log10(1 / torch.sqrt(mse))


def _force_list(item):
    if type(item) is not list:
        try:
            return list(item)
        except TypeError:
            return [item]
    return item


def _get_callbacks(raw):
    callbacks = [] if raw is None else _force_list(raw)
    takes_locals = [len([a for a in inspect.getfullargspec(cb).args if a != "self"]) == 1 for cb in callbacks]
    return callbacks, takes_locals


def _patch_images(batched, n_cols, n_rows, overlap, margin):
    size = batched.shape[-1]
    step = size - overlap
    H, W = n_rows * step + overlap, n_cols * step + overlap
    acc, cnt = np.zeros((H, W)), np.zeros((H, W))
    for idx in range(n_rows * n_cols):
        row, col = divmod(idx, n_cols)
# ... 87 lines not shown
```

Measured before the change: 2406.

## Fuse maxpool and pixel-shuffle into conv tail epilogue, avgpool into SSIM forward

Adds an optional second output to the conv tail epilogue. It writes either a 2x2 max-pooled copy or a pixel-shuffled copy of the tile, so the separate maxpool2 and pixel_shuffle launches can be skipped. The shuffle fusion is now also used during training. The SSIM forward kernel with adjoint can now emit the next level's 2x2 average-pooled x/y from its shared-memory tile, which removes separate avgpool_pair launches and a reread of the pyramid level. The trade-off is extra epilogue work, with a __syncthreads and a re-read of just-written output, plus a larger descriptor that needs an ABI check.

```diff
diff --git a/include/pssr_mi355.h b/include/pssr_mi355.h
--- a/include/pssr_mi355.h
+++ b/include/pssr_mi355.h
@@ -59,6 +59,8 @@
     PSSR_FLAG_SOLO = 32,
     PSSR_FLAG_SHUF2 = 16
 };
+
+enum { PSSR_OUT2_NONE = 0, PSSR_OUT2_POOL2 = 1, PSSR_OUT2_SHUFFLE2 = 2 };
 
 typedef struct pssr_conv_desc {
     int32_t dtype;
@@ -81,7 +83,10 @@
     float out_scale, out_shift;
     void* workspace; int64_t workspace_bytes;
     const float* head_w; float* head_q;
+    void* out2; int32_t out2_cstride, out2_coff, out2_kind, reserved0;
 } pssr_conv_desc;
+
+int pssr_conv_desc_bytes(void);
 
 int pssr_conv2d(const pssr_conv_desc* desc, pssr_stream_t stream);
 int64_t pssr_conv2d_workspace_bytes(const pssr_conv_desc* desc);
@@ -179,6 +184,9 @@
 int pssr_ssim_level_fwd_adj(const float* x, const float* y, float in_div, int planes, int h, int w, const float* win_host, int k,
                             float c1, float c2, int use_ssim, double* sums, double* l1_sum, int stripes, int64_t stripe_stride,
                             float* adj, pssr_stream_t stream);
+int pssr_ssim_level_fwd_adj_pool(const float* x, const float* y, float in_div, int planes, int h, int w, const float* win_host, int k,
+                                 float c1, float c2, int use_ssim, double* sums, double* l1_sum, int stripes, int64_t stripe_stride,
+                                 float* adj, float* xo, float* yo, pssr_stream_t stream);
 int pssr_msssim_weights_striped(const double* sums, int stripes, int64_t stripe_stride, double* folded, int levels, int planes,
                                 const double* nvalid, const float* level_weights, int ms, float mix, const double* l1_sum,
                                 double l1_numel, const float* grad_out, float* loss_out, float* wts, float* l1_coef,
diff --git a/pssr2_amd/_lib.py b/pssr2_amd/_lib.py
--- a/pssr2_amd/_lib.py
+++ b/pssr2_amd/_lib.py
@@ -11,6 +11,8 @@
 PRO_NONE, PRO_BN_RELU, PRO_GELU = 0, 1, 2
 EPI_STORE, EPI_TAIL, EPI_DGRAD_MASK, EPI_FINAL, EPI_DGRAD_GELU, EPI_HEADQ = 0, 1, 2, 3, 4, 5
 FLAG_RELU, FLAG_STATS, FLAG_AFFINE, FLAG_HEADQ, FLAG_SHUF2, FLAG_SOLO = 1, 2, 4, 8, 16, 32
+OUT2_NONE, OUT2_POOL2, OUT2_SHUFFLE2 = 0, 1, 2
+ABI_VERSION = 5
 
 c_void_p, c_int, c_i64, c_float = C.c_void_p, C.c_int, C.c_int64, C.c_float
 
@@ -33,6 +35,7 @@
         ("out_scale", C.c_float), ("out_shift", C.c_float),
         ("workspace", c_void_p), ("workspace_bytes", C.c_int64),
         ("head_w", c_void_p), ("head_q", c_void_p),
+        ("out2", c_void_p), ("out2_cstride", C.c_int32), ("out2_coff", C.c_int32), ("out2_kind", C.c_int32), ("reserved0", C.c_int32),
     ]
 
 
@@ -89,6 +92,16 @@
                 ("mode", C.c_int32), ("k_pad", C.c_int32), ("n_pad", C.c_int32), ("dtype", C.c_int32), ("center", C.c_int32)]
 
 
+def _check_abi(handle):
+    version = handle.pssr_abi_version()
+    desc_bytes = handle.pssr_conv_desc_bytes() if hasattr(handle, "pssr_conv_desc_bytes") else None
+    if version != ABI_VERSION or desc_bytes != C.sizeof(ConvDesc):
+        raise RuntimeError(
+            f"{_LIB_PATH} does not match this package: it reports ABI version {version} and a {desc_bytes}-byte pssr_conv_desc, the Python "
+            f"mirrors are written for version {ABI_VERSION} and {C.sizeof(ConvDesc)} bytes.  Rebuild it (make -C pssr2_amd/csrc).")
+    return handle
+
+
 def lib():
     global _lib
     if _lib is None:
@@ -97,7 +110,7 @@
                 f"{_LIB_PATH} not found: build the HIP extension first (python -c 'import __graft_entry__ as g; g.build()' "
                 "or make -C pssr2_amd/csrc). pssr2_amd has no CPU fallback.")
         import torch
-        _lib = C.CDLL(str(_LIB_PATH))
+        _lib = _check_abi(C.CDLL(str(_LIB_PATH)))
         _lib.pssr_last_error.restype = C.c_char_p
         _lib.pssr_packed_weight_bytes.restype = C.c_int64
         _lib.pssr_conv2d_workspace_bytes.restype = C.c_int64
diff --git a/pssr2_amd/csrc/conv_igemm.hip b/pssr2_amd/csrc/conv_igemm.hip
--- a/pssr2_amd/csrc/conv_igemm.hip
+++ b/pssr2_amd/csrc/conv_igemm.hip
@@ -8,6 +8,8 @@
 }
 
 static int conv2d_entry(const pssr_conv_desc* d, pssr_stream_t stream, long* query_ws);
+
+extern "C" int pssr_conv_desc_bytes(void) { return (int)sizeof(pssr_conv_desc); }
 
 #ifdef PSSR_V3_STAMPS
 static unsigned* g_stamp_buf = nullptr;
@@ -102,6 +104,18 @@
     a.epi8 = esz == 2 && d->epilogue != PSSR_EPI_FINAL && d->cout % 8 == 0 && d->out_coff % 8 == 0 && d->out_cstride % 8 == 0 &&
              (d->epilogue == PSSR_EPI_STORE || d->epilogue == PSSR_EPI_HEADQ || (d->aux_coff % 8 == 0 && d->aux_cstride % 8 == 0));
     if (!pssr_tunables().conv_epi8) a.epi8 = 0;
+    a.out2 = nullptr; a.out2_cs = a.out2_co = 0; a.out2_kind = PSSR_OUT2_NONE;
+    if (d->out2_kind != PSSR_OUT2_NONE) {
+        const bool pool = d->out2_kind == PSSR_OUT2_POOL2;
+        PSSR_CHECK((pool || d->out2_kind == PSSR_OUT2_SHUFFLE2) && d->epilogue == PSSR_EPI_TAIL && (query_ws || d->out2), PSSR_ERR_ARG,
+                   "conv2d: out2_kind=%d goes with EPI_TAIL and an out2 buffer", d->out2_kind);
+        PSSR_CHECK(d->out2_coff >= 0 && d->out2_coff + (pool ? d->cout : d->cout / 4) <= d->out2_cstride, PSSR_ERR_ARG, "conv2d: out2 stride/offset");
+        PSSR_CHECK(a.epi8 && d->out_blk == 0 && d->out2_cstride % 8 == 0 && d->out2_coff % 8 == 0, PSSR_ERR_UNSUPPORTED,
+                   "conv2d: a second output needs 16-bit storage, plain pixel order and 8-channel aligned slices");
+        PSSR_CHECK(pool ? (d->h % 2 == 0 && d->w % 2 == 0) : d->cout % 32 == 0, PSSR_ERR_UNSUPPORTED,
+                   "conv2d: POOL2 needs even h and w, SHUFFLE2 cout %% 32 == 0");
+        a.out2 = d->out2; a.out2_cs = d->out2_cstride; a.out2_co = d->out2_coff; a.out2_kind = d->out2_kind;
+    }
     a.dbg = pssr_tunables().igemm_dbg;
     a.stamps = nullptr;
 #ifdef PSSR_V3_STAMPS
diff --git a/pssr2_amd/csrc/conv_igemm_args.h b/pssr2_amd/csrc/conv_igemm_args.h
--- a/pssr2_amd/csrc/conv_igemm_args.h
+++ b/pssr2_amd/csrc/conv_igemm_args.h
@@ -22,6 +22,7 @@
     int dbg;
     int ksplit; float* ws;
     const float* head_w; float* head_q;
+    void* out2; int out2_cs, out2_co, out2_kind;
 };
 
 int launch_bf16(const ConvArgs& a, hipStream_t s);
diff --git a/pssr2_amd/csrc/conv_igemm_impl.h b/pssr2_amd/csrc/conv_igemm_impl.h
--- a/pssr2_amd/csrc/conv_igemm_impl.h
+++ b/pssr2_amd/csrc/conv_igemm_impl.h
@@ -180,6 +180,58 @@
     }
 }
 
+struct TailOut2 { const void* out; void* out2; int N, H, W, cout, out_cs, out_co, out2_cs, out2_co, out2_kind; };
+
+template <typename T, int BN, class C>
+__device__ __attribute__((noinline)) void conv_tail_out2(const TailOut2 p, int tid, int x0, int y0, int img0, int n0) {
+    using X = TT<T>;
+    static_assert(sizeof(T) == 2, "16-bit storage");
+    __syncthreads();
+    const T* src = (const T*)p.out + p.out_co;
+    if (p.out2_kind == PSSR_OUT2_POOL2) {
+        if constexpr (C::TWL >= 1 && C::THL >= 1) {
+            constexpr int CG = BN / 8, PWL = C::TWL - 1, PHL = C::THL - 1;
+            constexpr int ITEMS = (C::MP / 4) * CG;
+            const int HO = p.H >> 1, WO = p.W >> 1;
+            const long xstep = p.out_cs, ystep = (long)p.W * p.out_cs;
+            for (int it = tid; it < ITEMS; it += 256) {
+                const int c8 = it % CG, pp = it / CG;
+                const int px = pp & ((1 << PWL) - 1), py = (pp >> PWL) & ((1 << PHL) - 1), img = pp >> (PWL + PHL);
+                const int gi = img0 + img, oy = (y0 >> 1) + py, ox = (x0 >> 1) + px, nb = n0 + c8 * 8;
+                if (!(gi < p.N && oy < HO && ox < WO && nb < p.cout)) continue;
+                const T* s0 = src + (((long)gi * p.H + 2 * oy) * p.W + 2 * ox) * p.out_cs + nb;
+                float a[8], b[8], c[8], d[8], m[8];
+                X::unpack(*(const u32x4*)s0, a); X::unpack(*(const u32x4*)(s0 + xstep), b);
+                X::unpack(*(const u32x4*)(s0 + ystep), c); X::unpack(*(const u32x4*)(s0 + ystep + xstep), d);
+#pragma unroll
+                for (int e = 0; e < 8; ++e) m[e] = fmaxf(fmaxf(a[e], b[e]), fmaxf(c[e], d[e]));
+                *(u32x4*)((T*)p.out2 + (((long)gi * HO + oy) * WO + ox) * p.out2_cs + p.out2_co + nb) = X::pack(m);
+            }
+        }
+    } else {
+        constexpr int G = BN / 32;
+        constexpr int ITEMS = C::MP * G;
+        for (int it = tid; it < ITEMS; it += 256) {
+            const int g = it % G, m = it / G;
+            const int tx = m & (C::TW - 1), ty = (m >> C::TWL) & (C::TH - 1), img = m >> (C::TWL + C::THL);
+            const int gi = img0 + img, gy = y0 + ty, gx = x0 + tx, nb = n0 + g * 32;
+            if (!(gi < p.N && gy < p.H && gx < p.W && nb < p.cout)) continue;
+            const unsigned short* lop = (const unsigned short*)src + (((long)gi * p.H + gy) * p.W + gx) * p.out_cs + nb;
+            unsigned short e[32];
+#pragma unroll
+            for (int q = 0; q < 4; ++q) *(u32x4*)(e + 8 * q) = *(const u32x4*)(lop + 8 * q);
+#pragma unroll
+            for (int k = 0; k < 4; ++k) {
+                const long phi = ((long)gi * 2 * p.H + 2 * gy + (k >> 1)) * (2L * p.W) + 2 * gx + (k & 1);
+                unsigned short v[8];
+#pragma unroll
+                for (int cc = 0; cc < 8; ++cc) v[cc] = e[4 * cc + k];
+                *(u32x4*)((unsigned short*)p.out2 + phi * p.out2_cs + p.out2_co + (nb >> 2)) = *(const u32x4*)v;
+            }
+        }
+    }
+}
+
 template <typename T, int BN, class C, int EPI, bool STATS, bool TR = false, bool AFF = false>
 __device__ __forceinline__ void conv_epilogue8(const ConvArgs& p, f32x16 (&acc)[C::MI][C::NJ], char* smem, int tid, int x0, int y0, int img0, int n0) {
     static_assert(!AFF || (EPI == PSSR_EPI_STORE && !STATS), "FLAG_AFFINE: EPI_STORE without statistics");
@@ -324,6 +376,11 @@
             stat_add(st + n0 + tid, lo, t1);
             stat_add(st + p.cout + n0 + tid, lo, t2);
         }
+    }
+    if constexpr (EPI == PSSR_EPI_TAIL) {
+        if (p.out2_kind)
+            conv_tail_out2<T, BN, C>(TailOut2{p.out, p.out2, p.N, p.H, p.W, p.cout, p.out_cs, p.out_co, p.out2_cs, p.out2_co, p.out2_kind},
+                                     tid, x0, y0, img0, n0);
     }
 }
 
diff --git a/pssr2_amd/csrc/loss.hip b/pssr2_amd/csrc/loss.hip
--- a/pssr2_amd/csrc/loss.hip
+++ b/pssr2_amd/csrc/loss.hip
@@ -399,7 +399,8 @@
 template <int K>
 __global__ __launch_bounds__(256) void ssim_fwd_adj_k(const float* __restrict__ X, const float* __restrict__ Y, int H, int W,
                                                       Win win, float C1, float C2, double* sums, double* l1_sum, int stripes, long stripe_stride,
-                                                      float* __restrict__ adj, int use_ssim, float in_mul) {
+                                                      float* __restrict__ adj, int use_ssim, float in_mul,
+                                                      float* __restrict__ xo, float* __restrict__ yo) {
     constexpr int halo = K - 1, IN = TS + halo, SEG = 8, NS = TS / SEG;
     constexpr int HPW = TS + 1;
     extern __shared__ float lds[];
@@ -421,6 +422,20 @@
         xs[i] = xv; ys[i] = yv;
     }
     __syncthreads();
+    if (xo) {
+        const int HO = H >> 1, WO = W >> 1;
+        const int pr = tid / (TS / 2), pc = tid % (TS / 2);
+        const int py = (oy0 >> 1) + pr, px = (ox0 >> 1) + pc;
+        if (py < HO && px < WO) {
+            const float* a = xs + 2 * pr * IN + 2 * pc;
+            const float* b = ys + 2 * pr * IN + 2 * pc;
+            float sa = 0.f, sb = 0.f;
+            sa += a[0]; sa += a[1]; sa += a[IN]; sa += a[IN + 1];
+            sb += b[0]; sb += b[1]; sb += b[IN]; sb += b[IN + 1];
+            const long o = ((long)plane * HO + py) * WO + px;
+            xo[o] = 0.25f * sa; yo[o] = 0.25f * sb;
+        }
+    }
     if (l1_sum) {
         constexpr int r5 = K / 2;
         float wsum = 0.f;
@@ -822,19 +837,36 @@
     return PSSR_OK;
 }
 
-int pssr_ssim_level_fwd_adj(const float* x, const float* y, float in_div, int planes, int h, int w, const float* win_host, int k, float c1,
-                            float c2, int use_ssim, double* sums, double* l1_sum, int stripes, int64_t stripe_stride, float* adj,
-                            pssr_stream_t s) {
+static int ssim_level_fwd_adj_launch(const float* x, const float* y, float in_div, int planes, int h, int w, const float* win_host, int k, float c1,
+                                     float c2, int use_ssim, double* sums, double* l1_sum, int stripes, int64_t stripe_stride, float* adj,
+                                     float* xo, float* yo, pssr_stream_t s) {
     PSSR_CHECK(x && y && sums && win_host && planes > 0 && adj && k == 11, PSSR_ERR_ARG,
                "ssim_level_fwd_adj: needs the adjoint buffer and the 11-tap window (k=%d)", k);
     PSSR_CHECK(h >= k && w >= k && stripes >= 1 && (stripes == 1 || stripe_stride > 0) && in_div > 0.f, PSSR_ERR_ARG, "ssim_level_fwd_adj: bad size / stripes / in_div");
     const int IN = TS + k - 1;
     const size_t lds = (size_t)(2 * IN * IN + IN * (TS + 1)) * sizeof(float);
-    const int eh = l1_sum ? h : h - k + 1, ew = l1_sum ? w : w - k + 1;
+    const bool whole = l1_sum || xo;
+    const int eh = whole ? h : h - k + 1, ew = whole ? w : w - k + 1;
     hipLaunchKernelGGL(ssim_fwd_adj_k<11>, dim3(cdiv(ew, TS), cdiv(eh, TS), planes), dim3(256), lds, (hipStream_t)s, x, y, h, w,
-                       make_win(win_host, k), c1, c2, sums, l1_sum, stripes, (long)stripe_stride, adj, use_ssim, in_div == 1.f ? 1.f : 1.f / in_div);
+                       make_win(win_host, k), c1, c2, sums, l1_sum, stripes, (long)stripe_stride, adj, use_ssim, in_div == 1.f ? 1.f : 1.f / in_div,
+                       xo, yo);
     PSSR_LAUNCH_CHECK();
     return PSSR_OK;
+}
+
+int pssr_ssim_level_fwd_adj(const float* x, const float* y, float in_div, int planes, int h, int w, const float* win_host, int k, float c1,
+                            float c2, int use_ssim, double* sums, double* l1_sum, int stripes, int64_t stripe_stride, float* adj,
+                            pssr_stream_t s) {
+    return ssim_level_fwd_adj_launch(x, y, in_div, planes, h, w, win_host, k, c1, c2, use_ssim, sums, l1_sum, stripes, stripe_stride, adj,
+                                     nullptr, nullptr, s);
+}
+
+int pssr_ssim_level_fwd_adj_pool(const float* x, const float* y, float in_div, int planes, int h, int w, const float* win_host, int k, float c1,
+                                 float c2, int use_ssim, double* sums, double* l1_sum, int stripes, int64_t stripe_stride, float* adj,
+                                 float* xo, float* yo, pssr_stream_t s) {
+    PSSR_CHECK(xo && yo, PSSR_ERR_ARG, "ssim_level_fwd_adj_pool: null output");
+    PSSR_CHECK(h % 2 == 0 && w % 2 == 0, PSSR_ERR_UNSUPPORTED, "ssim_level_fwd_adj_pool: %dx%d is not even (the padded pool is pssr_avgpool2_pair_div's)", h, w);
+    return ssim_level_fwd_adj_launch(x, y, in_div, planes, h, w, win_host, k, c1, c2, use_ssim, sums, l1_sum, stripes, stripe_stride, adj, xo, yo, s);
 }
 
 int pssr_ssim_level_bwd_adj(const float* x, const float* y, float in_div, const float* adj, int planes, int h, int w, const float* win_host,
diff --git a/pssr2_amd/engine.py b/pssr2_amd/engine.py
--- a/pssr2_amd/engine.py
+++ b/pssr2_amd/engine.py
@@ -22,6 +22,8 @@
 _NO_MATERIALISE = os.environ.get("PSSR_MATERIALISE", "0") != "1"
 _XCOL_SIDE = os.environ.get("PSSR_XCOL_SIDE", "0") == "1"
 _FUSE_DOUT = os.environ.get("PSSR_FUSE_DOUT", "1") != "0"
+_TAIL_POOL = os.environ.get("PSSR_TAIL_POOL", "1") != "0"
+_TAIL_SHUF = os.environ.get("PSSR_TAIL_SHUF", "1") != "0"
 _OVERWRITE_GRADS = os.environ.get("PSSR_OVERWRITE_GRADS", "1") != "0"
 _EVAL_SHUF = os.environ.get("PSSR_EVAL_SHUF", "1") != "0"
 _EVAL_AFFINE = os.environ.get("PSSR_EVAL_AFFINE", "1") != "0"
@@ -582,7 +584,7 @@
             cache[(c, device)] = (perm, perm.to(torch.int32))
         return cache[(c, device)]
 
-    def _block_forward(self, p, blk, module, src, cin, first, dst, dst_coff, train, shuf=None):
+    def _block_forward(self, p, blk, module, src, cin, first, dst, dst_coff, train, shuf=None, pool=None):
         if blk.a is not None:
             A.ablock_forward(self, blk.a, module, p.xin if first else src, 0, p.n, p.code, dst, dst_coff, train)
             return
@@ -637,8 +639,15 @@
                 self._materialise(p, blk, k)
         pw = self._pw(rp, "fwd", p.code, **fwd_rp)
         last = blk.bn[-1]
+        slices = (dst.shape[-1], dst_coff, blk.y[-1].shape[-1])
+        out2 = {}
+        if pool is not None and _TAIL_POOL and ops.tail_pool_ok(p.code, blk.c, hh, ww, pool.shape[-1], *slices):
+            out2 = dict(pool2=pool)
+        elif shuf is not None and _TAIL_SHUF and ops.tail_shuffle_ok(p.code, blk.c, shuf.shape[-1], *slices):
+            out2 = dict(shuffle2=shuf)
         ops.conv2d(src, cin, pw, dst, blk.c, n=n, h=hh, w=ww, out_coff=dst_coff, bias=rp.bias, epilogue=L.EPI_TAIL,
-                   aux=blk.y[-1], aux_scale=last.scale, aux_shift=last.shift)
+                   aux=blk.y[-1], aux_scale=last.scale, aux_shift=last.shift, **out2)
+        return True if out2 else None
 
     def _forward_begin(self, x, train):
         m = self.model
@@ -681,8 +690,9 @@
             else:
                 dst, off = blk.out, 0
             shuffled = self._block_forward(p, blk, m.encoder[i], src, cin, i == 0, dst, off, train,
-                                           shuf=p.cat[Lv - 2] if (i == Lv - 1 and Lv > 1 and p.epool is None and not train) else None)
-            if i < Lv - 1:
+                                           shuf=p.cat[Lv - 2] if (i == Lv - 1 and Lv > 1 and p.epool is None) else None,
+                                           pool=p.pooled[i] if i < Lv - 1 else None)
+            if i < Lv - 1 and not shuffled:
                 ops.maxpool2(dst, p.pooled[i], n, *p.dims[i], hid[i], code, in_coff=off)
         deep = p.enc[Lv - 1].out
         if p.epool is not None:
@@ -694,7 +704,7 @@
                 ops.pixel_shuffle(prev, p.cat[l], n, *p.dims[l + 1], hid[l + 1] // 4, 2, code)
             blk = p.dec[l]
             shuffled = self._block_forward(p, blk, m.decoder[Lv - 2 - l], p.cat[l], p.cat[l].shape[-1], False, blk.out, 0, train,
-                                           shuf=p.cat[l - 1] if (l > 0 and not train) else None)
+                                           shuf=p.cat[l - 1] if l > 0 else None)
         feat = p.dec[0].out if Lv > 1 else deep
         if p.rpool is not None:
             A.psp_forward(self, p.rpool, m.reconstruction_pool, feat, 0, n, code, p.rpool_out, 0, train)
diff --git a/pssr2_amd/ops.py b/pssr2_amd/ops.py
--- a/pssr2_amd/ops.py
+++ b/pssr2_amd/ops.py
@@ -55,7 +55,8 @@
            x1=None, cin1=0, w1: PackedWeight | None = None, in1_coff=0,
            pro_scale=None, pro_shift=None, epilogue=L.EPI_STORE, flags=0,
            aux=None, aux_coff=0, aux_scale=None, aux_shift=None, aux_mean=None, aux_invstd=None, stats=None,
-           in0_blk=0, out_blk=0, aux_blk=0, out_scale=1.0, out_shift=0.0, gelu_in=False, head_w=None, head_q=None):
+           in0_blk=0, out_blk=0, aux_blk=0, out_scale=1.0, out_shift=0.0, gelu_in=False, head_w=None, head_q=None,
+           pool2=None, shuffle2=None, out2_coff=0):
     d = L.ConvDesc()
     d.dtype = w0.dtype
     d.n, d.h, d.w = n, h, w
@@ -79,6 +80,11 @@
         d.out_cstride, d.out_coff = cout, 0
     if epilogue == L.EPI_HEADQ or flags & L.FLAG_HEADQ:
         d.head_w, d.head_q = L.ptr(head_w), L.ptr(head_q)
+    if pool2 is not None or shuffle2 is not None:
+        if pool2 is not None and shuffle2 is not None:
+            raise ValueError("conv2d: one second output per launch")
+        o2, d.out2_kind = (pool2, L.OUT2_POOL2) if pool2 is not None else (shuffle2, L.OUT2_SHUFFLE2)
+        d.out2, d.out2_cstride, d.out2_coff = L.ptr(o2), o2.shape[-1], out2_coff
     ws_bytes = L.lib().pssr_conv2d_workspace_bytes(C.byref(d))
     if ws_bytes > 0:
         ws = torch.empty(ws_bytes, dtype=torch.uint8, device=out.device)
@@ -197,6 +203,18 @@
                                         L.ptr(stats), C.c_int64(npix), c, dtype, L.stream_ptr()), "pssr_relu_bwd_stats")
 
 
+def _tail_out2_ok(dtype, c, slices):
+    return dtype != L.F32 and c % 8 == 0 and all(v % 8 == 0 for v in slices) and L.lib().pssr_get_option(b"CONV_EPI8") > 0
+
+
+def tail_pool_ok(dtype, c, h, w, *slices):
+    return _tail_out2_ok(dtype, c, slices) and h % 2 == 0 and w % 2 == 0
+
+
+def tail_shuffle_ok(dtype, c, *slices):
+    return _tail_out2_ok(dtype, c, slices) and c % 32 == 0
+
+
 def relu_bwd_stats_fused_ok(dtype, c, h=2, w=2, unshuffle=False):
     return dtype != L.F32 and (c & (c - 1)) == 0 and c >= (32 if unshuffle else 8) and (unshuffle or (h % 2 == 0 and w % 2 == 0))
 
@@ -256,10 +274,18 @@
                                         L.ptr(l1_sum), L.stream_ptr()), "pssr_ssim_level_fwd")
 
 
-def ssim_level_fwd_adj(x, y, planes, h, w, win, c1, c2, use_ssim, sums, l1_sum, stripes, stripe_stride, adj, in_div=1.0):
+def ssim_level_fwd_adj(x, y, planes, h, w, win, c1, c2, use_ssim, sums, l1_sum, stripes, stripe_stride, adj, in_div=1.0, xo=None, yo=None):
     k = len(win); arr = (C.c_float * k)(*win)
-    L.check(L.lib().pssr_ssim_level_fwd_adj(L.ptr(x), L.ptr(y), C.c_float(in_div), planes, h, w, arr, k, C.c_float(c1), C.c_float(c2), int(use_ssim), L.ptr(sums),
-                                            L.ptr(l1_sum), stripes, C.c_int64(stripe_stride), L.ptr(adj), L.stream_ptr()), "pssr_ssim_level_fwd_adj")
+    if xo is None and yo is None:
+        L.check(L.lib().pssr_ssim_level_fwd_adj(L.ptr(x), L.ptr(y), C.c_float(in_div), planes, h, w, arr, k, C.c_float(c1), C.c_float(c2), int(use_ssim), L.ptr(sums),
+                                                L.ptr(l1_sum), stripes, C.c_int64(stripe_stride), L.ptr(adj), L.stream_ptr()), "pssr_ssim_level_fwd_adj")
+        return
+    for t in (xo, yo):
+        if t is None or t.dtype != torch.float32 or not t.is_contiguous() or t.numel() != planes * (h // 2) * (w // 2):
+            raise ValueError("ssim_level_fwd_adj: xo and yo must both be contiguous float32 [planes, h / 2, w / 2]")
+    L.check(L.lib().pssr_ssim_level_fwd_adj_pool(L.ptr(x), L.ptr(y), C.c_float(in_div), planes, h, w, arr, k, C.c_float(c1), C.c_float(c2), int(use_ssim),
+                                                 L.ptr(sums), L.ptr(l1_sum), stripes, C.c_int64(stripe_stride), L.ptr(adj), L.ptr(xo), L.ptr(yo),
+                                                 L.stream_ptr()), "pssr_ssim_level_fwd_adj_pool")
 
 
 def msssim_weights_striped(sums, stripes, stripe_stride, folded, levels, planes, nvalid, level_weights, ms, mix, l1_sum, l1_numel, grad_out,
diff --git a/pssr2_amd/util.py b/pssr2_amd/util.py
--- a/pssr2_amd/util.py
+++ b/pssr2_amd/util.py
@@ -2,6 +2,7 @@
 
 import inspect
 import math
+import os
 
 import numpy as np
 import torch
@@ -19,6 +20,8 @@
 
 
 _CONST_CACHE = {}
+
+_LOSS_PYRAMID = os.environ.get("PSSR_LOSS_PYRAMID", "1") != "0"
 
 
 class _SSIMLossFunction(torch.autograd.Function):
@@ -40,17 +43,16 @@
         if in_div != 1.0 and not fused_div:
             x, y = x / in_div, y / in_div
         div0 = in_div if fused_div else 1.0
-        xs, ys, dims = [x], [y], [(h, w)]
+        dims = [(h, w)]
         for lv in range(1, levels):
             hh, ww = dims[-1]
-            ho, wo = (hh + 2 * (hh & 1) - 2) // 2 + 1, (ww + 2 * (ww & 1) - 2) // 2 + 1
-            xo = torch.empty(planes, ho, wo, device=dev)
-            yo = torch.empty(planes, ho, wo, device=dev)
-            ops.avgpool2_pair(xs[-1], ys[-1], xo, yo, planes, hh, ww, div0 if lv == 1 else 1.0)
-            xs.append(xo), ys.append(yo), dims.append((ho, wo))
+            dims.append(((hh + 2 * (hh & 1) - 2) // 2 + 1, (ww + 2 * (ww & 1) - 2) // 2 + 1))
+        xs = [x] + [torch.empty(planes, hh, ww, device=dev) for hh, ww in dims[1:]]
+        ys = [y] + [torch.empty(planes, hh, ww, device=dev) for hh, ww in dims[1:]]
         adjs = None
         if k == 11 and ctx.needs_input_grad[0]:
             adjs = [torch.empty(planes * 3 * hh * ww, device=dev) for hh, ww in dims]
+        emit = [adjs is not None and _LOSS_PYRAMID and l + 1 < levels and dims[l][0] % 2 == 0 and dims[l][1] % 2 == 0 for l in range(levels)]
         stripes = 16 if adjs is not None else 1
         sstride = levels * planes * 2 + 2
         rows = 2 * stripes if stripes > 1 else 1
@@ -58,9 +60,13 @@
         l1_sum = sums[sstride - 2:sstride - 1] if mix < 1 else None
         for l in range(levels):
             hh, ww = dims[l]
+            ldiv = div0 if l == 0 else 1.0
+            if l + 1 < levels and not emit[l]:
+                ops.avgpool2_pair(xs[l], ys[l], xs[l + 1], ys[l + 1], planes, hh, ww, ldiv)
             if adjs is not None:
+                nxt = dict(xo=xs[l + 1], yo=ys[l + 1]) if emit[l] else {}
                 ops.ssim_level_fwd_adj(xs[l], ys[l], planes, hh, ww, win, c1, c2, l == levels - 1, sums[l * planes * 2:],
-                                       l1_sum if l == 0 else None, stripes, sstride, adjs[l], div0 if l == 0 else 1.0)
+                                       l1_sum if l == 0 else None, stripes, sstride, adjs[l], ldiv, **nxt)
             else:
                 ops.ssim_level_fwd(xs[l], ys[l], planes, hh, ww, win, c1, c2, sums[l * planes * 2:], l1_sum if l == 0 else None)
         ckey = (tuple(dims), k, tuple(lvl_w) if ms else (1.0,), str(dev))
```

After: 2428, median of 6. Within noise of the previous version (+0.9%).
